# hbb1/2d-gaussian-splatting

Hardware: AMD Instinct MI355X
Metric: train iters/sec (full iteration: rasterizer fwd+bwd, L1+SSIM, normal+dist regularisers, Adam) + fwd Msplats/s @1080p (higher is better)
Workload: dtype f32; 1 GPU; garden: trained synthetic capture, 5400000 initial points -> 2136144 surfels after 2500 iterations of the reference schedule, 32 views of 1600x1060; steady-state iteration, every loss term on; P=2136144, image=1600x1060, n_pass=6, tiles=6700

## Files before the change

### 2d-gaussian-splatting_amd/build.py

```python
import os
import subprocess
import sys

HERE = os.path.dirname(os.path.abspath(__file__))
CSRC = os.path.join(HERE, "csrc")
LIB = os.path.join(HERE, "lib", "libsurfel_hip.so")
SOURCES = ["surfel_preprocess.hip", "surfel_forward.hip", "surfel_backward.hip", "surfel_backward_scan.hip", "surfel_sort.hip", "surfel_api.hip", "knn.hip", "box_probe.hip",
           "train_loss.hip", "train_post.hip", "train_fused.hip", "train_optim.hip", "train_api.hip",
           "device_scan.hip", "mesh_tsdf.hip", "mesh_unbounded.hip", "eval_geometry.hip", "eval_tnt.hip", "metrics_lpips.hip", "scene_image.hip", "frame_vis.hip", "view_image.hip", "mesh_cull.hip", "mesh_view.hip", "frame_jpeg.hip", "frame_png.hip", "scene_jpeg.hip", "scene_undistort.hip", "train_log.hip", "log_events.cpp", "mesh_simplify.hip", "mesh_texture.hip", "mesh_smooth.hip", "mesh_repair.hip"]
EXTRA = {"surfel_forward.hip": ["-fno-slp-vectorize"], "surfel_backward.hip": ["-fno-slp-vectorize", "-ffp-contract=off"],
         "surfel_backward_scan.hip": ["-fno-slp-vectorize", "-ffp-contract=off"],
         "mesh_tsdf.hip": ["-ffp-contract=off"],
         "eval_geometry.hip": ["-ffp-contract=off"],
         "eval_tnt.hip": ["-ffp-contract=off"],
         "scene_image.hip": ["-ffp-contract=off"],
         "frame_vis.hip": ["-ffp-contract=off"],
         "view_image.hip": ["-ffp-contract=off"],
         "mesh_cull.hip": ["-ffp-contract=off"],
         "mesh_view.hip": ["-ffp-contract=off"],
         "frame_jpeg.hip": ["-ffp-contract=off"],
         "scene_undistort.hip": ["-ffp-contract=off"],
         "train_log.hip": ["-ffp-contract=off"],
         "mesh_simplify.hip": ["-ffp-contract=off"],
         "mesh_texture.hip": ["-ffp-contract=off"],
         "mesh_smooth.hip": ["-ffp-contract=off"],
         "mesh_repair.hip": ["-ffp-contract=off"]}
HEADERS = ["surfel_common.h", "surfel_kernels.h", "surfel_blend_bwd.h", "train_kernels.h", "train_loss_body.h", "train_post_body.h", os.path.join("..", "..", "include", "surfel_hip.h"), os.path.join("..", "..", "include", "surfel_debug.h"),
           os.path.join("..", "..", "include", "surfel_train.h"), "mesh_mc_table.h", "mesh_mc.h", "block_ops.h", "side_util.h", "carve.h", "mesh_topology.h", os.path.join("..", "..", "include", "surfel_mesh.h"),
           os.path.join("..", "..", "include", "surfel_mesh_unbounded.h"), os.path.join("..", "..", "include", "surfel_eval.h"),
           os.path.join("..", "..", "include", "surfel_eval_tnt.h"), os.path.join("..", "..", "include", "surfel_metrics.h"),
           os.path.join("..", "..", "include", "surfel_scene.h"), "vis_turbo_table.h", os.path.join("..", "..", "include", "surfel_vis.h"),
           "vis_pixels.h", os.path.join("..", "..", "include", "surfel_view.h"), os.path.join("..", "..", "include", "surfel_cull.h"),
           "jpeg_tables.h", os.path.join("..", "..", "include", "surfel_jpeg.h"), os.path.join("..", "..", "include", "surfel_png.h"),
           os.path.join("..", "..", "include", "surfel_jpegdec.h"), os.path.join("..", "..", "include", "surfel_undistort.h"),
           "log_jet_table.h", os.path.join("..", "..", "include", "surfel_log.h"), "mesh_raster.h", "mesh_sample.h",
           os.path.join("..", "..", "include", "surfel_meshview.h"), os.path.join("..", "..", "include", "surfel_simplify.h"),
           os.path.join("..", "..", "include", "surfel_texture.h"), os.path.join("..", "..", "include", "surfel_smooth.h"),
           os.path.join("..", "..", "include", "surfel_repair.h")]
FLAGS = ["--offload-arch=gfx950", "-O3", "-std=c++17", "-fPIC", "-ffp-contract=fast", "-Wall", "-Wno-unused-result"]


def _stale(out, deps):
    if not os.path.exists(out):
        return True
    t = os.path.getmtime(out)
    return any(os.path.getmtime(d) > t for d in deps)


def build_variant(tag, defines, verbose=False):
    hipcc = os.environ.get("HIPCC", "/opt/rocm/bin/hipcc")
    bdir = os.path.join(HERE, "build_" + tag)
    os.makedirs(bdir, exist_ok=True)
    os.makedirs(os.path.join(HERE, "lib"), exist_ok=True)
    lib = os.path.join(HERE, "lib", "libsurfel_hip_%s.so" % tag)
    objs = []
    for src in SOURCES:
        obj = os.path.join(bdir, src + ".o")
        objs.append(obj)
        cmd = [hipcc] + FLAGS + list(defines) + EXTRA.get(src, []) + ["-c", os.path.join(CSRC, src), "-o", obj]
        if verbose:
            print(" ".join(cmd))
        subprocess.check_call(cmd)
    subprocess.check_call([hipcc, "--offload-arch=gfx950", "-shared", "-fPIC", "-o", lib] + objs)
    return lib


def build(force=False, verbose=False, ieee=False):
    hipcc = os.environ.get("HIPCC", "/opt/rocm/bin/hipcc")
    os.makedirs(os.path.join(HERE, "lib"), exist_ok=True)
    bdir = os.path.join(HERE, "build_ieee" if ieee else "build")
    os.makedirs(bdir, exist_ok=True)
    LIB = os.path.join(HERE, "lib", "libsurfel_hip_ieee.so" if ieee else "libsurfel_hip.so")
    hdrs = [os.path.join(CSRC, h) for h in HEADERS]
    objs = []
    for src in SOURCES:
        sp = os.path.join(CSRC, src)
        obj = os.path.join(bdir, src + ".o")
        objs.append(obj)
        if force or _stale(obj, [sp] + hdrs):
            cmd = [hipcc] + FLAGS + (["-DSURFEL_IEEE_MATH"] if ieee else []) + EXTRA.get(src, []) + ["-c", sp, "-o", obj]
            if verbose:
                print(" ".join(cmd))
            subprocess.check_call(cmd)
    if force or _stale(LIB, objs):
        cmd = [hipcc, "--offload-arch=gfx950", "-shared", "-fPIC", "-o", LIB] + objs
        if verbose:
            print(" ".join(cmd))
        subprocess.check_call(cmd)
    return LIB


if __name__ == "__main__":
    if "--variant" in sys.argv:
        k = sys.argv.index("--variant")
        print(build_variant(sys.argv[k + 1], sys.argv[k + 2:], verbose=False))
        sys.exit(0)
    print(build(force="--force" in sys.argv, verbose=True, ieee="--ieee" in sys.argv))
```

### 2d-gaussian-splatting_amd/csrc/surfel_api.hip

```cpp
#include <cstring>
#include <mutex>
#include <string>
#include <vector>

#include <hip/hip_runtime.h>

#include "../../include/surfel_debug.h"
#include "carve.h"
#include "surfel_common.h"
#include "surfel_kernels.h"
#include "train_kernels.h"

using namespace surfel;

namespace {

const char* kStageNames[] = {"preprocess_fwd", "depth_sort_scan", "emit_instances", "tile_sort", "tile_ranges", "blend_fwd",
                             "zero_grec", "blend_bwd", "preprocess_bwd", "knn", "tile_depth_sort"};
enum Stage { ST_PRE = 0, ST_SCAN, ST_EMIT, ST_SORT, ST_RANGES, ST_BLEND, ST_ZERO, ST_BBWD, ST_PBWD, ST_KNN, ST_TSORT, ST_COUNT };
static_assert(sizeof(kStageNames) / sizeof(kStageNames[0]) == ST_COUNT, "one name per stage");

struct CapEntry {
    int W = 0, H = 0; int64_t maxR = -1; unsigned frames = 0; int uniform_streak = 0; int boost = 0; unsigned last_overflow = 0;
    int slot() const; void begin_frame(); int64_t capacity(int end_bit) const; void record_count(int64_t R, bool overflowed);
};
constexpr int kCapEntries = 16;

constexpr int kMaxDevices = 32;
constexpr int kPinnedTotal = R_SLOTS + kCapEntries;
struct PerDevice { hipEvent_t ev = nullptr; uint32_t* pinned = nullptr; };

thread_local std::string g_err;
struct ThreadState {
    int64_t last_R = -1; int last_W = 0, last_H = 0;
    CapEntry caps[kCapEntries]; unsigned cap_next = 0; int cap_evictions = 0;
    int last_binning = 0;
    float stage_ms[16] = {}; int stage_id[16] = {}; int stage_n = 0;
    PerDevice dev[kMaxDevices];
};
thread_local ThreadState g_th;

int g_opt_cull = 1;
int g_opt_tile_sort = 1;
int g_opt_bwd_variant = 2;
int g_opt_stream = 1;
int g_opt_capacity = 1;
int g_opt_tile_order = 0;
surfel_hook_fn g_colour_hook = nullptr;
void* g_colour_hook_user = nullptr;
unsigned long long* g_blend_stats = nullptr;

int fail(int code, const char* what, hipError_t e = hipSuccess) {
    g_err = what;
    if (e != hipSuccess) { g_err += ": "; g_err += hipGetErrorString(e); }
    return code;
}

#define HIP_TRY(expr)                                                    \
    do {                                                                 \
        hipError_t _e = (expr);                                          \
        if (_e != hipSuccess) return fail(SURFEL_E_HIP, #expr, _e);      \
    } while (0)

struct GeomState {
    float* rec; float* depths; uint32_t* tiles_touched; uint8_t* clamped;
    uint32_t *dkey_a, *dkey_b, *ord_a, *ord_b;
    uint32_t* offsets;
    uint32_t* rects;
    float* shjac;
    char* temp;
    static GeomState carve(void* base, int P, size_t temp_bytes, size_t* total) {
        Carver c(base); GeomState g;
        g.rec = c.take<float>((size_t)P * REC_F);
        g.depths = c.take<float>(P);
        g.tiles_touched = c.take<uint32_t>(P);
        g.clamped = c.take<uint8_t>(P);
        g.dkey_a = c.take<uint32_t>(P); g.dkey_b = c.take<uint32_t>(P);
        g.ord_a = c.take<uint32_t>(P); g.ord_b = c.take<uint32_t>(P);
        g.offsets = c.take<uint32_t>(P);
        g.rects = c.take<uint32_t>(P);
        g.shjac = c.take<float>((size_t)9 * P);
        g.temp = c.take<char>(temp_bytes);
        if (total) *total = c.size();
        return g;
    }
};

struct BinState {
    uint32_t* point_list; uint32_t* vals_alt; uint32_t* keys_a; uint32_t* keys_b; char* sort_temp;
    float4* strm_rec = nullptr; uint32_t* strm_mask = nullptr;
    static bool wants_stream(size_t R) { return g_opt_stream != 0 && R > 0 && (long long)R <= STRM_MAX_R; }
    static BinState carve(void* base, size_t R, size_t sort_bytes, size_t* total, bool stream = false) {
        Carver c(base); BinState b;
        b.point_list = c.take<uint32_t>(R);
        b.vals_alt = c.take<uint32_t>(R);
        b.keys_a = c.take<uint32_t>(R);
        b.keys_b = c.take<uint32_t>(R);
        if (stream) {
            b.strm_rec = c.take<float4>(R * STRM_Q);
            b.strm_mask = c.take<uint32_t>(R);
        }
        b.sort_temp = c.take<char>(sort_bytes);
        if (total) *total = c.size();
        return b;
    }
};

struct ImgState {
    uint2* ranges; uint32_t* total; float* final_T; uint32_t* n_contrib; int* tile_map;
    static ImgState carve(void* base, int W, int H, size_t* total) {
        Carver c(base); ImgState im;
        const size_t tiles = (size_t)((W + TILE - 1) / TILE) * ((H + TILE - 1) / TILE);
        im.ranges = c.take<uint2>(tiles + R_SLOTS + 2);
        im.total = reinterpret_cast<uint32_t*>(im.ranges + tiles);
        im.final_T = c.take<float>((size_t)3 * W * H);
        im.n_contrib = c.take<uint32_t>((size_t)2 * W * H);
        im.tile_map = c.take<int>((size_t)tile_map_len((W + TILE - 1) / TILE, (H + TILE - 1) / TILE));
        if (total) *total = c.size();
        return im;
    }
};

struct StreamReg { const void* bin = nullptr; const void* img = nullptr; const float4* rec = nullptr; const uint32_t* mask = nullptr; bool jac = false; };
constexpr int kStreamRegs = 64;
StreamReg g_stream_regs[kStreamRegs];
unsigned g_stream_next = 0;
std::mutex g_stream_mu;
void stream_register(const void* bin, const void* img, const float4* rec, const uint32_t* mask, bool jac) {
    std::lock_guard<std::mutex> lk(g_stream_mu);
    for (auto& r : g_stream_regs) if (r.bin == bin) { r.img = img; r.rec = rec; r.mask = mask; r.jac = jac; return; }
    g_stream_regs[g_stream_next++ % kStreamRegs] = StreamReg{bin, img, rec, mask, jac};
}
bool stream_lookup(const void* bin, const void* img, const float4** rec, const uint32_t** mask, bool* jac) {
    std::lock_guard<std::mutex> lk(g_stream_mu);
    for (auto& r : g_stream_regs) if (r.bin == bin && r.img == img) {
        *jac = r.jac;
        if (!r.rec) return false;
        *rec = r.rec; *mask = r.mask;
        return true;
    }
    return false;
}

struct PendingStage { int stage; hipEvent_t e0, e1; };
std::vector<PendingStage> g_pending;
constexpr size_t kMaxPending = 8192;
std::mutex g_pending_mu;

struct StageTimer {
    int mode; hipStream_t s; hipEvent_t e0 = nullptr, e1 = nullptr;
    StageTimer(int mode_, hipStream_t s_) : mode(mode_), s(s_) {
        if (mode == 1) { (void)hipEventCreate(&e0); (void)hipEventCreate(&e1); }
    }
    ~StageTimer() { if (mode == 1) { (void)hipEventDestroy(e0); (void)hipEventDestroy(e1); } }
    bool armed = false;
    void begin(int stage = -1) {
        armed = mode == 1 || mode == 2 || (mode == 3 && stage == ST_BBWD);
        if (!armed) return;
        if (mode >= 2) { (void)hipEventCreate(&e0); (void)hipEventCreate(&e1); }
        (void)hipEventRecord(e0, s);
    }
    int end(int stage) {
        if (!armed) return 0;
        armed = false;
        (void)hipEventRecord(e1, s);
        if (mode >= 2) {
            std::lock_guard<std::mutex> lk(g_pending_mu);
            if (g_pending.size() >= kMaxPending) {
                (void)hipEventDestroy(g_pending.front().e0); (void)hipEventDestroy(g_pending.front().e1);
                g_pending.erase(g_pending.begin());
            }
            g_pending.push_back({stage, e0, e1});
            return 0;
        }
        hipError_t e = hipEventSynchronize(e1);
        if (e != hipSuccess) return (int)e;
        e = hipGetLastError();
        if (e != hipSuccess) return (int)e;
        float ms = 0.f; (void)hipEventElapsedTime(&ms, e0, e1);
        if (g_th.stage_n < 16) { g_th.stage_ms[g_th.stage_n] = ms; g_th.stage_id[g_th.stage_n] = stage; g_th.stage_n++; }
        return 0;
    }
};
#define STAGE_END(timer, st)                                                               \
    do {                                                                                   \
        int _e = (timer).end(st);                                                          \
        if (_e) return fail(SURFEL_E_HIP, kStageNames[st], (hipError_t)_e);                \
    } while (0)

PerDevice* per_device(int dev = -1) {
    int d = dev;
    if (d < 0 && hipGetDevice(&d) != hipSuccess) return nullptr;
    if (d < 0 || d >= kMaxDevices) return nullptr;
    return &g_th.dev[d];
}

hipEvent_t r_event() {
    PerDevice* pd = per_device();
    if (!pd) return nullptr;
    if (!pd->ev) { if (hipEventCreateWithFlags(&pd->ev, hipEventDisableTiming) != hipSuccess) pd->ev = nullptr; }
    return pd->ev;
}

uint32_t* pinned_u32() {
    PerDevice* pd = per_device();
    if (!pd) return nullptr;
    if (!pd->pinned) {
        if (hipHostMalloc(reinterpret_cast<void**>(&pd->pinned), sizeof(uint32_t) * (R_SLOTS + kCapEntries + 8), hipHostMallocMapped) != hipSuccess) pd->pinned = nullptr;
        else for (int k = 0; k < R_SLOTS + kCapEntries + 8; k++) pd->pinned[k] = 0u;
    }
    return pd->pinned;
}

int64_t pinned_total(const uint32_t* hR, bool host_total) {
    if (host_total) return (int64_t)hR[kPinnedTotal];
    int64_t R = 0;
    for (int k = 0; k < R_SLOTS; k++) R += (int64_t)hR[k];
    return R;
}

CapEntry* cap_entry(int W, int H) {
    for (auto& c : g_th.caps) if (c.W == W && c.H == H) return &c;
    CapEntry* c = &g_th.caps[g_th.cap_next++ % kCapEntries];
    if (c->W != 0) g_th.cap_evictions++;
    *c = CapEntry{};
    c->W = W; c->H = H;
    c->frames = ~0u;
    return c;
}

int CapEntry::slot() const { return (int)(this - g_th.caps); }
void CapEntry::begin_frame() {
    if (frames == ~0u) {
        frames = 0;
        if (uint32_t* hv = pinned_u32()) hv[R_SLOTS + slot()] = 0u;
    }
    frames++;
    if (boost > 0 && frames - last_overflow > 256u) { boost--; last_overflow = frames; }
}
int64_t CapEntry::capacity(int end_bit) const {
    if (maxR < 0) return 0;
    int64_t cap = maxR + (maxR >> (3 - boost)) + 4096;
    cap = (cap + 16383) / 16384 * 16384;
    return (cap > ((int64_t)1 << 20) || !capacity_binning_ok((size_t)cap, end_bit)) ? 0 : cap;
}
void CapEntry::record_count(int64_t R, bool overflowed) {
    g_th.last_R = R; g_th.last_W = W; g_th.last_H = H;
    if (overflowed) { if (boost < 2) boost++; last_overflow = frames; }
    maxR = R > maxR - maxR / 64 ? R : maxR - maxR / 64;
}

void run_tile_order(CapEntry* ce, const uint2* ranges, int gx, int gy, int* map, uint32_t* map_flag, int opt, hipStream_t s) {
    if (opt == 1) return;
    uint32_t* hv = pinned_u32();
    uint32_t* verdict = nullptr;
    if (hv && opt == 0) {
        const uint32_t v = hv[R_SLOTS + ce->slot()];
        if (v == 1u) ce->uniform_streak = ce->uniform_streak < 1000 ? ce->uniform_streak + 1 : 1000;
        else if (v == 2u) ce->uniform_streak = 0;
        void* dv = nullptr;
        if (hipHostGetDevicePointer(&dv, hv + R_SLOTS + ce->slot(), 0) == hipSuccess) verdict = static_cast<uint32_t*>(dv);
        if (verdict && ce->uniform_streak >= 4 && (ce->frames & 7u) != 0u) return;
    }
    launch_tile_order(ranges, gx, gy, map, map_flag, opt, verdict, s);
}

int higher_msb(uint32_t n) {
    int b = 0;
    while ((1ull << b) < (unsigned long long)n) b++;
    return b < 1 ? 1 : b;
}

int per_tile_pays(int64_t R, int P, int gx, int gy) {
    const int64_t tiles = (int64_t)gx * gy, Pf = P > (1 << 20) ? P : (1 << 20);
    if (R <= 640 * tiles) return 1;
    return (2 * R <= 7 * Pf && R <= 2048 * tiles) ? 1 : 0;
}

int alloc_bin(size_t n, size_t sort_bytes, bool stream, surfel_alloc_fn binning_alloc, void* binning_user, BinState* bin) {
    const bool strm = stream && BinState::wants_stream(n);
    size_t bytes = 0;
    BinState::carve(nullptr, n, sort_bytes, &bytes, strm);
    void* base = binning_alloc(binning_user, bytes > 0 ? bytes : 256);
    if (!base) return fail(SURFEL_E_ALLOC, "binning buffer allocation failed");
    *bin = BinState::carve(base, n, sort_bytes, nullptr, strm);
    return 0;
}

int bin_capacity(const PreprocessArgs& pa, int end_bit, int64_t cap, int64_t maxR, const GeomState& geom, const BinState& bin,
                 const ImgState& img, uint32_t* hR, hipEvent_t evR, StageTimer& tm, hipStream_t s) {
    uint32_t* n_dev = img.total + 2 * R_SLOTS;
    const bool odd = radix_sort_result_buffer((size_t)cap, 0, end_bit) == 1;
    uint32_t* va = odd ? bin.vals_alt : bin.point_list;
    uint32_t* vb = odd ? bin.point_list : bin.vals_alt;
    tm.begin();
    launch_bin_emit(pa.P, geom.tiles_touched, geom.rects, geom.offsets, geom.rec, bin.keys_a, va, pa.gx, (size_t)cap, bin.sort_temp, end_bit,
                    n_dev, hR + kPinnedTotal, s);
    HIP_TRY(hipEventRecord(evR, s));
    STAGE_END(tm, ST_EMIT);
    tm.begin();
    const bool fused_ranges = end_bit > 0;
    const int wk = radix_sort_pairs_u32_devn(bin.keys_a, va, bin.keys_b, vb, (size_t)cap, end_bit, n_dev, bin.sort_temp, fused_ranges ? img.ranges : nullptr, s);
    STAGE_END(tm, ST_SORT);
    if (!fused_ranges) { tm.begin(); launch_tile_ranges_devn((size_t)cap, n_dev, wk ? bin.keys_b : bin.keys_a, img.ranges, s); STAGE_END(tm, ST_RANGES); }
    tm.begin(); launch_tile_depth_sort(pa.gx * pa.gy, maxR, img.ranges, bin.point_list, geom.dkey_a, bin.vals_alt, bin.keys_a, bin.keys_b, fused_ranges, s);
    STAGE_END(tm, ST_TSORT);
    return 0;
}

int64_t bin_exact(const PreprocessArgs& pa, int end_bit, int per_tile, int64_t R, const GeomState& geom, BinState* bin,
                  const ImgState& img, const uint32_t* hR, hipEvent_t evR, bool stream, surfel_alloc_fn binning_alloc, void* binning_user,
                  StageTimer& tm, hipStream_t s) {
    if (per_tile < 0 && R < 0) {
        HIP_TRY(hipEventSynchronize(evR));
        per_tile = per_tile_pays(pinned_total(hR, false), pa.P, pa.gx, pa.gy);
    }
    tm.begin();
    const uint32_t* order = geom.ord_a;
    if (!per_tile) {
        const int which = radix_sort_pairs_u32(geom.dkey_a, geom.ord_a, geom.dkey_b, geom.ord_b, (size_t)pa.P, 0, 32, geom.temp, s, true);
        if (which < 0) return fail(SURFEL_E_LIMIT, "too many surfels for the depth sort");
        order = which ? geom.ord_b : geom.ord_a;
    }
    launch_scan_gather(geom.tiles_touched, order, pa.pack_tiles, geom.offsets, (size_t)pa.P, pa.zero_b, s);
    STAGE_END(tm, ST_SCAN);
    if (R < 0) {
        HIP_TRY(hipEventSynchronize(evR));
        R = pinned_total(hR, false);
    }
    if (int e = alloc_bin((size_t)R, radix_sort_scratch_bytes((size_t)R), stream, binning_alloc, binning_user, bin)) return e;
    if (R == 0) return 0;
    const bool odd = radix_sort_result_buffer((size_t)R, 0, end_bit) == 1;
    uint32_t* va = odd ? bin->vals_alt : bin->point_list;
    uint32_t* vb = odd ? bin->point_list : bin->vals_alt;
    tm.begin();
    launch_emit_instances(pa.P, geom.rec, geom.rects, order, pa.pack_tiles ? ((1u << PACK_ID_BITS) - 1u) : 0xffffffffu, geom.offsets, bin->keys_a, va, pa.gx,
                          reinterpret_cast<uint32_t*>(bin->sort_temp), (uint32_t)radix_sort_head_words((size_t)R), s);
    STAGE_END(tm, ST_EMIT);
    tm.begin();
    const int wk = radix_sort_pairs_u32(bin->keys_a, va, bin->keys_b, vb, (size_t)R, 0, end_bit, bin->sort_temp, s, true);
    if (wk < 0) return fail(SURFEL_E_LIMIT, "too many tile instances for the tile sort");
    STAGE_END(tm, ST_SORT);
    tm.begin(); launch_tile_ranges(R, wk ? bin->keys_b : bin->keys_a, img.ranges, s); STAGE_END(tm, ST_RANGES);
    if (per_tile) {
        tm.begin(); launch_tile_depth_sort(pa.gx * pa.gy, R, img.ranges, bin->point_list, geom.dkey_a, bin->vals_alt, bin->keys_a, bin->keys_b, false, s);
        STAGE_END(tm, ST_TSORT);
    }
    return R;
}

int blend(CapEntry* ce, int W, int H, int gx, int gy, const ImgState& img, const void* img_base, const BinState& bin, const float* rec,
          const float* background, float* out_color, float* out_others, int avg_list, bool jac, int tile_order, StageTimer& tm, hipStream_t s) {
    run_tile_order(ce, img.ranges, gx, gy, img.tile_map, img.total + 2 * R_SLOTS + 1, tile_order, s);
    BlendFwdArgs ba{};
    ba.W = W; ba.H = H; ba.gx = gx; ba.gy = gy;
    ba.ranges = img.ranges; ba.point_list = bin.point_list; ba.rec = rec; ba.bg = background;
    ba.out_color = out_color; ba.out_others = out_others; ba.final_T = img.final_T; ba.n_contrib = img.n_contrib;
    ba.tile_map = img.tile_map; ba.map_flag = img.total + 2 * R_SLOTS + 1; ba.map_len = tile_map_len(gx, gy);
    ba.stats = g_blend_stats;
    ba.avg_list = avg_list;
    ba.strm_rec = bin.strm_rec; ba.strm_mask = bin.strm_mask; ba.totals = img.total; ba.walk_word = img.total + 2 * R_SLOTS + 2;
    stream_register(bin.point_list, img_base, launch_blend_fwd_writes_stream(ba) ? bin.strm_rec : nullptr, bin.strm_mask, jac);
    tm.begin(); launch_blend_fwd(ba, s); STAGE_END(tm, ST_BLEND);
    return 0;
}

}

namespace surfel {
int api_fail(int code, const char* what, hipError_t e) { return fail(code, what, e); }
}

extern "C" {

int surfel_abi_version(void) { return SURFEL_ABI_VERSION; }
const char* surfel_last_error(void) { return g_err.c_str(); }
const char* surfel_stage_name(int stage) { return (stage >= 0 && stage < ST_COUNT) ? kStageNames[stage] : "?"; }
int surfel_last_stage_ms(float* ms, int cap) {
    int n = g_th.stage_n < cap ? g_th.stage_n : cap;
    for (int i = 0; i < n; i++) ms[i] = g_th.stage_ms[i];
    return n;
}
int surfel_last_stage_ids(int* ids, int cap) {
    int n = g_th.stage_n < cap ? g_th.stage_n : cap;
    for (int i = 0; i < n; i++) ids[i] = g_th.stage_id[i];
    return n;
}

int surfel_debug_sort_pairs(surfel_alloc_fn scratch_alloc, void* scratch_user, uint32_t* keys, uint32_t* vals, int64_t n,
                            int begin_bit, int end_bit, void* stream) {
    if (!scratch_alloc || n < 0 || (n > 0 && (!keys || !vals)) || begin_bit < 0 || end_bit > 32 || begin_bit > end_bit)
        return fail(SURFEL_E_INVALID, "bad arguments");
    if (n == 0) return 0;
    hipStream_t s = static_cast<hipStream_t>(stream);
    const size_t sb = radix_sort_scratch_bytes((size_t)n);
    const size_t words = align_up((size_t)n * sizeof(uint32_t));
    char* base = static_cast<char*>(scratch_alloc(scratch_user, 2 * words + sb));
    if (!base) return fail(SURFEL_E_ALLOC, "sort scratch allocation failed");
    uint32_t* kb = reinterpret_cast<uint32_t*>(base);
    uint32_t* vb = reinterpret_cast<uint32_t*>(base + words);
    const int w = radix_sort_pairs_u32(keys, vals, kb, vb, (size_t)n, begin_bit, end_bit, base + 2 * words, s);
    if (w < 0) return fail(SURFEL_E_LIMIT, "sort size limit");
    if (w == 1) {
        HIP_TRY(hipMemcpyAsync(keys, kb, (size_t)n * sizeof(uint32_t), hipMemcpyDeviceToDevice, s));
        HIP_TRY(hipMemcpyAsync(vals, vb, (size_t)n * sizeof(uint32_t), hipMemcpyDeviceToDevice, s));
    }
    HIP_TRY(hipGetLastError());
    return 0;
}

int surfel_debug_tile_depth_sort(int ntiles, int64_t n, uint32_t* ranges, uint32_t* point_list, const uint32_t* depth_keys, uint32_t* scratch,
                                 int decode, void* stream) {
    if (ntiles < 0 || n < 0 || n >= ((int64_t)1 << 32) || (ntiles > 0 && !ranges) || (n > 0 && (!point_list || !depth_keys || !scratch)))
        return fail(SURFEL_E_INVALID, "bad arguments");
    if (ntiles == 0) return 0;
    launch_tile_depth_sort(ntiles, n, reinterpret_cast<uint2*>(ranges), point_list, depth_keys, scratch, scratch + n, scratch + 2 * n, decode != 0,
                           static_cast<hipStream_t>(stream));
    HIP_TRY(hipGetLastError());
    return 0;
}
int surfel_debug_tile_depth_sort_classes(int* out, int cap) {
    if (!out || cap < 0) return fail(SURFEL_E_INVALID, "bad arguments");
    return tile_depth_sort_classes(out, cap);
}
int surfel_debug_set_tile_radix_min(int longest_network_run) { set_tile_radix_min(longest_network_run); return 0; }

int surfel_set_option(const char* name, int value) {
    if (name && std::strcmp(name, "cull") == 0) { g_opt_cull = value ? 1 : 0; return 0; }
    if (name && std::strcmp(name, "tile_depth_sort") == 0) { g_opt_tile_sort = value < 0 ? 0 : (value > 2 ? 2 : value); return 0; }
    if (name && std::strcmp(name, "large_sort") == 0) { set_large_sort_impl(value); return 0; }
    if (name && std::strcmp(name, "fwd_pipe") == 0) { set_fwd_pipe(value); return 0; }
    if (name && std::strcmp(name, "preprocess_dma") == 0) { set_preprocess_dma(value); return 0; }
    if (name && std::strcmp(name, "bwd_variant") == 0) { g_opt_bwd_variant = value < 0 ? 0 : (value > 3 ? 3 : value); return 0; }
    if (name && std::strcmp(name, "tile_stream") == 0) { g_opt_stream = value != 0; return 0; }
    if (name && std::strcmp(name, "capacity_binning") == 0) { g_opt_capacity = value != 0; return 0; }
    if (name && std::strcmp(name, "tile_order") == 0) { g_opt_tile_order = value < 0 ? 0 : (value > 2 ? 2 : value); return 0; }
    return fail(SURFEL_E_INVALID, "unknown option");
}

int surfel_set_backward_hook(surfel_hook_fn colour_ready, void* user) {
    g_colour_hook = colour_ready; g_colour_hook_user = user;
    return 0;
}

int surfel_debug_last_binning(void) { return g_th.last_binning; }
int surfel_debug_capacity_evictions(void) { return g_th.cap_evictions; }

int surfel_debug_image_layout(int width, int height, int64_t* out) {
    if (width <= 0 || height <= 0 || !out) return fail(SURFEL_E_INVALID, "bad arguments");
    size_t total = 0;
    ImgState::carve(nullptr, width, height, &total);
    char* const base = reinterpret_cast<char*>(static_cast<uintptr_t>(1) << 40);
    const ImgState im = ImgState::carve(base, width, height, nullptr);
    out[0] = (int64_t)total;
    out[1] = reinterpret_cast<char*>(im.final_T) - base;
    out[2] = reinterpret_cast<char*>(im.n_contrib) - base;
    out[3] = reinterpret_cast<char*>(im.tile_map) - base;
    return 0;
}
int surfel_debug_set_blend_stats(void* dev_u64x8) { g_blend_stats = static_cast<unsigned long long*>(dev_u64x8); return 0; }

int surfel_collect_stage_ms(float* sum_ms, int* count, int cap) {
    for (int i = 0; i < cap; i++) { sum_ms[i] = 0.f; count[i] = 0; }
    std::lock_guard<std::mutex> lk(g_pending_mu);
    for (auto& p : g_pending) {
        float ms = 0.f;
        if (hipEventSynchronize(p.e1) == hipSuccess && hipEventElapsedTime(&ms, p.e0, p.e1) == hipSuccess && p.stage < cap) {
            sum_ms[p.stage] += ms; count[p.stage]++;
        }
        (void)hipEventDestroy(p.e0); (void)hipEventDestroy(p.e1);
    }
    g_pending.clear();
    return ST_COUNT;
}

struct LazyPending { bool pending = false; int W = 0, H = 0, dev = -1; int64_t cap = 0; bool overflowed = false; int64_t R = 0; };
thread_local LazyPending g_lazy;

int64_t lazy_finish() {
    if (!g_lazy.pending) return g_lazy.R;
    PerDevice* pd = per_device(g_lazy.dev);
    uint32_t* hR = pd ? pd->pinned : nullptr;
    hipEvent_t evR = pd ? pd->ev : nullptr;
    if (!hR || !evR) return fail(SURFEL_E_HIP, "pinned buffer / event of the lazily counted frame's device not found");
    HIP_TRY(hipEventSynchronize(evR));
    const int64_t R = pinned_total(hR, true);
    g_lazy.pending = false;
    g_lazy.R = R;
    g_lazy.overflowed = R > g_lazy.cap;
    CapEntry* ce = cap_entry(g_lazy.W, g_lazy.H);
    if (ce->frames == ~0u) ce->frames = 0;
    ce->record_count(R, g_lazy.overflowed);
    return R;
}

int64_t surfel_forward_count(void) {
    const int64_t R = lazy_finish();
    if (R < 0) return R;
    if (g_lazy.overflowed) {
        g_lazy.overflowed = false;
        return fail(SURFEL_E_OVERFLOW, "the lazily counted frame held more tile instances than its capacity: render it again (its outputs are incomplete)");
    }
    return R;
}

int64_t surfel_rasterize_forward(surfel_alloc_fn geom_alloc, void* geom_user, surfel_alloc_fn binning_alloc, void* binning_user,
                                 surfel_alloc_fn image_alloc, void* image_user, int P, int D, int M, const float* background,
                                 int width, int height, const float* means3D, const float* shs, const float* colors_precomp,
                                 const float* opacities, const float* scales, float scale_modifier, const float* rotations,
                                 const float* transMat_precomp, const float* viewmatrix, const float* projmatrix,
                                 const float* cam_pos, float tan_fovx, float tan_fovy, int prefiltered, float* out_color,
                                 float* out_others, int* radii, int debug, void* stream) {
    (void)tan_fovx; (void)tan_fovy; (void)prefiltered;
    g_th.stage_n = 0;
    if (g_lazy.pending) { const int64_t r = lazy_finish(); if (r < 0) return r; }
    if (g_lazy.overflowed) {
        g_lazy.overflowed = false;
        return fail(SURFEL_E_OVERFLOW, "the previous lazily counted frame overflowed its capacity and surfel_forward_count() was never called for it");
    }
    const bool opt_lazy = (debug & SURFEL_OPT_LAZY_COUNT) != 0;
    const int opt_cull = (debug & SURFEL_OPT_NO_CULL) ? 0 : g_opt_cull;
    const int opt_tile_sort = ((debug >> 9) & 3) ? ((debug >> 9) & 3) - 1 : g_opt_tile_sort;
    const int opt_capacity = (debug & SURFEL_OPT_EXACT_BINNING) ? 0 : g_opt_capacity;
    const int opt_tile_order = ((debug >> 19) & 3) ? ((debug >> 19) & 3) - 1 : g_opt_tile_order;
    const bool opt_stream = !(debug & SURFEL_OPT_NO_STREAM);
    debug &= 0xff;
    g_th.last_binning = 0;
    hipStream_t s = static_cast<hipStream_t>(stream);
    if (!geom_alloc || !binning_alloc || !image_alloc) return fail(SURFEL_E_INVALID, "allocator callback is NULL");
    if (P < 0 || width <= 0 || height <= 0) return fail(SURFEL_E_INVALID, "bad sizes");
    if (P > 0) {
        if ((shs == nullptr) == (colors_precomp == nullptr)) return fail(SURFEL_E_INVALID, "provide exactly one of shs / colors_precomp");
        const bool has_sr = scales != nullptr && rotations != nullptr;
        if (has_sr == (transMat_precomp != nullptr) || ((scales != nullptr) != (rotations != nullptr)))
            return fail(SURFEL_E_INVALID, "provide exactly one of (scales, rotations) / transMat_precomp");
        if (!means3D || !opacities || !viewmatrix || !projmatrix || !cam_pos || !radii) return fail(SURFEL_E_INVALID, "required pointer is NULL");
        if (D < 0 || D > 3 || (shs && M < (D + 1) * (D + 1))) return fail(SURFEL_E_INVALID, "bad SH degree / coefficient count");
    }
    if (!background || !out_color || !out_others) return fail(SURFEL_E_INVALID, "required pointer is NULL");
    const int gx = (width + TILE - 1) / TILE, gy = (height + TILE - 1) / TILE;
    if (gx > 1023 || gy > 1023) return fail(SURFEL_E_LIMIT, "image larger than 16368 px per side");

    size_t img_bytes = 0;
    ImgState::carve(nullptr, width, height, &img_bytes);
    void* img_base = image_alloc(image_user, img_bytes);
    if (!img_base) return fail(SURFEL_E_ALLOC, "image buffer allocation failed");
    ImgState img = ImgState::carve(img_base, width, height, nullptr);
    HIP_TRY(hipMemsetAsync(img.ranges, 0, (size_t)(reinterpret_cast<char*>(img.final_T) - reinterpret_cast<char*>(img.ranges)), s));

    StageTimer tm(debug, s);
    const bool jac = P > 0 && opt_stream && shs != nullptr && M == 16;
    CapEntry* ce = cap_entry(width, height);
    ce->begin_frame();
    int64_t R = 0;
    bool blended = false;
    GeomState geom{}; BinState bin{};
    if (P == 0) {
        (void)geom_alloc(geom_user, 256);
        if (int e = alloc_bin(0, 0, false, binning_alloc, binning_user, &bin)) return e;
        g_lazy.R = 0;
    } else {
        const size_t psort_bytes = align_up(radix_sort_scratch_bytes((size_t)P));
        const size_t temp_bytes = psort_bytes + scan_scratch_words((size_t)P) * sizeof(uint32_t);
        size_t geom_bytes = 0;
        GeomState::carve(nullptr, P, temp_bytes, &geom_bytes);
        void* geom_base = geom_alloc(geom_user, geom_bytes);
        if (!geom_base) return fail(SURFEL_E_ALLOC, "geometry buffer allocation failed");
        geom = GeomState::carve(geom_base, P, temp_bytes, nullptr);

        PreprocessArgs pa{};
        pa.P = P; pa.D = D; pa.M = M; pa.W = width; pa.H = height; pa.gx = gx; pa.gy = gy; pa.scale_modifier = scale_modifier;
        pa.cull = opt_cull;
        pa.pack_tiles = P < (1 << PACK_ID_BITS) ? 1 : 0;
        pa.means3D = means3D; pa.opacities = opacities; pa.scales = scales; pa.rotations = rotations;
        pa.transMat_precomp = transMat_precomp; pa.colors_precomp = colors_precomp; pa.shs = shs;
        pa.viewmatrix = viewmatrix; pa.projmatrix = projmatrix; pa.campos = cam_pos;
        pa.rec = geom.rec; pa.depths = geom.depths; pa.depth_keys = geom.dkey_a; pa.ident = geom.ord_a; pa.radii = radii;
        pa.tiles_touched = geom.tiles_touched; pa.clamped = geom.clamped; pa.total_instances = img.total; pa.rects = geom.rects;
        pa.shjac = jac ? geom.shjac : nullptr;
        pa.zero_a = reinterpret_cast<uint32_t*>(geom.temp); pa.zero_a_words = (uint32_t)radix_sort_head_words((size_t)P);
        pa.zero_b = reinterpret_cast<uint32_t*>(geom.temp + psort_bytes); pa.zero_b_words = (uint32_t)scan_scratch_words((size_t)P);

        const int end_bit = higher_msb((uint32_t)(gx * gy));
        int per_tile = opt_tile_sort == 2 ? 1 : (opt_tile_sort == 0 ? 0 : -1);
        if (per_tile < 0 && g_th.last_R >= 0 && g_th.last_W == width && g_th.last_H == height) per_tile = per_tile_pays(g_th.last_R, P, gx, gy);
        const int64_t cap = (opt_capacity && per_tile == 1 && debug != 1) ? ce->capacity(end_bit) : 0;
        if (cap > 0) {
            if (int e = alloc_bin((size_t)cap, capacity_sort_scratch_bytes((size_t)cap, end_bit), opt_stream, binning_alloc, binning_user, &bin)) return e;
            pa.zero_c = reinterpret_cast<uint32_t*>(bin.sort_temp); pa.zero_c_words = (uint32_t)bin_emit_head_words();
            pa.block_totals = geom.offsets;
        }
        tm.begin(); launch_preprocess_fwd(pa, s); STAGE_END(tm, ST_PRE);
        uint32_t* hR = pinned_u32();
        hipEvent_t evR = r_event();
        if (!hR || !evR) return fail(SURFEL_E_HIP, "pinned buffer / event creation failed");
        if (cap == 0) {
            HIP_TRY(hipMemcpyAsync(hR, img.total, sizeof(uint32_t) * R_SLOTS, hipMemcpyDeviceToHost, s));
            HIP_TRY(hipEventRecord(evR, s));
        } else {
            if (int e = bin_capacity(pa, end_bit, cap, ce->maxR, geom, bin, img, hR, evR, tm, s)) return e;
            if (int e = blend(ce, width, height, gx, gy, img, img_base, bin, geom.rec, background, out_color, out_others, 0, jac, opt_tile_order, tm, s)) return e;
            if (opt_lazy) {
                g_lazy.pending = true; g_lazy.W = width; g_lazy.H = height; g_lazy.cap = cap; g_lazy.overflowed = false;
                if (hipGetDevice(&g_lazy.dev) != hipSuccess) g_lazy.dev = -1;
                g_th.last_binning = 4;
                HIP_TRY(hipGetLastError());
                return cap;
            }
            HIP_TRY(hipEventSynchronize(evR));
            R = pinned_total(hR, true);
            blended = R <= cap;
            g_th.last_binning = blended ? 1 : 2;
            if (!blended) {
                HIP_TRY(hipMemsetAsync(img.ranges, 0, sizeof(uint2) * (size_t)gx * gy, s));
                HIP_TRY(hipMemsetAsync(img.total + 2 * R_SLOTS, 0, 2 * sizeof(uint32_t), s));
            }
        }
        if (!blended) {
            R = bin_exact(pa, end_bit, per_tile, cap > 0 ? R : -1, geom, &bin, img, hR, evR, opt_stream, binning_alloc, binning_user, tm, s);
            if (R < 0) return R;
        }
        ce->record_count(R, cap > 0 && !blended);
        g_lazy.R = R;
    }
    if (!blended) {
        if (int e = blend(ce, width, height, gx, gy, img, img_base, bin, geom.rec, background, out_color, out_others, (int)(R / ((int64_t)gx * gy)), jac, opt_tile_order, tm, s)) return e;
    }
    HIP_TRY(hipGetLastError());
    return R;
}

int surfel_rasterize_backward(surfel_alloc_fn scratch_alloc, void* scratch_user, int P, int D, int M, int64_t R,
                              const float* background, int width, int height, const float* means3D, const float* shs,
                              const float* colors_precomp, const float* scales, float scale_modifier, const float* rotations,
                              const float* transMat_precomp, const float* viewmatrix, const float* projmatrix,
                              const float* cam_pos, float tan_fovx, float tan_fovy, const int* radii, const void* geom_buffer,
                              const void* binning_buffer, const void* image_buffer, const float* dL_dout_color,
                              const float* dL_dout_others, float* dL_dmeans2D, float* dL_dnormal, float* dL_dopacity,
                              float* dL_dcolors, float* dL_dmeans3D, float* dL_dtransMat, float* dL_dsh, float* dL_dscales,
                              float* dL_drots, int debug, void* stream) {
    (void)tan_fovx; (void)tan_fovy; (void)colors_precomp;
    g_th.stage_n = 0;
    const int debug_in = debug;
    const int opt_variant = (debug & SURFEL_OPT_BWD_SCAN) ? 3 : ((debug & SURFEL_OPT_BWD_QUAD) ? 1 : ((debug & SURFEL_OPT_BWD_ROWS) ? 0 : g_opt_bwd_variant));
    debug &= 0xff;
    hipStream_t s = static_cast<hipStream_t>(stream);
    if (P == 0) return 0;
    if (!scratch_alloc || !geom_buffer || !binning_buffer || !image_buffer) return fail(SURFEL_E_INVALID, "buffer / allocator is NULL");
    if (!dL_dout_color || !dL_dout_others || !dL_dmeans2D || !dL_dopacity || !dL_dcolors || !dL_dmeans3D)
        return fail(SURFEL_E_INVALID, "gradient pointer is NULL");
    if (transMat_precomp && !dL_dtransMat) return fail(SURFEL_E_INVALID, "dL_dtransMat is NULL but transMat_precomp was given");
    if (!transMat_precomp && (!dL_dscales || !dL_drots || !scales || !rotations)) return fail(SURFEL_E_INVALID, "scale/rotation pointers are NULL");
    const int gx = (width + TILE - 1) / TILE, gy = (height + TILE - 1) / TILE;

    GeomState geom = GeomState::carve(const_cast<void*>(geom_buffer), P, 0, nullptr);
    BinState bin = BinState::carve(const_cast<void*>(binning_buffer), (size_t)R, 0, nullptr);
    ImgState img = ImgState::carve(const_cast<void*>(image_buffer), width, height, nullptr);

    const size_t grec_bytes = align_up((size_t)(R > 0 ? R : 1) * GREC_F * sizeof(float));
    const size_t cut_bytes = align_up((size_t)gx * gy * sizeof(uint2));
    float* grec = static_cast<float*>(scratch_alloc(scratch_user, grec_bytes + cut_bytes + (size_t)P));
    if (!grec) return fail(SURFEL_E_ALLOC, "gradient record allocation failed");
    const bool use_cut = (debug_in & SURFEL_OPT_TILE_CUTS) ? true : ((debug_in & SURFEL_OPT_ZERO_RECORDS) ? false : R >= ((int64_t)1 << 21));
    uint2* cut = use_cut ? reinterpret_cast<uint2*>(reinterpret_cast<char*>(grec) + grec_bytes) : nullptr;
    uint8_t* has_rec = use_cut ? reinterpret_cast<uint8_t*>(grec) + grec_bytes + cut_bytes : nullptr;
    if (has_rec) HIP_TRY(hipMemsetAsync(has_rec, 0, (size_t)P, s));
    StageTimer tm(debug, s);

    BlendBwdArgs bb{};
    bb.W = width; bb.H = height; bb.gx = gx; bb.gy = gy;
    bb.ranges = img.ranges; bb.point_list = bin.point_list; bb.rec = geom.rec; bb.bg = background;
    bb.final_T = img.final_T; bb.n_contrib = img.n_contrib; bb.dL_dpix = dL_dout_color; bb.dL_dothers = dL_dout_others;
    bb.tile_map = img.tile_map; bb.map_flag = img.total + 2 * R_SLOTS + 1; bb.map_len = tile_map_len(gx, gy);
    bb.grec = grec; bb.cut = cut; bb.has_rec = has_rec; bb.depths = geom.depths; bb.variant = opt_variant; bb.stats = g_blend_stats; bb.walk_word = img.total + 2 * R_SLOTS + 2;
    bool have_jac = false;
    {
        const float4* srec = nullptr; const uint32_t* smask = nullptr;
        const bool found = stream_lookup(binning_buffer, image_buffer, &srec, &smask, &have_jac);
        if (found && !(debug_in & SURFEL_OPT_BWD_GATHER) && g_opt_stream) { bb.strm_rec = srec; bb.strm_mask = smask; }
    }
    bb.n_dev = img.total + 2 * R_SLOTS; bb.n_cap = (uint32_t)(R < 0xffffffffll ? R : 0xffffffffll);
    if (R > 0) {
        const bool auto_walk = opt_variant == 2;
        bb.variant = auto_walk ? 0 : opt_variant;
        if (auto_walk && !g_blend_stats) {
            if (R >= ((int64_t)1 << 21)) bb.variant = R < ((int64_t)1 << 26) ? 3 : 0;
            else bb.scan_rule = 1;
        }
        tm.begin(ST_BBWD);
        launch_blend_bwd(bb, s);
        STAGE_END(tm, ST_BBWD);
    }

    PreprocessBwdArgs pb{};
    pb.P = P; pb.D = D; pb.M = M; pb.W = width; pb.H = height; pb.scale_modifier = scale_modifier;
    pb.coop = (debug_in & SURFEL_OPT_PBWD_COOP) ? 1 : ((debug_in & SURFEL_OPT_PBWD_THREAD) ? 0 : ((R >= (int64_t)6 * P && R >= ((int64_t)32 << 20)) ? 1 : 0));
    pb.shjac = (have_jac && !(debug_in & SURFEL_OPT_PBWD_NO_JAC)) ? geom.shjac : nullptr;
    pb.means3D = means3D; pb.radii = radii; pb.shs = shs; pb.clamped = geom.clamped; pb.scales = scales; pb.rotations = rotations;
    pb.transMat_precomp = transMat_precomp; pb.viewmatrix = viewmatrix; pb.projmatrix = projmatrix; pb.campos = cam_pos;
    pb.rec = geom.rec; pb.tiles_touched = geom.tiles_touched; pb.grec = grec; pb.cut = cut; pb.has_rec = has_rec; pb.depths = geom.depths; pb.gx = gx;
    pb.n_dev = bb.n_dev; pb.n_cap = bb.n_cap;
    pb.dL_dtransMat = dL_dtransMat; pb.dL_dnormal = dL_dnormal; pb.dL_dopacity = dL_dopacity; pb.dL_dcolors = dL_dcolors;
    pb.dL_dsh = dL_dsh; pb.dL_dmeans2D = dL_dmeans2D; pb.dL_dmeans3D = dL_dmeans3D; pb.dL_dscales = dL_dscales; pb.dL_drots = dL_drots;
    tm.begin();
    if (g_colour_hook) {
        launch_colour_gradients(pb, s);
        pb.keep_colors = 1;
        g_colour_hook(g_colour_hook_user);
    }
    launch_preprocess_bwd(pb, s);
    STAGE_END(tm, ST_PBWD);
    HIP_TRY(hipGetLastError());
    return 0;
}

int surfel_mark_visible(int P, const float* means3D, const float* viewmatrix, const float* projmatrix, uint8_t* present,
                        void* stream) {
    (void)projmatrix;
    if (P < 0 || (P > 0 && (!means3D || !viewmatrix || !present))) return fail(SURFEL_E_INVALID, "bad arguments");
    launch_mark_visible(P, means3D, viewmatrix, present, static_cast<hipStream_t>(stream));
    HIP_TRY(hipGetLastError());
    return 0;
}

int surfel_knn_dist2(surfel_alloc_fn scratch_alloc, void* scratch_user, int P, const float* points, float* mean_dist2,
                     void* stream) {
    if (P < 0 || (P > 0 && (!points || !mean_dist2 || !scratch_alloc))) return fail(SURFEL_E_INVALID, "bad arguments");
    if (P == 0) return 0;
    const size_t bytes = knn_scratch_bytes(P);
    void* scratch = scratch_alloc(scratch_user, bytes);
    if (!scratch) return fail(SURFEL_E_ALLOC, "knn scratch allocation failed");
    launch_knn(P, points, mean_dist2, scratch, bytes, static_cast<hipStream_t>(stream));
    HIP_TRY(hipGetLastError());
    return 0;
}

}
```

### 2d-gaussian-splatting_amd/csrc/surfel_kernels.h

```cpp
#pragma once
#include <hip/hip_runtime.h>
#include <stdint.h>

namespace surfel {

struct PreprocessArgs {
    int P, D, M, W, H, gx, gy;
    int cull;
    int pack_tiles;
    float scale_modifier;
    const float* means3D; const float* opacities; const float* scales; const float* rotations;
    const float* transMat_precomp; const float* colors_precomp; const float* shs;
    const float* viewmatrix; const float* projmatrix; const float* campos;
    float* rec; float* depths; uint32_t* depth_keys; uint32_t* ident; int* radii; uint32_t* tiles_touched; uint8_t* clamped;
    uint32_t* rects;
    float* shjac;
    uint32_t* total_instances;
    uint32_t* block_totals;
    uint32_t* zero_a; uint32_t zero_a_words;
    uint32_t* zero_b; uint32_t zero_b_words;
    uint32_t* zero_c; uint32_t zero_c_words;
};

struct BlendFwdArgs {
    int W, H, gx, gy;
    const uint2* ranges; const uint32_t* point_list; const float* rec; const float* bg;
    float* out_color; float* out_others; float* final_T; uint32_t* n_contrib;
    const int* tile_map; const uint32_t* map_flag; int map_len;
    unsigned long long* stats;
    int avg_list;
    float4* strm_rec; uint32_t* strm_mask;
    const uint32_t* totals; uint32_t* walk_word;
};

struct BlendBwdArgs {
    int W, H, gx, gy;
    const uint2* ranges; const uint32_t* point_list; const float* rec; const float* bg;
    const float* final_T; const uint32_t* n_contrib;
    const int* tile_map; const uint32_t* map_flag; int map_len;
    const float* dL_dpix; const float* dL_dothers;
    float* grec;
    uint2* cut;
    uint8_t* has_rec;
    const float* depths;
    int variant;
    const float4* strm_rec; const uint32_t* strm_mask;
    int scan_rule;
    const uint32_t* walk_word;
    const uint32_t* n_dev; uint32_t n_cap;
    unsigned long long* stats;
};

struct PreprocessBwdArgs {
    int P, D, M, W, H;
    int coop;
    int keep_colors;
    const float* shjac;
    float scale_modifier;
    const float* means3D; const int* radii; const float* shs; const uint8_t* clamped;
    const float* scales; const float* rotations; const float* transMat_precomp;
    const float* viewmatrix; const float* projmatrix; const float* campos;
    const float* rec; const uint32_t* tiles_touched; const float* grec;
    const uint2* cut; const uint8_t* has_rec; const float* depths; int gx;
    const uint32_t* n_dev; uint32_t n_cap;
    float* dL_dtransMat; float* dL_dnormal; float* dL_dopacity; float* dL_dcolors; float* dL_dsh;
    float* dL_dmeans2D; float* dL_dmeans3D; float* dL_dscales; float* dL_drots;
};

void launch_preprocess_fwd(const PreprocessArgs& a, hipStream_t s);
void set_preprocess_dma(int v);
void launch_emit_instances(int P, float* rec, const uint32_t* rects, const uint32_t* order, uint32_t id_mask, const uint32_t* offsets_sorted, uint32_t* keys,
                           uint32_t* vals, int gx, uint32_t* zero_ptr, uint32_t zero_words, hipStream_t s);
void launch_tile_ranges(int64_t R, const uint32_t* keys, uint2* ranges, hipStream_t s);
int tile_map_len(int gx, int gy);
void launch_tile_order(const uint2* ranges, int gx, int gy, int* map, uint32_t* map_flag , int force, uint32_t* verdict, hipStream_t s);
void launch_blend_fwd(const BlendFwdArgs& a, hipStream_t s);
bool launch_blend_fwd_writes_stream(const BlendFwdArgs& a);
void set_fwd_pipe(int v);
void launch_mark_visible(int P, const float* means3D, const float* vm, uint8_t* present, hipStream_t s);
void launch_blend_bwd(const BlendBwdArgs& a, hipStream_t s);
void launch_blend_bwd_scan(const BlendBwdArgs& a, hipStream_t s);
void launch_preprocess_bwd(const PreprocessBwdArgs& a, hipStream_t s);
void launch_colour_gradients(const PreprocessBwdArgs& a, hipStream_t s);
void launch_knn(int P, const float* points, float* out, void* scratch, size_t scratch_bytes, hipStream_t s);
size_t knn_scratch_bytes(int P);
size_t radix_sort_scratch_bytes(size_t n);
void set_large_sort_impl(int v);
int radix_sort_passes(size_t n, int begin_bit, int end_bit);
int radix_sort_result_buffer(size_t n, int begin_bit, int end_bit);
int radix_sort_pairs_u32(uint32_t* keys_a, uint32_t* vals_a, uint32_t* keys_b, uint32_t* vals_b, size_t n, int begin_bit, int end_bit,
                         void* scratch, hipStream_t s, bool head_zeroed = false);
size_t radix_sort_head_words(size_t n);
size_t scan_scratch_words(size_t n);
int tile_depth_sort_classes(int* out, int cap);
void set_tile_radix_min(int v);
void launch_tile_depth_sort(int ntiles, int64_t R, uint2* ranges, uint32_t* point_list, const uint32_t* depth_keys, uint32_t* tmp_ids,
                            uint32_t* tmp_keys, uint32_t* tmp_rank, bool decode, hipStream_t s);
void launch_scan_gather(const uint32_t* vals, const uint32_t* order, int packed, uint32_t* out, size_t n, void* zeroed_scratch, hipStream_t s);
bool capacity_binning_ok(size_t cap, int end_bit);
size_t capacity_sort_scratch_bytes(size_t cap, int end_bit);
size_t bin_emit_head_words();
void launch_bin_emit(int P, const uint32_t* tiles_touched, const uint32_t* rects, const uint32_t* block_totals, float* rec, uint32_t* keys, uint32_t* vals,
                     int gx, size_t cap, void* sort_scratch , int end_bit, uint32_t* n_out, uint32_t* n_host ,
                     hipStream_t s);
int radix_sort_pairs_u32_devn(uint32_t* keys_a, uint32_t* vals_a, uint32_t* keys_b, uint32_t* vals_b, size_t cap, int end_bit, const uint32_t* n_dev,
                              void* scratch, uint2* ranges, hipStream_t s);
void launch_tile_ranges_devn(size_t cap, const uint32_t* n_dev, const uint32_t* keys, uint2* ranges, hipStream_t s);

}
```

### 2d-gaussian-splatting_amd/csrc/surfel_preprocess.hip

```cpp
#include "surfel_common.h"
#include "surfel_kernels.h"

namespace surfel {


__device__ __constant__ float SH_C0 = 0.28209479177387814f;
__device__ __constant__ float SH_C1 = 0.4886025119029199f;
__device__ __constant__ float SH_C2[5] = {1.0925484305920792f, -1.0925484305920792f, 0.31539156525252005f,
                                          -1.0925484305920792f, 0.5462742152960396f};
__device__ __constant__ float SH_C3[7] = {-0.5900435899266435f, 2.890611442640554f, -0.4570457994644658f,
                                          0.3731763325901154f, -0.4570457994644658f, 1.445305721320277f,
                                          -0.5900435899266435f};

__device__ __forceinline__ void sh_basis_gradient(int D, float x, float y, float z, float (&Bx)[16], float (&By)[16], float (&Bz)[16]) {
#pragma unroll
    for (int k = 0; k < 16; k++) { Bx[k] = 0.f; By[k] = 0.f; Bz[k] = 0.f; }
    if (D > 0) {
        By[1] = -SH_C1; Bz[2] = SH_C1; Bx[3] = -SH_C1;
        if (D > 1) {
            const float xx = x * x, yy = y * y, zz = z * z, xy = x * y, yz = y * z, xz = x * z;
            Bx[4] = SH_C2[0] * y; By[4] = SH_C2[0] * x;
            By[5] = SH_C2[1] * z; Bz[5] = SH_C2[1] * y;
            Bx[6] = SH_C2[2] * -2.f * x; By[6] = SH_C2[2] * -2.f * y; Bz[6] = SH_C2[2] * 4.f * z;
            Bx[7] = SH_C2[3] * z; Bz[7] = SH_C2[3] * x;
            Bx[8] = SH_C2[4] * 2.f * x; By[8] = SH_C2[4] * -2.f * y;
            if (D > 2) {
                Bx[9] = SH_C3[0] * 6.f * xy; By[9] = SH_C3[0] * 3.f * (xx - yy);
                Bx[10] = SH_C3[1] * yz; By[10] = SH_C3[1] * xz; Bz[10] = SH_C3[1] * xy;
                Bx[11] = SH_C3[2] * -2.f * xy; By[11] = SH_C3[2] * (-3.f * yy + 4.f * zz - xx); Bz[11] = SH_C3[2] * 8.f * yz;
                Bx[12] = SH_C3[3] * -6.f * xz; By[12] = SH_C3[3] * -6.f * yz; Bz[12] = SH_C3[3] * 3.f * (2.f * zz - xx - yy);
                Bx[13] = SH_C3[4] * (-3.f * xx + 4.f * zz - yy); By[13] = SH_C3[4] * -2.f * xy; Bz[13] = SH_C3[4] * 8.f * xz;
                Bx[14] = SH_C3[5] * 2.f * xz; By[14] = SH_C3[5] * -2.f * yz; Bz[14] = SH_C3[5] * (xx - yy);
                Bx[15] = SH_C3[6] * 3.f * (xx - yy); By[15] = SH_C3[6] * -6.f * xy;
            }
        }
    }
}

__device__ __forceinline__ void sh_colour_jacobian(int D, float x, float y, float z, const float4 (&c4)[12], float (&G)[3][3]) {
    float Bx[16], By[16], Bz[16];
    sh_basis_gradient(D, x, y, z, Bx, By, Bz);
#pragma unroll
    for (int c = 0; c < 3; c++) { G[c][0] = 0.f; G[c][1] = 0.f; G[c][2] = 0.f; }
#pragma unroll
    for (int v = 0; v < 12; v++) {
        const float cv[4] = {c4[v].x, c4[v].y, c4[v].z, c4[v].w};
#pragma unroll
        for (int e = 0; e < 4; e++) {
            const int flat = 4 * v + e, k = flat / 3, c = flat % 3;
            G[c][0] = __builtin_fmaf(Bx[k], cv[e], G[c][0]); G[c][1] = __builtin_fmaf(By[k], cv[e], G[c][1]); G[c][2] = __builtin_fmaf(Bz[k], cv[e], G[c][2]);
        }
    }
}

__device__ __forceinline__ uint32_t preprocess_one(const PreprocessArgs& a, const int i, const float4* sh_lds = nullptr) {
    int rad_out = 0;
    uint32_t tiles = 0;
    uint32_t dkey = 0xffffffffu;
    const float* __restrict__ vm = a.viewmatrix;
    const float px = a.means3D[3 * i], py = a.means3D[3 * i + 1], pz = a.means3D[3 * i + 2];
    const float opa_in = a.opacities[i];
    float4 q_in = make_float4(1.f, 0.f, 0.f, 0.f);
    float2 sc_in = make_float2(1.f, 1.f);
    if (a.transMat_precomp == nullptr) {
        q_in = reinterpret_cast<const float4*>(a.rotations)[i];
        sc_in = reinterpret_cast<const float2*>(a.scales)[i];
    }
    const float vx = vm[0] * px + vm[4] * py + vm[8] * pz + vm[12];
    const float vy = vm[1] * px + vm[5] * py + vm[9] * pz + vm[13];
    const float vz = vm[2] * px + vm[6] * py + vm[10] * pz + vm[14];
    do {
        if (vz <= 0.2f) break;
        float T[9];
        float nx, ny, nz;
        if (a.transMat_precomp == nullptr) {
            const float4 q = q_in;
            const float2 sc = sc_in;
            const float s = rsqrtf(q.x * q.x + q.y * q.y + q.z * q.z + q.w * q.w);
            const float w = q.x * s, x = q.y * s, y = q.z * s, z = q.w * s;
            const float sx = a.scale_modifier * sc.x, sy = a.scale_modifier * sc.y;
            const float L0x = (1.f - 2.f * (y * y + z * z)) * sx, L0y = (2.f * (x * y + w * z)) * sx, L0z = (2.f * (x * z - w * y)) * sx;
            const float L1x = (2.f * (x * y - w * z)) * sy, L1y = (1.f - 2.f * (x * x + z * z)) * sy, L1z = (2.f * (y * z + w * x)) * sy;
            const float L2x = 2.f * (x * z + w * y), L2y = 2.f * (y * z - w * x), L2z = 1.f - 2.f * (x * x + y * y);
            float Pm[12];
            world2pix(a.projmatrix, a.W, a.H, Pm);
#pragma unroll
            for (int c = 0; c < 3; c++) {
                T[3 * c + 0] = L0x * Pm[0 * 3 + c] + L0y * Pm[1 * 3 + c] + L0z * Pm[2 * 3 + c];
                T[3 * c + 1] = L1x * Pm[0 * 3 + c] + L1y * Pm[1 * 3 + c] + L1z * Pm[2 * 3 + c];
                T[3 * c + 2] = px * Pm[0 * 3 + c] + py * Pm[1 * 3 + c] + pz * Pm[2 * 3 + c] + Pm[3 * 3 + c];
            }
            nx = vm[0] * L2x + vm[4] * L2y + vm[8] * L2z;
            ny = vm[1] * L2x + vm[5] * L2y + vm[9] * L2z;
            nz = vm[2] * L2x + vm[6] * L2y + vm[10] * L2z;
        } else {
#pragma unroll
            for (int k = 0; k < 9; k++) T[k] = a.transMat_precomp[9 * (size_t)i + k];
            nx = 0.f; ny = 0.f; nz = 1.f;
        }
        const float cosv = -(vx * nx + vy * ny + vz * nz);
        if (cosv == 0.f) break;
        const float flip = cosv > 0.f ? 1.f : -1.f;
        nx *= flip; ny *= flip; nz *= flip;

        const float t0 = CUTOFF * CUTOFF, t2 = -1.0f;
        const float dist = t0 * T[6] * T[6] + t0 * T[7] * T[7] + t2 * T[8] * T[8];
        if (dist == 0.f) break;
        const float f0 = t0 / dist, f2 = t2 / dist;
        const float cx = f0 * T[0] * T[6] + f0 * T[1] * T[7] + f2 * T[2] * T[8];
        const float cy = f0 * T[3] * T[6] + f0 * T[4] * T[7] + f2 * T[5] * T[8];
        const float hx = cx * cx - (f0 * T[0] * T[0] + f0 * T[1] * T[1] + f2 * T[2] * T[2]);
        const float hy = cy * cy - (f0 * T[3] * T[3] + f0 * T[4] * T[4] + f2 * T[5] * T[5]);
        const float ex = sqrtf(fmaxf(1e-4f, hx)), ey = sqrtf(fmaxf(1e-4f, hy));
        const float radius = ceilf(fmaxf(fmaxf(ex, ey), CUTOFF * FILTER_SIZE));
        const int irad = (int)radius;
        const Rect rc = tile_rect(cx, cy, irad, a.gx, a.gy);
        const int ntiles = (rc.x1 - rc.x0) * (rc.y1 - rc.y0);
        if (ntiles == 0) break;

        float r = 0.f, g = 0.f, b = 0.f;
        uint8_t clampbits = 0;
        if (a.colors_precomp == nullptr) {
            const float4* __restrict__ shq = reinterpret_cast<const float4*>(a.shs + (size_t)i * a.M * 3);
            float dx = px - a.campos[0], dy = py - a.campos[1], dz = pz - a.campos[2];
            const float il = rsqrtf(dx * dx + dy * dy + dz * dz);
            dx *= il; dy *= il; dz *= il;
            float B[16];
#pragma unroll
            for (int k = 1; k < 16; k++) B[k] = 0.f;
            B[0] = SH_C0;
            int nb = 1;
            if (a.D > 0) {
                B[1] = -SH_C1 * dy; B[2] = SH_C1 * dz; B[3] = -SH_C1 * dx; nb = 4;
                if (a.D > 1) {
                    const float xx = dx * dx, yy = dy * dy, zz = dz * dz, xy = dx * dy, yz = dy * dz, xz = dx * dz;
                    B[4] = SH_C2[0] * xy; B[5] = SH_C2[1] * yz; B[6] = SH_C2[2] * (2.f * zz - xx - yy);
                    B[7] = SH_C2[3] * xz; B[8] = SH_C2[4] * (xx - yy); nb = 9;
                    if (a.D > 2) {
                        B[9] = SH_C3[0] * dy * (3.f * xx - yy); B[10] = SH_C3[1] * xy * dz;
                        B[11] = SH_C3[2] * dy * (4.f * zz - xx - yy); B[12] = SH_C3[3] * dz * (2.f * zz - 3.f * xx - 3.f * yy);
                        B[13] = SH_C3[4] * dx * (4.f * zz - xx - yy); B[14] = SH_C3[5] * dz * (xx - yy);
                        B[15] = SH_C3[6] * dx * (xx - 3.f * yy); nb = 16;
                    }
                }
            }
            if (a.M == 16) {
                float4 c4[12];
#pragma unroll
                for (int v = 0; v < 12; v++) c4[v] = make_float4(0.f, 0.f, 0.f, 0.f);
                if (sh_lds) {
                    asm volatile("s_waitcnt vmcnt(0)" ::: "memory");
#pragma unroll
                    for (int v = 0; v < 12; v++) c4[v] = sh_lds[v];
                } else if (a.D > 2) {
#pragma unroll
                    for (int v = 0; v < 12; v++) c4[v] = shq[v];
                } else if (a.D == 2) {
#pragma unroll
                    for (int v = 0; v < 7; v++) c4[v] = shq[v];
                } else if (a.D == 1) {
#pragma unroll
                    for (int v = 0; v < 3; v++) c4[v] = shq[v];
                } else {
                    c4[0] = shq[0];
                }
                float acc[3] = {0.f, 0.f, 0.f};
#pragma unroll
                for (int v = 0; v < 12; v++) {
                    const float cv[4] = {c4[v].x, c4[v].y, c4[v].z, c4[v].w};
#pragma unroll
                    for (int e = 0; e < 4; e++) {
                        const int flat = 4 * v + e;
                        acc[flat % 3] += B[flat / 3] * cv[e];
                    }
                }
                r = acc[0]; g = acc[1]; b = acc[2];
                if (a.shjac) {
                    float G[3][3];
                    sh_colour_jacobian(a.D, dx, dy, dz, c4, G);
#pragma unroll
                    for (int c = 0; c < 3; c++) {
#pragma unroll
                        for (int q = 0; q < 3; q++) a.shjac[(size_t)(3 * c + q) * a.P + i] = G[c][q];
                    }
                }
            } else {
                const float* __restrict__ sh = a.shs + (size_t)i * a.M * 3;
                r = SH_C0 * sh[0]; g = SH_C0 * sh[1]; b = SH_C0 * sh[2];
                if (nb > 1) {
#pragma unroll
                    for (int k = 1; k < 16; k++) {
                        if (k < nb && k < a.M) { r += B[k] * sh[3 * k]; g += B[k] * sh[3 * k + 1]; b += B[k] * sh[3 * k + 2]; }
                    }
                }
            }
            r += 0.5f; g += 0.5f; b += 0.5f;
            clampbits = (r < 0.f ? 1 : 0) | (g < 0.f ? 2 : 0) | (b < 0.f ? 4 : 0);
            r = fmaxf(r, 0.f); g = fmaxf(g, 0.f); b = fmaxf(b, 0.f);
        } else {
            r = a.colors_precomp[3 * (size_t)i]; g = a.colors_precomp[3 * (size_t)i + 1]; b = a.colors_precomp[3 * (size_t)i + 2];
        }
        float bx0 = 1.f, bx1 = 0.f, by0 = 1.f, by1 = 0.f;
        float ecx = cx, ecy = cy, Sxx = FOOT_UNBOUNDED, Sxy = 0.f, Syy = FOOT_UNBOUNDED, r2sq = 0.f, Sdet = 1.f;
        {
            const float opa = opa_in;
            if (opa * 255.f >= 0.999f) {
                const float rmax = 2.f * __logf(fmaxf(opa * 255.f, 1.f)) * 1.0001f + 1e-3f;
                const float r2 = sqrtf(0.5f * rmax) + 0.05f;
                r2sq = r2 * r2;
                bx0 = cx - r2; bx1 = cx + r2; by0 = cy - r2; by1 = cy + r2;
                const float tw2 = T[8] * T[8];
                const float dc = rmax * (T[6] * T[6] + T[7] * T[7]) - tw2;
                bool bounded = dc < -1e-3f * tw2;
                if (bounded) {
                    const float g0 = rmax / dc, g2 = -1.f / dc;
                    const float ox = T[2] / T[8], oy = T[5] / T[8];
                    const float U0 = T[0] - ox * T[6], U1 = T[1] - ox * T[7], U2 = T[2] - ox * T[8];
                    const float V0 = T[3] - oy * T[6], V1 = T[4] - oy * T[7], V2 = T[5] - oy * T[8];
                    const float ex_ = g0 * U0 * T[6] + g0 * U1 * T[7] + g2 * U2 * T[8];
                    const float ey_ = g0 * V0 * T[6] + g0 * V1 * T[7] + g2 * V2 * T[8];
                    const float sxx = ex_ * ex_ - (g0 * U0 * U0 + g0 * U1 * U1 + g2 * U2 * U2);
                    const float sxy = ex_ * ey_ - (g0 * U0 * V0 + g0 * U1 * V1 + g2 * U2 * V2);
                    const float syy = ey_ * ey_ - (g0 * V0 * V0 + g0 * V1 * V1 + g2 * V2 * V2);
                    constexpr float EPS = 0.09f;
                    const float ixx = fmaxf(sxx, 0.f) * 1.002f + EPS, iyy = fmaxf(syy, 0.f) * 1.002f + EPS;
                    const float det = fmaxf(ixx * iyy - sxy * sxy, EPS * (ixx + iyy - 2.f * EPS)) + 4e-7f * ixx * iyy;
                    bounded = (ex_ == ex_) && (ey_ == ey_) && (det == det) && (ixx < 1e12f) && (iyy < 1e12f) && (fabsf(sxy) < 1e12f);
                    if (bounded) {
                        ecx = ox + ex_; ecy = oy + ey_; Sxx = ixx; Sxy = sxy; Syy = iyy; Sdet = det;
                        const float mx = sqrtf(ixx) + 1e-4f * fabsf(ecx) + 0.01f, my = sqrtf(iyy) + 1e-4f * fabsf(ecy) + 0.01f;
                        bx0 = fminf(bx0, ecx - mx); bx1 = fmaxf(bx1, ecx + mx);
                        by0 = fminf(by0, ecy - my); by1 = fmaxf(by1, ecy + my);
                    }
                }
                if (!bounded) { bx0 = by0 = -3.0e38f; bx1 = by1 = 3.0e38f; Sxx = Syy = FOOT_UNBOUNDED; Sxy = 0.f; Sdet = 1.f; }
            }
            if (!a.cull) { bx0 = by0 = -3.0e38f; bx1 = by1 = 3.0e38f; ecx = cx; ecy = cy; Sxx = Syy = FOOT_UNBOUNDED; Sxy = 0.f; Sdet = 1.f; }
        }
        float4* __restrict__ rec = reinterpret_cast<float4*>(a.rec + (size_t)i * REC_F);
        rec[0] = make_float4(T[0], T[1], T[2], T[3]);
        rec[1] = make_float4(T[4], T[5], T[6], T[7]);
        rec[2] = make_float4(T[8], cx, cy, opa_in);
        rec[3] = make_float4(nx, ny, nz, r);
        int ex0 = rc.x0, ex1 = rc.x1, ey0 = rc.y0, ey1 = rc.y1;
        {
            const float lo_x = ceilf(fmaxf(bx0, 0.f)), hi_x = floorf(fminf(bx1, (float)(a.gx * TILE)));
            const float lo_y = ceilf(fmaxf(by0, 0.f)), hi_y = floorf(fminf(by1, (float)(a.gy * TILE)));
            if (!(lo_x <= hi_x) || !(lo_y <= hi_y)) { ex1 = ex0; ey1 = ey0; }
            else {
                ex0 = max(ex0, (int)lo_x >> 4); ex1 = min(ex1, ((int)hi_x >> 4) + 1);
                ey0 = max(ey0, (int)lo_y >> 4); ey1 = min(ey1, ((int)hi_y >> 4) + 1);
                if (ex1 < ex0) ex1 = ex0;
                if (ey1 < ey0) ey1 = ey0;
            }
        }
        const uint32_t rectbits = (uint32_t)ex0 | ((uint32_t)ey0 << 10) | ((uint32_t)(ex1 - ex0) << 20);
        a.rects[i] = rectbits;
        rec[4] = make_float4(g, b, 0.f , __uint_as_float(rectbits));
        rec[5] = make_float4(ecx, ecy, Sxx, Sxy);
        rec[6] = make_float4(Syy, r2sq, Sdet, 0.f);
        dkey = __float_as_uint(vz);
        a.clamped[i] = clampbits;
        rad_out = irad;
        tiles = (uint32_t)((ex1 - ex0) * (ey1 - ey0));
    } while (false);
    a.radii[i] = rad_out;
    a.tiles_touched[i] = tiles;
    a.depths[i] = vz;
    a.depth_keys[i] = tiles ? dkey : 0xffffffffu;
    a.ident[i] = a.pack_tiles ? ((uint32_t)i | (min(tiles, PACK_TILES_MAX) << PACK_ID_BITS)) : (uint32_t)i;
    return tiles;
}

#ifndef PRE_FWD_MINWG
#define PRE_FWD_MINWG 4
#endif
template <bool DMA>
__global__ void __launch_bounds__(256, PRE_FWD_MINWG) preprocess_fwd_kernel(PreprocessArgs a) {
    __shared__ uint32_t s_tot[4], s_vis[4];
    const int i = blockIdx.x * blockDim.x + threadIdx.x;
    __shared__ float4 s_sh[DMA ? 4 : 1][DMA ? 64 * 12 : 1];
    const float4* sh_lds = nullptr;
    if (DMA && a.shs != nullptr && a.colors_precomp == nullptr && a.M == 16 && a.D > 2) {
        const int wave = threadIdx.x >> 6, lane = threadIdx.x & 63;
        const int first = blockIdx.x * 256 + wave * 64;
        const int npieces = 12 * min(64, a.P - first);
        const float4* __restrict__ src = reinterpret_cast<const float4*>(a.shs) + (size_t)first * 12;
        const unsigned base = __builtin_amdgcn_readfirstlane(lds_offset(&s_sh[wave][0]));
#pragma unroll
        for (int v = 0; v < 12; v++) {
            const int p = v * 64 + lane;
            if (p < npieces) dma16(src + p, base + (unsigned)v * 1024u);
        }
        sh_lds = &s_sh[wave][lane * 12];
    }
    for (uint32_t w = (uint32_t)i; w < a.zero_a_words; w += gridDim.x * blockDim.x) a.zero_a[w] = 0u;
    for (uint32_t w = (uint32_t)i; w < a.zero_b_words; w += gridDim.x * blockDim.x) a.zero_b[w] = 0u;
    for (uint32_t w = (uint32_t)i; w < a.zero_c_words; w += gridDim.x * blockDim.x) a.zero_c[w] = 0u;
    uint32_t tiles = i < a.P ? preprocess_one(a, i, sh_lds) : 0u;
    const uint32_t vis = (uint32_t)__popcll(__ballot(tiles != 0u));
#pragma unroll
    for (int o = 32; o > 0; o >>= 1) tiles += __shfl_xor(tiles, o);
    if ((threadIdx.x & 63) == 0) { s_tot[threadIdx.x >> 6] = tiles; s_vis[threadIdx.x >> 6] = vis; }
    __syncthreads();
    if (threadIdx.x == 0) {
        const uint32_t t = s_tot[0] + s_tot[1] + s_tot[2] + s_tot[3];
        if (a.block_totals) a.block_totals[blockIdx.x] = t;
        if (t) {
            atomicAdd(a.total_instances + (blockIdx.x % R_SLOTS), t);
            atomicAdd(a.total_instances + R_SLOTS + (blockIdx.x % R_SLOTS), s_vis[0] + s_vis[1] + s_vis[2] + s_vis[3]);
        }
    }
}

__global__ void __launch_bounds__(256) emit_instances_kernel(int P, float* rec, const uint32_t* __restrict__ rects, const uint32_t* __restrict__ order,
                                                             uint32_t id_mask, const uint32_t* __restrict__ offsets_sorted, uint32_t* __restrict__ keys,
                                                             uint32_t* __restrict__ vals, int gx, uint32_t* __restrict__ zero_ptr,
                                                             uint32_t zero_words) {
    const int k = blockIdx.x * blockDim.x + threadIdx.x;
    for (uint32_t w = (uint32_t)k; w < zero_words; w += gridDim.x * blockDim.x) zero_ptr[w] = 0u;
    uint32_t off = 0, i = 0, rectbits = 0;
    int n = 0;
    if (k < P) {
        off = (k == 0) ? 0u : offsets_sorted[k - 1];
        n = (int)(offsets_sorted[k] - off);
        if (n > 0) {
            i = order[k] & id_mask;
            rectbits = rects[i];
            rec[(size_t)i * REC_F + 18] = __uint_as_float(off);
        }
    }
    const int lane = threadIdx.x & 63;
    int wave_total = n;
#pragma unroll
    for (int o = 32; o > 0; o >>= 1) wave_total += __shfl_xor(wave_total, o);
    if (wave_total < 8 * 64) {
        const int x0 = rectbits & 1023, y0 = (rectbits >> 10) & 1023, w = rectbits >> 20;
        int x = 0, y = 0;
        for (int t = 0; t < n; t++) {
            keys[off + t] = (uint32_t)((y0 + y) * gx + (x0 + x));
            vals[off + t] = i;
            if (++x == w) { x = 0; ++y; }
        }
        return;
    }
    for (int s = 0; s < 64; s++) {
        const int ns = __builtin_amdgcn_readlane(n, s);
        if (ns == 0) continue;
        const uint32_t offs = (uint32_t)__builtin_amdgcn_readlane((int)off, s);
        const uint32_t is = (uint32_t)__builtin_amdgcn_readlane((int)i, s);
        const uint32_t rb = (uint32_t)__builtin_amdgcn_readlane((int)rectbits, s);
        const int x0 = rb & 1023, y0 = (rb >> 10) & 1023, w = rb >> 20;
        const float inv_w = 1.0f / (float)w;
        for (int t = lane; t < ns; t += 64) {
            const int y = (int)(((float)t + 0.5f) * inv_w);
            const int x = t - y * w;
            keys[offs + t] = (uint32_t)((y0 + y) * gx + (x0 + x));
            vals[offs + t] = is;
        }
    }
}

constexpr int TO_CLASSES = 24, TO_THREADS = 1024, TO_WAVES = TO_THREADS / 64;
__device__ __forceinline__ int len_class(uint32_t len) { return len < 16u ? 0 : min(TO_CLASSES - 1, 32 - __clz(len >> 4)); }

__global__ void __launch_bounds__(TO_THREADS) tile_order_kernel(const uint2* __restrict__ ranges, int gx, int gy, int* __restrict__ map, int map_len,
                                                                uint32_t* __restrict__ map_flag, int force, uint32_t* __restrict__ verdict) {
    __shared__ uint32_t s_wsum[TO_WAVES], s_wmax[TO_WAVES], s_bound[9], s_uniform;
    __shared__ uint32_t s_cnt[TO_CLASSES], s_off[TO_CLASSES], s_wcnt[TO_WAVES][TO_CLASSES];
    const int n = gx * gy, ggx = (gx + 3) >> 2, G = ggx * gy;
    const int tid = threadIdx.x, lane = tid & 63, wave = tid >> 6;
    const int k = (n + TO_THREADS - 1) / TO_THREADS;
    const int q = n >> 3, r = n & 7;
    uint32_t sum = 0, mx = 0;
    for (int j = 0; j < k; j++) {
        const int t = tid * k + j;
        if (t < n) { const uint2 rg = ranges[t]; const uint32_t len = rg.y - rg.x; sum += len; mx = max(mx, len); }
    }
    uint32_t x = sum;
#pragma unroll
    for (int o = 1; o < 64; o <<= 1) { const uint32_t y = __shfl_up(x, o); if (lane >= o) x += y; }
#pragma unroll
    for (int o = 32; o > 0; o >>= 1) mx = max(mx, (uint32_t)__shfl_xor((int)mx, o));
    if (lane == 63) s_wsum[wave] = x;
    if (lane == 0) s_wmax[wave] = mx;
    __syncthreads();
    uint32_t pre = x - sum;
    for (int w = 0; w < wave; w++) pre += s_wsum[w];
    for (int j = 0; j < k; j++) {
        const int t = tid * k + j;
        if (t < n) {
#pragma unroll
            for (int xc = 0; xc < 8; xc++) {
                const int B = xc < r ? xc * (q + 1) : r * (q + 1) + (xc - r) * q;
                if (t == B) s_bound[xc] = pre;
            }
            const uint2 rg = ranges[t];
            pre += rg.y - rg.x;
        }
    }
    if (tid == TO_THREADS - 1) s_bound[8] = pre;
    if (tid < TO_CLASSES) s_cnt[tid] = 0u;
    __syncthreads();
    if (tid == 0) {
        uint32_t total = 0, maxlen = 0;
        for (int w = 0; w < TO_WAVES; w++) { total += s_wsum[w]; maxlen = max(maxlen, s_wmax[w]); }
        uint32_t busiest = 0;
        for (int xc = 0; xc < 8; xc++) {
            const uint32_t lo = q == 0 && xc >= r ? total : s_bound[xc];
            const uint32_t hi = xc == 7 ? total : (q == 0 && xc + 1 >= r ? total : s_bound[xc + 1]);
            busiest = max(busiest, hi - lo);
        }
        const bool uniform = total == 0u || ((unsigned long long)busiest * 800ull <= (unsigned long long)total * 115ull &&
                                             (unsigned long long)maxlen * (unsigned long long)n <= 4ull * total);
        s_uniform = force == 1 ? 1u : (force == 2 ? 0u : (uniform ? 1u : 0u));
        if (s_uniform) map_flag[0] = 0u;
        if (verdict) verdict[0] = uniform ? 1u : 2u;
    }
    __syncthreads();
    if (s_uniform) return;
    for (int b = tid; b < map_len; b += TO_THREADS) map[b] = -1;
    auto group_class = [&](int g) {
        const int ty = g / ggx, tx0 = (g - ty * ggx) << 2;
        uint32_t len4 = 0;
        for (int j = 0; j < 4 && tx0 + j < gx; j++) { const uint2 rg = ranges[ty * gx + tx0 + j]; len4 += rg.y - rg.x; }
        return len_class(len4);
    };
    const unsigned long long lt = (1ull << lane) - 1ull;
    for (int g0 = 0; g0 < G; g0 += TO_THREADS) {
        const int g = g0 + tid;
        const int c = g < G ? group_class(g) : -1;
        unsigned long long rest = __ballot(c >= 0);
        while (rest) {
            const int cc = __shfl(c, __builtin_ctzll(rest));
            const unsigned long long m = __ballot(c == cc);
            if (lane == __builtin_ctzll(m)) atomicAdd(&s_cnt[cc], (uint32_t)__popcll(m));
            rest &= ~m;
        }
    }
    __syncthreads();
    if (tid == 0) {
        uint32_t run = 0;
        for (int c = TO_CLASSES - 1; c >= 0; c--) { s_off[c] = run; run += s_cnt[c]; }
    }
    for (int g0 = 0; g0 < G; g0 += TO_THREADS) {
        for (int i = tid; i < TO_WAVES * TO_CLASSES; i += TO_THREADS) (&s_wcnt[0][0])[i] = 0u;
        __syncthreads();
        const int g = g0 + tid;
        const int c = g < G ? group_class(g) : -1;
        uint32_t rank = 0;
        unsigned long long rest = __ballot(c >= 0);
        while (rest) {
            const int cc = __shfl(c, __builtin_ctzll(rest));
            const unsigned long long m = __ballot(c == cc);
            if (c == cc) rank = (uint32_t)__popcll(m & lt);
            if (lane == __builtin_ctzll(m)) s_wcnt[wave][cc] = (uint32_t)__popcll(m);
            rest &= ~m;
        }
        __syncthreads();
        if (c >= 0) {
            uint32_t kpos = s_off[c] + rank;
            for (int w = 0; w < wave; w++) kpos += s_wcnt[w][c];
            const int ty = g / ggx, tx0 = (g - ty * ggx) << 2;
            for (int j = 0; j < 4 && tx0 + j < gx; j++) map[((((kpos >> 3) << 2) + j) << 3) | (kpos & 7u)] = ty * gx + tx0 + j;
        }
        __syncthreads();
        if (tid < TO_CLASSES) { uint32_t add = 0; for (int w = 0; w < TO_WAVES; w++) add += s_wcnt[w][tid]; s_off[tid] += add; }
        __syncthreads();
    }
    if (tid == 0) map_flag[0] = 1u;
}

__global__ void __launch_bounds__(256) tile_ranges_kernel(int64_t R, const uint32_t* __restrict__ keys, uint2* __restrict__ ranges) {
    const int64_t k = (int64_t)blockIdx.x * blockDim.x + threadIdx.x;
    if (k >= R) return;
    const uint32_t tile = keys[k];
    if (k == 0) ranges[tile].x = 0;
    else {
        const uint32_t prev = keys[k - 1];
        if (prev != tile) { ranges[prev].y = (uint32_t)k; ranges[tile].x = (uint32_t)k; }
    }
    if (k == R - 1) ranges[tile].y = (uint32_t)R;
}

__global__ void __launch_bounds__(256) mark_visible_kernel(int P, const float* __restrict__ means3D, const float* __restrict__ vm,
                                                           uint8_t* __restrict__ present) {
    const int i = blockIdx.x * blockDim.x + threadIdx.x;
    if (i >= P) return;
    const float vz = vm[2] * means3D[3 * i] + vm[6] * means3D[3 * i + 1] + vm[10] * means3D[3 * i + 2] + vm[14];
    present[i] = vz > 0.2f ? 1 : 0;
}

__device__ __constant__ float BSH_C0 = 0.28209479177387814f;
__device__ __constant__ float BSH_C1 = 0.4886025119029199f;
__device__ __constant__ float BSH_C2[5] = {1.0925484305920792f, -1.0925484305920792f, 0.31539156525252005f,
                                           -1.0925484305920792f, 0.5462742152960396f};
__device__ __constant__ float BSH_C3[7] = {-0.5900435899266435f, 2.890611442640554f, -0.4570457994644658f,
                                           0.3731763325901154f, -0.4570457994644658f, 1.445305721320277f,
                                           -0.5900435899266435f};


constexpr int NV = 18;

struct RecWalk {
    uint32_t key, idp, x0, rw, gx;
    uint32_t tile, col;
    __device__ __forceinline__ void init(uint32_t depth_bits, uint32_t i, uint32_t rectbits, int gx_) {
        key = depth_bits; idp = i; gx = (uint32_t)gx_;
        x0 = rectbits & 1023u; rw = rectbits >> 20;
        tile = ((rectbits >> 10) & 1023u) * gx + x0; col = 0u;
    }
    __device__ __forceinline__ bool has_record(const uint2* __restrict__ cut) const {
        const uint2 c = cut[tile];
        return key < c.x || (key == c.x && idp < c.y);
    }
    __device__ __forceinline__ void next() { col++; tile++; if (col == rw) { col = 0u; tile += gx - rw; } }
};

__device__ __forceinline__ void store3(float* p, size_t i, float x, float y, float z) { p[3 * i] = x; p[3 * i + 1] = y; p[3 * i + 2] = z; }

constexpr uint32_t HEAVY_MIN = 128;

#ifndef PRE_BWD_MINWG
#define PRE_BWD_MINWG 4
#endif
template <bool COOP, bool CUT, bool JAC>
__global__ void __launch_bounds__(256, PRE_BWD_MINWG) preprocess_bwd_kernel(PreprocessBwdArgs a) {
    __shared__ float4 s_sum[COOP ? 256 * 5 : 1];
    if (frame_overflowed(a.n_dev, a.n_cap)) return;
    const int i = blockIdx.x * blockDim.x + threadIdx.x;
    float4 hs0 = make_float4(0.f, 0.f, 0.f, 0.f), hs1 = hs0, hs2 = hs0, hs3 = hs0, hs4 = hs0;
    bool heavy = false;
    {
        const int lane = threadIdx.x & 63;
        uint32_t hb = 0, hc = 0, hd = 0, hr = 0;
        if (i < a.P && a.radii[i] > 0 && (!CUT || a.has_rec[i])) {
            hc = a.tiles_touched[i];
            if (hc > HEAVY_MIN) {
                hb = __float_as_uint(a.rec[(size_t)i * REC_F + 18]);
                hr = __float_as_uint(a.rec[(size_t)i * REC_F + 19]);
                hd = __float_as_uint(a.depths[i]);
            }
        }
        heavy = hc > HEAVY_MIN;
        unsigned long long hv = __ballot(heavy);
        while (hv) {
            const int src = __builtin_ctzll(hv);
            hv &= hv - 1ull;
            const uint32_t b = __shfl(hb, src), c = __shfl(hc, src), key = __shfl(hd, src), rb = __shfl(hr, src);
            const uint32_t idp = (uint32_t)(blockIdx.x * blockDim.x + (threadIdx.x & ~63) + src);
            const uint32_t x0 = rb & 1023u, y0 = (rb >> 10) & 1023u, w = rb >> 20;
            const float inv_w = 1.0f / (float)w;
            float4 p0 = make_float4(0.f, 0.f, 0.f, 0.f), p1 = p0, p2 = p0, p3 = p0, p4 = p0;
            const float4* __restrict__ g4 = reinterpret_cast<const float4*>(a.grec);
            for (uint32_t r = (uint32_t)lane; r < c; r += 64u) {
                bool has = true;
                if (CUT) {
                    const uint32_t row = (uint32_t)(((float)r + 0.5f) * inv_w);
                    const uint2 ct = a.cut[(y0 + row) * (uint32_t)a.gx + x0 + (r - row * w)];
                    has = key < ct.x || (key == ct.x && idp < ct.y);
                }
                if (has) {
                    const float4* __restrict__ sp = g4 + (size_t)(b + r) * 5;
                    const float4 v0 = sp[0], v1 = sp[1], v2 = sp[2], v3 = sp[3], v4 = sp[4];
                    p0.x += v0.x; p0.y += v0.y; p0.z += v0.z; p0.w += v0.w; p1.x += v1.x; p1.y += v1.y; p1.z += v1.z; p1.w += v1.w;
                    p2.x += v2.x; p2.y += v2.y; p2.z += v2.z; p2.w += v2.w; p3.x += v3.x; p3.y += v3.y; p3.z += v3.z; p3.w += v3.w;
                    p4.x += v4.x; p4.y += v4.y;
                }
            }
#pragma unroll
            for (int o = 32; o > 0; o >>= 1) {
                p0.x += __shfl_xor(p0.x, o); p0.y += __shfl_xor(p0.y, o); p0.z += __shfl_xor(p0.z, o); p0.w += __shfl_xor(p0.w, o);
                p1.x += __shfl_xor(p1.x, o); p1.y += __shfl_xor(p1.y, o); p1.z += __shfl_xor(p1.z, o); p1.w += __shfl_xor(p1.w, o);
                p2.x += __shfl_xor(p2.x, o); p2.y += __shfl_xor(p2.y, o); p2.z += __shfl_xor(p2.z, o); p2.w += __shfl_xor(p2.w, o);
                p3.x += __shfl_xor(p3.x, o); p3.y += __shfl_xor(p3.y, o); p3.z += __shfl_xor(p3.z, o); p3.w += __shfl_xor(p3.w, o);
                p4.x += __shfl_xor(p4.x, o); p4.y += __shfl_xor(p4.y, o);
            }
            if (lane == src) { hs0 = p0; hs1 = p1; hs2 = p2; hs3 = p3; hs4 = p4; }
        }
    }
    if (COOP) {
        const int lane = threadIdx.x & 63, wbase = threadIdx.x & ~63;
        uint32_t beg = 0, cnt = 0, dbits = 0, rbits = 0;
        if (i < a.P && a.radii[i] > 0 && !heavy && (!CUT || a.has_rec[i])) {
            beg = __float_as_uint(a.rec[(size_t)i * REC_F + 18]);
            rbits = __float_as_uint(a.rec[(size_t)i * REC_F + 19]);
            cnt = a.tiles_touched[i];
            dbits = __float_as_uint(a.depths[i]);
        }
        const int grp = lane / 5, q = lane - 5 * grp;
        const bool worker = grp < 12;
        const int leader = grp * 5;
        int owner = worker ? grp : 64;
        int next = 12;
        uint32_t b = __shfl(beg, owner & 63), c = __shfl(cnt, owner & 63), r = 0;
        RecWalk rw;
        rw.init(__shfl(dbits, owner & 63), (uint32_t)(blockIdx.x * blockDim.x + wbase + (owner & 63)), __shfl(rbits, owner & 63), a.gx);
        if (!worker) c = 0;
        float4 acc = make_float4(0.f, 0.f, 0.f, 0.f);
        const float4* __restrict__ g4 = reinterpret_cast<const float4*>(a.grec);
        for (;;) {
            const bool done = worker && owner < 64 && r >= c;
            const unsigned long long req = __ballot(done && q == 0);
            if (req) {
                if (done) s_sum[(wbase + owner) * 5 + q] = acc;
                const int rank = __popcll(req & ((1ull << leader) - 1ull));
                int nown = next + rank;
                next += __popcll(req);
                if (done) {
                    owner = nown < 64 ? nown : 64;
                    acc = make_float4(0.f, 0.f, 0.f, 0.f); r = 0;
                }
                const uint32_t nb = __shfl(beg, owner & 63), nc = __shfl(cnt, owner & 63);
                const uint32_t nd = __shfl(dbits, owner & 63), nr = __shfl(rbits, owner & 63);
                if (done) { b = nb; c = owner < 64 ? nc : 0u; rw.init(nd, (uint32_t)(blockIdx.x * blockDim.x + wbase + (owner & 63)), nr, a.gx); }
            }
            const bool live = worker && owner < 64 && r < c;
            if (!__any(worker && owner < 64)) break;
            if (live) {
                if (!CUT || rw.has_record(a.cut)) {
                    const float4 v = g4[(size_t)(b + r) * 5 + q];
                    acc.x += v.x; acc.y += v.y; acc.z += v.z; acc.w += v.w;
                }
                rw.next();
                r++;
            }
        }
        __syncthreads();
    }
    if (i >= a.P) return;
    const bool precomp = a.transMat_precomp != nullptr;
    const bool vis = a.radii[i] > 0;
    float4* __restrict__ gshq = (a.shs && a.dL_dsh) ? reinterpret_cast<float4*>(a.dL_dsh + (size_t)i * a.M * 3) : nullptr;
    if (!vis) {
        a.dL_dopacity[i] = 0.f;
        if (a.dL_dnormal) store3(a.dL_dnormal, i, 0.f, 0.f, 0.f);
        if (!a.keep_colors) store3(a.dL_dcolors, i, 0.f, 0.f, 0.f);
        store3(a.dL_dmeans2D, i, 0.f, 0.f, 0.f); store3(a.dL_dmeans3D, i, 0.f, 0.f, 0.f);
        if (a.dL_dtransMat) {
#pragma unroll
            for (int q = 0; q < 9; q++) a.dL_dtransMat[9 * (size_t)i + q] = 0.f;
        }
        if (!precomp) {
            reinterpret_cast<float2*>(a.dL_dscales)[i] = make_float2(0.f, 0.f);
            reinterpret_cast<float4*>(a.dL_drots)[i] = make_float4(0.f, 0.f, 0.f, 0.f);
        }
        if (gshq) {
            if (a.M == 16) {
#pragma unroll
                for (int v = 0; v < 12; v++) gshq[v] = make_float4(0.f, 0.f, 0.f, 0.f);
            } else {
                for (int v = 0; v < a.M * 3; v++) a.dL_dsh[(size_t)i * a.M * 3 + v] = 0.f;
            }
        }
        return;
    }
    float g[NV];
#pragma unroll
    for (int q = 0; q < NV; q++) g[q] = 0.f;
    const float4* __restrict__ rq = reinterpret_cast<const float4*>(a.rec + (size_t)i * REC_F);
    const float4 r4 = rq[4], r0 = rq[0], r1 = rq[1], r2 = rq[2];
    const uint32_t beg = __float_as_uint(r4.z);
    const uint32_t end = beg + a.tiles_touched[i];
    auto add_rec = [&](const float4& v0, const float4& v1, const float4& v2, const float4& v3, const float4& v4) {
        g[0] += v0.x; g[1] += v0.y; g[2] += v0.z; g[3] += v0.w;
        g[4] += v1.x; g[5] += v1.y; g[6] += v1.z; g[7] += v1.w;
        g[8] += v2.x; g[9] += v2.y; g[10] += v2.z; g[11] += v2.w;
        g[12] += v3.x; g[13] += v3.y; g[14] += v3.z; g[15] += v3.w;
        g[16] += v4.x; g[17] += v4.y;
    };
    if (COOP) {
        const float4 v0 = s_sum[threadIdx.x * 5 + 0], v1 = s_sum[threadIdx.x * 5 + 1], v2 = s_sum[threadIdx.x * 5 + 2],
                     v3 = s_sum[threadIdx.x * 5 + 3], v4 = s_sum[threadIdx.x * 5 + 4];
        g[0] = v0.x; g[1] = v0.y; g[2] = v0.z; g[3] = v0.w; g[4] = v1.x; g[5] = v1.y; g[6] = v1.z; g[7] = v1.w;
        g[8] = v2.x; g[9] = v2.y; g[10] = v2.z; g[11] = v2.w; g[12] = v3.x; g[13] = v3.y; g[14] = v3.z; g[15] = v3.w;
        g[16] = v4.x; g[17] = v4.y;
    } else if (!heavy) {
    if (CUT) {
        if (a.has_rec[i]) {
        RecWalk rw;
        rw.init(__float_as_uint(a.depths[i]), (uint32_t)i, __float_as_uint(r4.w), a.gx);
        uint32_t k = beg;
        for (; k + 1 < end; k += 2) {
            const bool h0 = rw.has_record(a.cut);
            rw.next();
            const bool h1 = rw.has_record(a.cut);
            rw.next();
            const float4* __restrict__ src = reinterpret_cast<const float4*>(a.grec + (size_t)k * GREC_F);
            const float4 zz = make_float4(0.f, 0.f, 0.f, 0.f);
            float4 v0 = zz, v1 = zz, v2 = zz, v3 = zz, v4 = zz, w0 = zz, w1 = zz, w2 = zz, w3 = zz, w4 = zz;
            if (h0) { v0 = src[0]; v1 = src[1]; v2 = src[2]; v3 = src[3]; v4 = src[4]; }
            if (h1) { w0 = src[5]; w1 = src[6]; w2 = src[7]; w3 = src[8]; w4 = src[9]; }
            if (h0) add_rec(v0, v1, v2, v3, v4);
            if (h1) add_rec(w0, w1, w2, w3, w4);
        }
        if (k < end && rw.has_record(a.cut)) {
            const float4* __restrict__ src = reinterpret_cast<const float4*>(a.grec + (size_t)k * GREC_F);
            const float4 v0 = src[0], v1 = src[1], v2 = src[2], v3 = src[3], v4 = src[4];
            add_rec(v0, v1, v2, v3, v4);
        }
        }
    } else {
        uint32_t k = beg;
        for (; k + 1 < end; k += 2) {
            const float4* __restrict__ src = reinterpret_cast<const float4*>(a.grec + (size_t)k * GREC_F);
            const float4 v0 = src[0], v1 = src[1], v2 = src[2], v3 = src[3], v4 = src[4];
            const float4 w0 = src[5], w1 = src[6], w2 = src[7], w3 = src[8], w4 = src[9];
            add_rec(v0, v1, v2, v3, v4);
            add_rec(w0, w1, w2, w3, w4);
        }
        if (k < end) {
            const float4* __restrict__ src = reinterpret_cast<const float4*>(a.grec + (size_t)k * GREC_F);
            const float4 v0 = src[0], v1 = src[1], v2 = src[2], v3 = src[3], v4 = src[4];
            add_rec(v0, v1, v2, v3, v4);
        }
    }
    }
    if (heavy) {
        g[0] = hs0.x; g[1] = hs0.y; g[2] = hs0.z; g[3] = hs0.w; g[4] = hs1.x; g[5] = hs1.y; g[6] = hs1.z; g[7] = hs1.w;
        g[8] = hs2.x; g[9] = hs2.y; g[10] = hs2.z; g[11] = hs2.w; g[12] = hs3.x; g[13] = hs3.y; g[14] = hs3.z; g[15] = hs3.w;
        g[16] = hs4.x; g[17] = hs4.y;
    }
    a.dL_dopacity[i] = g[14];
    if (a.dL_dnormal) store3(a.dL_dnormal, i, g[11], g[12], g[13]);
    if (!a.keep_colors) store3(a.dL_dcolors, i, g[15], g[16], g[17]);

    const float T[9] = {r0.x, r0.y, r0.z, r0.w, r1.x, r1.y, r1.z, r1.w, r2.x};
    float gT[9];
#pragma unroll
    for (int q = 0; q < 9; q++) gT[q] = g[q];
    const float gx2 = g[9], gy2 = g[10];
    if (gx2 != 0.f || gy2 != 0.f) {
        const float t[3] = {CUTOFF * CUTOFF, CUTOFF * CUTOFF, -1.f};
        const float d = t[0] * T[6] * T[6] + t[1] * T[7] * T[7] + t[2] * T[8] * T[8];
        const float id = 1.f / d;
        float f[3], dd = 0.f;
#pragma unroll
        for (int k = 0; k < 3; k++) {
            f[k] = t[k] * id;
            dd += (gx2 * T[k] * T[6 + k] + gy2 * T[3 + k] * T[6 + k]) * f[k];
        }
        dd *= -id;
#pragma unroll
        for (int k = 0; k < 3; k++) {
            gT[k] += gx2 * f[k] * T[6 + k];
            gT[3 + k] += gy2 * f[k] * T[6 + k];
            gT[6 + k] += gx2 * f[k] * T[k] + gy2 * f[k] * T[3 + k] + dd * t[k] * T[6 + k] * 2.f;
        }
    }
    const float px = a.means3D[3 * (size_t)i], py = a.means3D[3 * (size_t)i + 1], pz = a.means3D[3 * (size_t)i + 2];
    float dmx = 0.f, dmy = 0.f, dmz = 0.f;
    if (precomp) {
#pragma unroll
        for (int q = 0; q < 9; q++) a.dL_dtransMat[9 * (size_t)i + q] = gT[q];
        store3(a.dL_dmeans2D, i, gT[2] * T[8] * 0.5f * (float)a.W, gT[5] * T[8] * 0.5f * (float)a.H, 0.f);
    } else {
        if (a.dL_dtransMat) {
#pragma unroll
            for (int q = 0; q < 9; q++) a.dL_dtransMat[9 * (size_t)i + q] = g[q];
        }
        store3(a.dL_dmeans2D, i, g[2] * T[8] * 0.5f * (float)a.W, g[5] * T[8] * 0.5f * (float)a.H, 0.f);
        const float* __restrict__ vm = a.viewmatrix;
        float Pm[12];
        world2pix(a.projmatrix, a.W, a.H, Pm);
        const float4 q = reinterpret_cast<const float4*>(a.rotations)[i];
        const float2 sc = reinterpret_cast<const float2*>(a.scales)[i];
        const float s = rsqrtf(q.x * q.x + q.y * q.y + q.z * q.z + q.w * q.w);
        const float w = q.x * s, x = q.y * s, y = q.z * s, z = q.w * s;
        const float sx = a.scale_modifier * sc.x, sy = a.scale_modifier * sc.y;
        const float R00 = 1.f - 2.f * (y * y + z * z), R01 = 2.f * (x * y - w * z), R02 = 2.f * (x * z + w * y);
        const float R10 = 2.f * (x * y + w * z), R11 = 1.f - 2.f * (x * x + z * z), R12 = 2.f * (y * z - w * x);
        const float R20 = 2.f * (x * z - w * y), R21 = 2.f * (y * z + w * x), R22 = 1.f - 2.f * (x * x + y * y);
        float dA[3][3];
// ... 191 lines not shown
```

### 2d-gaussian-splatting_amd/csrc/surfel_sort.hip

```cpp
#include <hip/hip_runtime.h>
#include <stdint.h>

#include <cstring>
#include <rocprim/device/device_radix_sort.hpp>

#include "surfel_common.h"
#include "surfel_kernels.h"

namespace surfel {

constexpr size_t RS_ONESWEEP_MAX_ITEMS = (size_t)1 << 20;
constexpr size_t g_onesweep_max = RS_ONESWEEP_MAX_ITEMS;
int g_large_sort_impl = 2;
void set_large_sort_impl(int v) { g_large_sort_impl = v < 0 ? 0 : (v > 3 ? 2 : v); }
static inline bool use_rocprim(size_t n, int begin_bit, int end_bit) {
    if (begin_bit != 0) return false;
    if (g_large_sort_impl == 3) return true;
    if (n <= g_onesweep_max) return false;
    if (g_large_sort_impl != 2) return g_large_sort_impl == 1;
    return n > ((size_t)1 << 25);
}
static size_t rocprim_sort_temp_bytes(size_t n) {
    thread_local size_t last_n = 0, last_bytes = 0;
    if (n == last_n && last_bytes) return last_bytes;
    size_t bytes = 0;
    uint32_t* nul = nullptr;
    (void)rocprim::radix_sort_pairs(nullptr, bytes, nul, nul, nul, nul, n, 0u, 32u, (hipStream_t)0);
    last_n = n; last_bytes = bytes;
    return bytes;
}

constexpr int RS_THREADS = 256;
constexpr int RS_IPT = 8;
constexpr int RS_TILE = RS_THREADS * RS_IPT;
static inline bool rs_onesweep(size_t n) { return n <= g_onesweep_max; }
constexpr int RS_BITS = 8;
constexpr int RS_RADIX = 1 << RS_BITS;
constexpr int RS_MAX_PASSES = 4;
constexpr uint32_t ST_AGG = 1u << 30, ST_PREFIX = 2u << 30, ST_VALUE = (1u << 30) - 1u;

constexpr size_t RS_HEAD_WORDS = RS_MAX_PASSES * RS_RADIX + 64;

static inline uint32_t rs_nblocks(size_t n) { return (uint32_t)((n + RS_TILE - 1) / RS_TILE); }

size_t radix_sort_scratch_bytes(size_t n) {
    if (!rs_onesweep(n)) {
        const size_t own = ((size_t)RS_RADIX * rs_nblocks(n) + RS_RADIX) * sizeof(uint32_t) + 256;
        const size_t rp = rocprim_sort_temp_bytes(n) + 256;
        return own > rp ? own : rp;
    }
    const size_t own = (RS_HEAD_WORDS + (size_t)RS_MAX_PASSES * rs_nblocks(n) * RS_RADIX) * sizeof(uint32_t) + 256;
    const size_t rp = g_large_sort_impl == 3 ? rocprim_sort_temp_bytes(n) + 256 : 0;
    return own > rp ? own : rp;
}
int radix_sort_passes(size_t, int begin_bit, int end_bit) { return (end_bit - begin_bit + RS_BITS - 1) / RS_BITS; }
int radix_sort_result_buffer(size_t n, int begin_bit, int end_bit) {
    if (n == 0 || end_bit <= begin_bit) return 0;
    if (use_rocprim(n, begin_bit, end_bit)) return 1;
    return radix_sort_passes(n, begin_bit, end_bit) & 1;
}
size_t radix_sort_head_bytes() { return RS_HEAD_WORDS * sizeof(uint32_t); }

__device__ __forceinline__ uint32_t ld_agent(const uint32_t* p) { return __hip_atomic_load(p, __ATOMIC_RELAXED, __HIP_MEMORY_SCOPE_AGENT); }
__device__ __forceinline__ void st_agent(uint32_t* p, uint32_t v) { __hip_atomic_store(p, v, __ATOMIC_RELAXED, __HIP_MEMORY_SCOPE_AGENT); }

__global__ void __launch_bounds__(RS_THREADS) os_hist_kernel(const uint32_t* __restrict__ keys, uint32_t n, int begin_bit, int end_bit,
                                                             int passes, uint32_t* __restrict__ ghist, uint32_t* __restrict__ status,
                                                             uint32_t nblocks) {
    __shared__ uint32_t s_h[RS_MAX_PASSES][RS_RADIX];
    for (int p = 0; p < passes; p++) s_h[p][threadIdx.x] = 0;
    for (int p = 0; p < passes; p++) status[((size_t)p * nblocks + blockIdx.x) * RS_RADIX + threadIdx.x] = 0u;
    __syncthreads();
    const uint32_t base = blockIdx.x * (RS_THREADS * RS_IPT);
#pragma unroll
    for (int it = 0; it < RS_IPT; it++) {
        const uint32_t e = base + it * RS_THREADS + threadIdx.x;
        if (e < n) {
            const uint32_t k = keys[e];
            for (int p = 0; p < passes; p++) {
                const int bit = begin_bit + p * RS_BITS;
                const int nb = min(RS_BITS, end_bit - bit);
                atomicAdd(&s_h[p][(k >> bit) & ((1u << nb) - 1u)], 1u);
            }
        }
    }
    __syncthreads();
    for (int p = 0; p < passes; p++) {
        const uint32_t c = s_h[p][threadIdx.x];
        if (c) atomicAdd(&ghist[p * RS_RADIX + threadIdx.x], c);
    }
}

constexpr int FTH_THREADS = 1024;
template <int FTH_IPT>
__global__ void __launch_bounds__(FTH_THREADS) rs_hist_fat_kernel(const uint32_t* __restrict__ keys, uint32_t n, int shift, uint32_t mask,
                                                                  uint32_t* __restrict__ hist, uint32_t nblocks) {
    __shared__ uint32_t s_h[RS_RADIX];
    if (threadIdx.x < RS_RADIX) s_h[threadIdx.x] = 0;
    __syncthreads();
    const uint32_t base = blockIdx.x * (uint32_t)(FTH_THREADS * FTH_IPT);
#pragma unroll
    for (int it = 0; it < FTH_IPT; it++) {
        const uint32_t e = base + it * FTH_THREADS + threadIdx.x;
        if (e < n) atomicAdd(&s_h[(keys[e] >> shift) & mask], 1u);
    }
    __syncthreads();
    if (threadIdx.x < RS_RADIX) hist[(size_t)threadIdx.x * nblocks + blockIdx.x] = s_h[threadIdx.x];
}
__global__ void __launch_bounds__(RS_THREADS) rs_scan_kernel(uint32_t* __restrict__ hist, uint32_t nblocks, uint32_t* __restrict__ total) {
    __shared__ uint32_t s_w[4];
    __shared__ uint32_t s_carry;
    uint32_t* row = hist + (size_t)blockIdx.x * nblocks;
    if (threadIdx.x == 0) s_carry = 0;
    __syncthreads();
    const int lane = threadIdx.x & 63, wave = threadIdx.x >> 6;
    for (uint32_t c0 = 0; c0 < nblocks; c0 += RS_THREADS) {
        const uint32_t i = c0 + threadIdx.x;
        const uint32_t v = i < nblocks ? row[i] : 0u;
        uint32_t x = v;
#pragma unroll
        for (int o = 1; o < 64; o <<= 1) { const uint32_t y = __shfl_up(x, o); if (lane >= o) x += y; }
        if (lane == 63) s_w[wave] = x;
        __syncthreads();
        uint32_t woff = 0;
        for (int w = 0; w < wave; w++) woff += s_w[w];
        const uint32_t carry = s_carry;
        if (i < nblocks) row[i] = carry + woff + x - v;
        __syncthreads();
        if (threadIdx.x == RS_THREADS - 1) s_carry = carry + woff + x;
        __syncthreads();
    }
    if (threadIdx.x == 0) total[blockIdx.x] = s_carry;
}

constexpr int FT_THREADS = 1024, FT_IPT = 4, FT_TILE = FT_THREADS * FT_IPT, FT_WAVES = FT_THREADS / 64;
constexpr int FT_LB = 32;
static inline uint32_t ft_nblocks(size_t n) { return (uint32_t)((n + FT_TILE - 1) / FT_TILE); }

template <bool LOOKBACK, int IPT>
__global__ void __launch_bounds__(FT_THREADS) os_pass_fat_kernel(const uint32_t* __restrict__ keys, const uint32_t* __restrict__ vals,
                                                                 uint32_t* __restrict__ keys_out, uint32_t* __restrict__ vals_out, uint32_t n,
                                                                 int shift, uint32_t mask, const uint32_t* __restrict__ ghist,
                                                                 uint32_t* __restrict__ status, uint32_t* __restrict__ ticket,
                                                                 const uint32_t* __restrict__ n_dev, int hstride, uint2* __restrict__ ranges,
                                                                 uint32_t nblocks) {
    __shared__ uint32_t s_cnt[FT_WAVES][RS_RADIX];
    constexpr int TILE_ITEMS = FT_THREADS * IPT;
    __shared__ uint2 s_item[TILE_ITEMS];
    __shared__ uint32_t s_gbase[RS_RADIX];
    __shared__ uint32_t s_w[4][2];
    __shared__ uint32_t s_tile;
    const int lane = threadIdx.x & 63, wave = threadIdx.x >> 6;
    const uint32_t d_t = threadIdx.x;
    if (LOOKBACK && threadIdx.x == 0) s_tile = atomicAdd(ticket, 1u);
    for (int i = threadIdx.x; i < FT_WAVES * RS_RADIX; i += FT_THREADS) (&s_cnt[0][0])[i] = 0u;
    __syncthreads();
    const uint32_t tile = LOOKBACK ? s_tile : blockIdx.x;
    if (n_dev) n = min(n, *n_dev);
    if (tile * (uint32_t)TILE_ITEMS >= n) return;
    const uint32_t wbase = tile * (uint32_t)TILE_ITEMS + wave * (64 * IPT);
    uint32_t k[IPT], v[IPT], rank[IPT];
#pragma unroll
    for (int it = 0; it < IPT; it++) {
        const uint32_t e = wbase + it * 64 + lane;
        const bool valid = e < n;
        k[it] = valid ? keys[e] : 0xffffffffu;
        v[it] = valid ? vals[e] : 0u;
    }
#pragma unroll
    for (int it = 0; it < IPT; it++) {
        const uint32_t e = wbase + it * 64 + lane;
        const bool valid = e < n;
        const uint32_t d = (k[it] >> shift) & mask;
        unsigned long long mm = __ballot(valid);
#pragma unroll
        for (int b = 0; b < RS_BITS; b++) {
            const bool bit = (d >> b) & 1u;
            const unsigned long long bal = __ballot(bit);
            mm &= bit ? bal : ~bal;
        }
        if (!valid) mm = 0ull;
        const uint32_t below = __builtin_amdgcn_mbcnt_hi((uint32_t)(mm >> 32), __builtin_amdgcn_mbcnt_lo((uint32_t)mm, 0u));
        const uint32_t prev = valid ? s_cnt[wave][d] : 0u;
        rank[it] = prev + below;
        if (valid && below == 0) s_cnt[wave][d] = prev + (uint32_t)__popcll(mm);
    }
    __syncthreads();
    uint32_t cw[FT_WAVES], cnt = 0, excl = 0, tot = 0, x = 0, y = 0;
    if (threadIdx.x < RS_RADIX) {
#pragma unroll
        for (int w = 0; w < FT_WAVES; w++) { cw[w] = s_cnt[w][d_t]; cnt += cw[w]; }
        uint32_t* my = status + (size_t)tile * RS_RADIX + d_t;
        if (!LOOKBACK) {
            excl = status[(size_t)d_t * nblocks + tile];
        } else if (tile == 0) {
            st_agent(my, cnt | ST_PREFIX);
        } else {
            st_agent(my, cnt | ST_AGG);
            int p = (int)tile - 1;
            bool done = false;
            while (!done) {
                uint32_t w[FT_LB];
#pragma unroll
                for (int i = 0; i < FT_LB; i++) w[i] = (p - i >= 0) ? ld_agent(status + (size_t)(p - i) * RS_RADIX + d_t) : ST_PREFIX;
                int used = 0;
#pragma unroll
                for (int i = 0; i < FT_LB; i++) {
                    if (!done && used == i) {
                        if ((w[i] >> 30) != 0u) {
                            excl += w[i] & ST_VALUE;
                            used = i + 1;
                            if (w[i] & ST_PREFIX) done = true;
                        }
                    }
                }
                p -= used;
                if (!done && used == 0) __builtin_amdgcn_s_sleep(1);
            }
            st_agent(my, (excl + cnt) | ST_PREFIX);
        }
        tot = ghist[(size_t)d_t * hstride];
        x = tot; y = cnt;
#pragma unroll
        for (int o = 1; o < 64; o <<= 1) {
            const uint32_t xa = __shfl_up(x, o), ya = __shfl_up(y, o);
            if (lane >= o) { x += xa; y += ya; }
        }
        if (lane == 63) { s_w[wave][0] = x; s_w[wave][1] = y; }
    }
    __syncthreads();
    if (threadIdx.x < RS_RADIX) {
        uint32_t goff = x - tot + excl, loff = y - cnt;
        for (int w = 0; w < wave; w++) { goff += s_w[w][0]; loff += s_w[w][1]; }
        s_gbase[d_t] = goff - loff;
        uint32_t run = loff;
#pragma unroll
        for (int w = 0; w < FT_WAVES; w++) { s_cnt[w][d_t] = run; run += cw[w]; }
    }
    __syncthreads();
#pragma unroll
    for (int it = 0; it < IPT; it++) {
        const uint32_t e = wbase + it * 64 + lane;
        if (e < n) {
            const uint32_t d = (k[it] >> shift) & mask;
            s_item[s_cnt[wave][d] + rank[it]] = make_uint2(k[it], v[it]);
        }
    }
    __syncthreads();
    const uint32_t items = min((uint32_t)TILE_ITEMS, n - tile * (uint32_t)TILE_ITEMS);
#pragma unroll
    for (int it = 0; it < IPT; it++) {
        const uint32_t q = (uint32_t)it * FT_THREADS + threadIdx.x;
        if (q < items) {
            const uint2 kv = s_item[q];
            const uint32_t dst = s_gbase[(kv.x >> shift) & mask] + q;
            keys_out[dst] = kv.x;
            vals_out[dst] = kv.y;
            if (ranges) {
                const bool first = q == 0u || s_item[q - 1].x != kv.x;
                const bool last = q + 1u == items || s_item[q + 1].x != kv.x;
                if (first) atomicMax(&ranges[kv.x].x, ~dst);
                if (last) atomicMax(&ranges[kv.x].y, dst + 1u);
            }
        }
    }
}

size_t radix_sort_head_words(size_t n) { return rs_onesweep(n) ? RS_HEAD_WORDS : 0; }

constexpr int SC_IPT = 8, SC_TILE = RS_THREADS * SC_IPT;
size_t scan_scratch_words(size_t n) { return 64 + (n + SC_TILE - 1) / SC_TILE; }

__global__ void __launch_bounds__(RS_THREADS) scan_gather_kernel(const uint32_t* __restrict__ vals, const uint32_t* __restrict__ order, int packed,
                                                                 uint32_t* __restrict__ out, uint32_t n, uint32_t* __restrict__ scratch) {
    __shared__ uint32_t s_w[4];
    __shared__ uint32_t s_tile, s_excl;
    uint32_t* ticket = scratch;
    uint32_t* status = scratch + 64;
    const int lane = threadIdx.x & 63, wave = threadIdx.x >> 6;
    if (threadIdx.x == 0) s_tile = atomicAdd(ticket, 1u);
    __syncthreads();
    const uint32_t tile = s_tile;
    const uint32_t base = tile * SC_TILE + threadIdx.x * SC_IPT;
    uint32_t v[SC_IPT], sum = 0;
#pragma unroll
    for (int i = 0; i < SC_IPT; i++) {
        const uint32_t e = base + i;
        uint32_t t = 0u;
        if (e < n) {
            const uint32_t ov = order[e];
            if (packed) { t = ov >> PACK_ID_BITS; if (t == PACK_TILES_MAX) t = vals[ov & ((1u << PACK_ID_BITS) - 1u)]; }
            else t = vals[ov];
        }
        v[i] = t;
        sum += v[i];
    }
    uint32_t x = sum;
#pragma unroll
    for (int o = 1; o < 64; o <<= 1) { const uint32_t y = __shfl_up(x, o); if (lane >= o) x += y; }
    if (lane == 63) s_w[wave] = x;
    __syncthreads();
    uint32_t woff = 0;
    for (int w = 0; w < wave; w++) woff += s_w[w];
    const uint32_t agg = s_w[0] + s_w[1] + s_w[2] + s_w[3];
    if (wave == 0) {
        uint32_t excl = 0;
        if (tile == 0) {
            if (lane == 0) st_agent(status, agg | ST_PREFIX);
        } else {
            if (lane == 0) st_agent(status + tile, agg | ST_AGG);
            int p = (int)tile - 1;
            for (;;) {
                const int idx = p - lane;
                const uint32_t sw = idx >= 0 ? ld_agent(status + idx) : ST_PREFIX;
                const unsigned long long ready = __ballot((sw >> 30) != 0u);
                const unsigned long long pref = __ballot((sw & ST_PREFIX) != 0u);
                const int nready = ready == ~0ull ? 64 : __builtin_ctzll(~ready);
                const int firstp = pref ? __builtin_ctzll(pref) : 64;
                const int take = min(nready, firstp + 1);
                uint32_t c = lane < take ? (sw & ST_VALUE) : 0u;
#pragma unroll
                for (int o = 32; o > 0; o >>= 1) c += __shfl_xor(c, o);
                excl += c;
                if (firstp < nready) break;
                p -= take;
                if (take == 0) __builtin_amdgcn_s_sleep(1);
            }
            if (lane == 0) st_agent(status + tile, (excl + agg) | ST_PREFIX);
        }
        if (lane == 0) s_excl = excl;
    }
    __syncthreads();
    uint32_t run = s_excl + woff + x - sum;
#pragma unroll
    for (int i = 0; i < SC_IPT; i++) {
        run += v[i];
        if (base + i < n) out[base + i] = run;
    }
}

void launch_scan_gather(const uint32_t* vals, const uint32_t* order, int packed, uint32_t* out, size_t n, void* zeroed_scratch, hipStream_t s) {
    if (n == 0) return;
    hipLaunchKernelGGL(scan_gather_kernel, dim3((unsigned)((n + SC_TILE - 1) / SC_TILE)), dim3(RS_THREADS), 0, s, vals, order, packed, out, (uint32_t)n,
                       static_cast<uint32_t*>(zeroed_scratch));
}


template <int E>
__device__ __forceinline__ void tile_sort_regs(uint32_t n, uint32_t* __restrict__ pl, const uint32_t* __restrict__ depth_keys,
                                               unsigned long long* __restrict__ s, uint32_t tid) {
    unsigned long long v[E];
#pragma unroll
    for (int e = 0; e < E; e++) {
        const uint32_t idx = (uint32_t)e * RS_THREADS + tid;
        v[e] = ~0ull;
        if (idx < n) { const uint32_t id = pl[idx]; v[e] = ((unsigned long long)depth_keys[id] << 32) | id; }
    }
#pragma unroll
    for (uint32_t k = 2; k <= (uint32_t)RS_THREADS * E; k <<= 1) {
#pragma unroll
        for (uint32_t j = k >> 1; j > 0; j >>= 1) {
            if (j >= (uint32_t)RS_THREADS) {
#pragma unroll
                for (int e = 0; e < E; e++) {
                    const int e2 = e | (int)(j / RS_THREADS);
                    if ((e & (int)(j / RS_THREADS)) == 0 && e2 < E) {
                        const bool up = ((((uint32_t)e * RS_THREADS + tid) & k) == 0u);
                        const unsigned long long a = v[e], b = v[e2];
                        if ((a > b) == up) { v[e] = b; v[e2] = a; }
                    }
                }
            } else {
                unsigned long long pv[E];
                if (j >= 64u) {
#pragma unroll
                    for (int e = 0; e < E; e++) s[e * RS_THREADS + tid] = v[e];
                    __syncthreads();
#pragma unroll
                    for (int e = 0; e < E; e++) pv[e] = s[e * RS_THREADS + (tid ^ j)];
                    __syncthreads();
                } else {
#pragma unroll
                    for (int e = 0; e < E; e++) pv[e] = __shfl_xor(v[e], (int)j, 64);
                }
#pragma unroll
                for (int e = 0; e < E; e++) {
                    const uint32_t idx = (uint32_t)e * RS_THREADS + tid;
                    const bool take_min = ((idx & j) == 0u) == ((idx & k) == 0u);
                    v[e] = ((pv[e] < v[e]) == take_min) ? pv[e] : v[e];
                }
            }
        }
    }
#pragma unroll
    for (int e = 0; e < E; e++) {
        const uint32_t idx = (uint32_t)e * RS_THREADS + tid;
        if (idx < n) pl[idx] = (uint32_t)v[e];
    }
}

constexpr int TR_WAVES = RS_THREADS / 64;
constexpr int TR_BITONIC_MAX = 8 * RS_THREADS;
constexpr int TR_RADIX_MIN = 2 * RS_THREADS;
constexpr int TR_CHUNK_IPT = 8;
int g_tile_radix_min = TR_RADIX_MIN;
void set_tile_radix_min(int v) { g_tile_radix_min = v < 0 ? TR_RADIX_MIN : (v > TR_BITONIC_MAX ? TR_BITONIC_MAX : v); }

__device__ __forceinline__ uint32_t tr_rank(uint32_t d, bool valid, uint32_t* cnt_row) {
    unsigned long long mm = __ballot(valid);
#pragma unroll
    for (int b = 0; b < RS_BITS; b++) {
        const bool bit = (d >> b) & 1u;
        const unsigned long long bal = __ballot(bit);
        mm &= bit ? bal : ~bal;
    }
    if (!valid) mm = 0ull;
    const uint32_t below = __builtin_amdgcn_mbcnt_hi((uint32_t)(mm >> 32), __builtin_amdgcn_mbcnt_lo((uint32_t)mm, 0u));
    const uint32_t prev = valid ? cnt_row[d] : 0u;
    if (valid && below == 0) cnt_row[d] = prev + (uint32_t)__popcll(mm);
    return prev + below;
}

__device__ __forceinline__ uint32_t tr_key_spread(uint32_t o, uint32_t a, uint32_t* s_w, int lane, int wave) {
#pragma unroll
    for (int off = 32; off > 0; off >>= 1) { o |= __shfl_xor(o, off); a &= __shfl_xor(a, off); }
    if (lane == 0) { s_w[wave] = o; s_w[TR_WAVES + wave] = a; }
    __syncthreads();
    o = 0u; a = ~0u;
#pragma unroll
    for (int w = 0; w < TR_WAVES; w++) { o |= s_w[w]; a &= s_w[TR_WAVES + w]; }
    return o ^ a;
}

__device__ __forceinline__ uint32_t tr_digit_scan(uint32_t cnt, uint32_t* s_w, int lane, int wave) {
    uint32_t x = cnt;
#pragma unroll
    for (int o = 1; o < 64; o <<= 1) { const uint32_t y = __shfl_up(x, o); if (lane >= o) x += y; }
    if (lane == 63) s_w[wave] = x;
    __syncthreads();
    uint32_t excl = x - cnt;
    for (int w = 0; w < wave; w++) excl += s_w[w];
    return excl;
}

template <int IPT>
__device__ __forceinline__ void tile_radix_lds(uint32_t n, uint32_t* __restrict__ pl, const uint32_t* __restrict__ depth_keys,
                                               uint32_t (*s_cnt)[RS_RADIX], uint2* s_item, uint32_t* s_w, uint32_t tid) {
    const int lane = tid & 63, wave = tid >> 6;
    const uint32_t ipt = (n + RS_THREADS - 1) / RS_THREADS;
    const uint32_t wbase = (uint32_t)wave * 64u * ipt;
    uint32_t k[IPT], v[IPT], rank[IPT];
    uint32_t o = 0u, a = ~0u;
#pragma unroll
    for (int it = 0; it < IPT; it++) {
        const uint32_t idx = wbase + (uint32_t)it * 64u + lane;
        const bool ok = (uint32_t)it < ipt && idx < n;
        const uint32_t id = pl[ok ? idx : 0u], key = depth_keys[id];
        v[it] = id; k[it] = ok ? key : 0xffffffffu; rank[it] = 0u;
        o |= ok ? key : 0u; a &= ok ? key : 0xffffffffu;
    }
    for (int j = lane; j < RS_RADIX; j += 64) s_cnt[wave][j] = 0u;
    const uint32_t diff = tr_key_spread(o, a, s_w, lane, wave);
    if (diff == 0u) return;
#pragma unroll 1
    for (int shift = 0; shift < 32; shift += RS_BITS) {
        if (((diff >> shift) & (RS_RADIX - 1u)) == 0u) continue;
#pragma unroll
        for (int it = 0; it < IPT; it++) {
            uint32_t r = 0u;
            if ((uint32_t)it < ipt) r = tr_rank((k[it] >> shift) & (RS_RADIX - 1u), true, s_cnt[wave]);
            rank[it] = r;
            __builtin_amdgcn_sched_barrier(0);
        }
        __syncthreads();
        uint32_t cw[TR_WAVES], cnt = 0;
#pragma unroll
        for (int w = 0; w < TR_WAVES; w++) { cw[w] = s_cnt[w][tid]; cnt += cw[w]; }
        uint32_t run = tr_digit_scan(cnt, s_w + 2 * TR_WAVES, lane, wave);
#pragma unroll
        for (int w = 0; w < TR_WAVES; w++) { s_cnt[w][tid] = run; run += cw[w]; }
        __syncthreads();
#pragma unroll
        for (int it = 0; it < IPT; it++) {
            if ((uint32_t)it < ipt) s_item[s_cnt[wave][(k[it] >> shift) & (RS_RADIX - 1u)] + rank[it]] = make_uint2(k[it], v[it]);
        }
        for (int j = lane; j < RS_RADIX; j += 64) s_cnt[wave][j] = 0u;
        __syncthreads();
#pragma unroll
        for (int it = 0; it < IPT; it++) {
            const uint32_t idx = wbase + (uint32_t)it * 64u + lane;
            const uint2 kv = s_item[(uint32_t)it < ipt ? idx : 0u];
            k[it] = kv.x; v[it] = kv.y;
        }
    }
#pragma unroll
    for (int it = 0; it < IPT; it++) {
        const uint32_t idx = wbase + (uint32_t)it * 64u + lane;
        if ((uint32_t)it < ipt && idx < n) pl[idx] = v[it];
    }
}

__device__ __forceinline__ void tile_radix_chunked(uint32_t n, uint32_t* pl, const uint32_t* __restrict__ depth_keys, uint32_t* ak,
                                                   uint32_t* bk, uint32_t* bv, uint32_t (*s_cnt)[RS_RADIX], uint32_t (*s_hist)[RS_RADIX],
                                                   uint32_t* s_base, uint32_t* s_w, uint32_t tid) {
    const int lane = tid & 63, wave = tid >> 6;
    for (int p = 0; p < RS_MAX_PASSES; p++) s_hist[p][tid] = 0u;
    for (int j = lane; j < RS_RADIX; j += 64) s_cnt[wave][j] = 0u;
    __syncthreads();
    uint32_t o = 0u, a = ~0u;
    for (uint32_t i = tid; i < n; i += RS_THREADS) {
        const uint32_t key = depth_keys[pl[i]];
        ak[i] = key; o |= key; a &= key;
#pragma unroll
        for (int p = 0; p < RS_MAX_PASSES; p++) atomicAdd(&s_hist[p][(key >> (p * RS_BITS)) & (RS_RADIX - 1u)], 1u);
    }
    const uint32_t diff = tr_key_spread(o, a, s_w, lane, wave);
    if (diff == 0u) return;
    uint32_t *sk = ak, *sv = pl, *dk = bk, *dv = bv;
#pragma unroll 1
    for (int p = 0; p < RS_MAX_PASSES; p++) {
        const int shift = p * RS_BITS;
        if (((diff >> shift) & (RS_RADIX - 1u)) == 0u) continue;
        s_base[tid] = tr_digit_scan(s_hist[p][tid], s_w + 2 * TR_WAVES, lane, wave);
        __syncthreads();
        for (uint32_t c0 = 0; c0 < n; c0 += (uint32_t)(RS_THREADS * TR_CHUNK_IPT)) {
            const uint32_t wbase = c0 + (uint32_t)wave * (64u * TR_CHUNK_IPT);
            uint32_t k[TR_CHUNK_IPT], v[TR_CHUNK_IPT], rank[TR_CHUNK_IPT];
#pragma unroll
            for (int it = 0; it < TR_CHUNK_IPT; it++) {
                const uint32_t idx = wbase + (uint32_t)it * 64u + lane;
                k[it] = idx < n ? sk[idx] : 0xffffffffu;
                v[it] = idx < n ? sv[idx] : 0u;
            }
#pragma unroll
            for (int it = 0; it < TR_CHUNK_IPT; it++) {
                rank[it] = tr_rank((k[it] >> shift) & (RS_RADIX - 1u), wbase + (uint32_t)it * 64u + lane < n, s_cnt[wave]);
                __builtin_amdgcn_sched_barrier(0);
            }
            __syncthreads();
            uint32_t run = s_base[tid];
#pragma unroll
            for (int w = 0; w < TR_WAVES; w++) { const uint32_t c = s_cnt[w][tid]; s_cnt[w][tid] = run; run += c; }
            s_base[tid] = run;
            __syncthreads();
#pragma unroll
            for (int it = 0; it < TR_CHUNK_IPT; it++) {
                if (wbase + (uint32_t)it * 64u + lane < n) {
                    const uint32_t dst = s_cnt[wave][(k[it] >> shift) & (RS_RADIX - 1u)] + rank[it];
                    if (dst < n) { dk[dst] = k[it]; dv[dst] = v[it]; }
                }
            }
            for (int j = lane; j < RS_RADIX; j += 64) s_cnt[wave][j] = 0u;
        }
        __syncthreads();
        uint32_t* t = sk; sk = dk; dk = t;
        t = sv; sv = dv; dv = t;
    }
    if (sv != pl) for (uint32_t i = tid; i < n; i += RS_THREADS) pl[i] = sv[i];
}

template <int TS_CAP>
__global__ void __launch_bounds__(RS_THREADS) tile_depth_sort_kernel(uint2* __restrict__ ranges, uint32_t* __restrict__ point_list,
                                                                    const uint32_t* __restrict__ depth_keys, uint32_t* __restrict__ tmp_ids,
                                                                    uint32_t* __restrict__ tmp_keys, uint32_t* __restrict__ tmp_rank, int decode,
                                                                    uint32_t radix_min) {
    static_assert(TS_CAP % RS_THREADS == 0 && TS_CAP * 8 + 4 * TR_WAVES * RS_RADIX >= TR_BITONIC_MAX * 8, "LDS layout");
    __shared__ unsigned long long s_raw[TS_CAP + TR_WAVES * RS_RADIX / 2];
    __shared__ uint32_t s_w[3 * TR_WAVES];
    unsigned long long* s = s_raw;
    uint32_t (*s_cnt)[RS_RADIX] = reinterpret_cast<uint32_t (*)[RS_RADIX]>(s_raw);
    uint2* s_item = reinterpret_cast<uint2*>(s_raw + TR_WAVES * RS_RADIX / 2);
    uint2 rg = ranges[blockIdx.x];
    if (decode) {
        rg.x = __builtin_amdgcn_readfirstlane(rg.x); rg.y = __builtin_amdgcn_readfirstlane(rg.y);
        __syncthreads();
        if (rg.y != 0u) {
            rg.x = ~rg.x;
            if (threadIdx.x == 0) ranges[blockIdx.x].x = rg.x;
        }
    }
    const uint32_t n = rg.y - rg.x;
    if (n < 2u) return;
    uint32_t* __restrict__ pl = point_list + rg.x;
    const uint32_t tid = threadIdx.x;
    if (n <= radix_min) {
        if (n <= (uint32_t)RS_THREADS) { tile_sort_regs<1>(n, pl, depth_keys, s, tid); return; }
        if (n <= 2u * RS_THREADS) { tile_sort_regs<2>(n, pl, depth_keys, s, tid); return; }
        if (n <= 4u * RS_THREADS) { tile_sort_regs<4>(n, pl, depth_keys, s, tid); return; }
        tile_sort_regs<8>(n, pl, depth_keys, s, tid);
        return;
    }
    if (n <= 4u * RS_THREADS) { tile_radix_lds<4>(n, pl, depth_keys, s_cnt, s_item, s_w, tid); return; }
    constexpr int MID = TS_CAP < 8 * RS_THREADS ? TS_CAP : 8 * RS_THREADS;
    if (n <= (uint32_t)MID) { tile_radix_lds<MID / RS_THREADS>(n, pl, depth_keys, s_cnt, s_item, s_w, tid); return; }
    if constexpr (TS_CAP > MID) {
        if (n <= (uint32_t)TS_CAP) { tile_radix_lds<TS_CAP / RS_THREADS>(n, pl, depth_keys, s_cnt, s_item, s_w, tid); return; }
    }
    tile_radix_chunked(n, pl, depth_keys, tmp_keys + rg.x, tmp_rank + rg.x, tmp_ids + rg.x, s_cnt, reinterpret_cast<uint32_t (*)[RS_RADIX]>(s_item),
                       reinterpret_cast<uint32_t*>(s_item) + RS_MAX_PASSES * RS_RADIX, s_w, tid);
}

constexpr int TS_CAP_SMALL = 1536, TS_CAP_LARGE = 4096;
constexpr int TS_SMALL_MAX_AVG = 256;
int tile_depth_sort_classes(int* out, int cap) {
    const int v[6] = {g_tile_radix_min, TS_CAP_SMALL, TS_CAP_LARGE, TS_SMALL_MAX_AVG, 4 * RS_THREADS, 8 * RS_THREADS};
    for (int i = 0; i < 6 && i < cap; i++) out[i] = v[i];
    return 6;
}

void launch_tile_depth_sort(int ntiles, int64_t R, uint2* ranges, uint32_t* point_list, const uint32_t* depth_keys, uint32_t* tmp_ids,
                            uint32_t* tmp_keys, uint32_t* tmp_rank, bool decode, hipStream_t st) {
    if (ntiles <= 0) return;
    if (R <= (int64_t)TS_SMALL_MAX_AVG * ntiles)
        hipLaunchKernelGGL(tile_depth_sort_kernel<TS_CAP_SMALL>, dim3(ntiles), dim3(RS_THREADS), 0, st, ranges, point_list, depth_keys, tmp_ids,
                           tmp_keys, tmp_rank, decode ? 1 : 0, (uint32_t)g_tile_radix_min);
    else
        hipLaunchKernelGGL(tile_depth_sort_kernel<TS_CAP_LARGE>, dim3(ntiles), dim3(RS_THREADS), 0, st, ranges, point_list, depth_keys, tmp_ids,
                           tmp_keys, tmp_rank, decode ? 1 : 0, (uint32_t)g_tile_radix_min);
}

int radix_sort_pairs_u32(uint32_t* keys_a, uint32_t* vals_a, uint32_t* keys_b, uint32_t* vals_b, size_t n, int begin_bit, int end_bit,
                         void* scratch, hipStream_t s, bool head_zeroed) {
    if (n == 0 || end_bit <= begin_bit) return 0;
    if (n >= ST_VALUE) return -1;
    const uint32_t nblocks = rs_nblocks(n);
    const int passes = radix_sort_passes(n, begin_bit, end_bit);
    if (passes > RS_MAX_PASSES) return -1;
    int cur = 0;
    if (use_rocprim(n, begin_bit, end_bit)) {
        size_t bytes = rocprim_sort_temp_bytes(n);
        if (rocprim::radix_sort_pairs(scratch, bytes, keys_a, keys_b, vals_a, vals_b, n, (unsigned)begin_bit, (unsigned)end_bit, s) != hipSuccess) return -1;
        return 1;
    }
    if (!rs_onesweep(n)) {
        uint32_t* hist = static_cast<uint32_t*>(scratch);
        uint32_t* total = hist + (size_t)RS_RADIX * nblocks;
        for (int p = 0; p < passes; p++) {
            const int bit = begin_bit + p * RS_BITS;
            const int nb = end_bit - bit < RS_BITS ? end_bit - bit : RS_BITS;
            const uint32_t mask = (1u << nb) - 1u;
            const uint32_t* kin = cur ? keys_b : keys_a; const uint32_t* vin = cur ? vals_b : vals_a;
            uint32_t* kout = cur ? keys_a : keys_b; uint32_t* vout = cur ? vals_a : vals_b;
            const uint32_t fb = ft_nblocks(n);
            hipLaunchKernelGGL(rs_hist_fat_kernel<FT_IPT>, dim3(fb), dim3(FTH_THREADS), 0, s, kin, (uint32_t)n, bit, mask, hist, fb);
            hipLaunchKernelGGL(rs_scan_kernel, dim3(RS_RADIX), dim3(RS_THREADS), 0, s, hist, fb, total);
            hipLaunchKernelGGL((os_pass_fat_kernel<false, FT_IPT>), dim3(fb), dim3(FT_THREADS), 0, s, kin, vin, kout, vout, (uint32_t)n, bit, mask, total, hist,
                               (uint32_t*)nullptr, (const uint32_t*)nullptr, 1, (uint2*)nullptr, fb);
            cur ^= 1;
        }
        return cur;
    }
    uint32_t* ghist = static_cast<uint32_t*>(scratch);
    uint32_t* ticket = ghist + RS_MAX_PASSES * RS_RADIX;
    uint32_t* status = ghist + RS_HEAD_WORDS;
    if (!head_zeroed) (void)hipMemsetAsync(scratch, 0, RS_HEAD_WORDS * sizeof(uint32_t), s);
    hipLaunchKernelGGL(os_hist_kernel, dim3(nblocks), dim3(RS_THREADS), 0, s, keys_a, (uint32_t)n, begin_bit, end_bit, passes, ghist, status, nblocks);
    for (int p = 0; p < passes; p++) {
        const int bit = begin_bit + p * RS_BITS;
        const int nb = end_bit - bit < RS_BITS ? end_bit - bit : RS_BITS;
        const uint32_t mask = (1u << nb) - 1u;
        const uint32_t* kin = cur ? keys_b : keys_a; const uint32_t* vin = cur ? vals_b : vals_a;
        uint32_t* kout = cur ? keys_a : keys_b; uint32_t* vout = cur ? vals_a : vals_b;
        hipLaunchKernelGGL((os_pass_fat_kernel<true, FT_IPT>), dim3(ft_nblocks(n)), dim3(FT_THREADS), 0, s, kin, vin, kout, vout, (uint32_t)n, bit, mask,
                           ghist + p * RS_RADIX, status + (size_t)p * nblocks * RS_RADIX, ticket + p, (const uint32_t*)nullptr, 1, (uint2*)nullptr, 0u);
        cur ^= 1;
    }
    return cur;
}

constexpr int BE_HSTRIDE = 32;
size_t bin_emit_head_words() { return (size_t)RS_MAX_PASSES * RS_RADIX * BE_HSTRIDE + 64; }

constexpr int BE_THREADS = 1024;
__global__ void __launch_bounds__(BE_THREADS) bin_emit_kernel(int P, const uint32_t* __restrict__ tiles_touched, const uint32_t* __restrict__ rects,
                                                              const uint32_t* __restrict__ block_totals, uint32_t nblock_totals, float* __restrict__ rec,
                                                              uint32_t* __restrict__ keys, uint32_t* __restrict__ vals, int gx, uint32_t cap,
                                                              uint32_t* __restrict__ ghist, uint32_t* __restrict__ sort_status,
                                                              uint32_t sort_status_words, int passes, int end_bit, uint32_t* __restrict__ n_out,
                                                              uint32_t* __restrict__ n_host) {
    constexpr int NW = BE_THREADS / 64;
    __shared__ uint32_t s_w[NW], s_p[NW];
    __shared__ uint32_t s_h[2][RS_RADIX];
    const int lane = threadIdx.x & 63, wave = threadIdx.x >> 6;
    const uint32_t k = blockIdx.x * BE_THREADS + threadIdx.x;
    if (threadIdx.x < 2 * RS_RADIX) s_h[threadIdx.x >> 8][threadIdx.x & (RS_RADIX - 1)] = 0u;
    for (uint32_t w = k; w < sort_status_words; w += gridDim.x * BE_THREADS) sort_status[w] = 0u;
    auto sat = [](uint32_t a, uint32_t b) { const uint32_t c = a + b; return c < a ? 0xffffffffu : c; };
    uint32_t pre = 0;
    const uint32_t ahead = min(nblock_totals, blockIdx.x * (uint32_t)(BE_THREADS / 256));
    for (uint32_t j = threadIdx.x; j < ahead; j += BE_THREADS) pre = sat(pre, block_totals[j]);
    const uint32_t n = k < (uint32_t)P ? tiles_touched[k] : 0u;
    uint32_t x = n;
#pragma unroll
    for (int o = 1; o < 64; o <<= 1) { const uint32_t y = __shfl_up(x, o); if (lane >= o) x = sat(x, y); }
#pragma unroll
    for (int o = 32; o > 0; o >>= 1) pre = sat(pre, __shfl_xor(pre, o));
    if (lane == 63) s_w[wave] = x;
    if (lane == 0) s_p[wave] = pre;
    __syncthreads();
    uint32_t off = x - n;
#pragma unroll
    for (int w = 0; w < NW; w++) off = sat(off, sat(s_p[w], w < wave ? s_w[w] : 0u));
    if (k == (uint32_t)P - 1u) {
        n_out[0] = sat(off, n);
        if (n_host) n_host[0] = sat(off, n);
    }
    const uint32_t mask0 = (1u << min(RS_BITS, end_bit)) - 1u;
    const uint32_t mask1 = passes > 1 ? (1u << min(RS_BITS, end_bit - RS_BITS)) - 1u : 0u;
    if (n) {
        const uint32_t rectbits = rects[k];
        rec[(size_t)k * REC_F + 18] = __uint_as_float(off);
        const int x0 = rectbits & 1023, y0 = (rectbits >> 10) & 1023, w = rectbits >> 20;
        int xx = 0, yy = 0;
        for (uint32_t t = 0; t < n; t++) {
            const uint32_t key = (uint32_t)((y0 + yy) * gx + (x0 + xx));
            if (off < cap && t < cap - off) {
                keys[off + t] = key; vals[off + t] = k;
                atomicAdd(&s_h[0][key & mask0], 1u);
                if (passes > 1) atomicAdd(&s_h[1][(key >> RS_BITS) & mask1], 1u);
            }
            if (++xx == w) { xx = 0; ++yy; }
        }
    }
    __syncthreads();
    if ((int)threadIdx.x < passes * RS_RADIX) {
        const uint32_t c = s_h[threadIdx.x >> 8][threadIdx.x & (RS_RADIX - 1)];
        if (c) atomicAdd(&ghist[(size_t)threadIdx.x * BE_HSTRIDE], c);
    }
}

int radix_sort_pairs_u32_devn(uint32_t* keys_a, uint32_t* vals_a, uint32_t* keys_b, uint32_t* vals_b, size_t cap, int end_bit, const uint32_t* n_dev,
                              void* scratch, uint2* ranges, hipStream_t s) {
    const uint32_t nblocks = rs_nblocks(cap);
    const int passes = radix_sort_passes(cap, 0, end_bit);
    uint32_t* ghist = static_cast<uint32_t*>(scratch);
    uint32_t* ticket = ghist + (size_t)RS_MAX_PASSES * RS_RADIX * BE_HSTRIDE;
    uint32_t* status = ghist + bin_emit_head_words();
    int cur = 0;
    for (int p = 0; p < passes; p++) {
        const int bit = p * RS_BITS;
        const int nb = end_bit - bit < RS_BITS ? end_bit - bit : RS_BITS;
        const uint32_t mask = (1u << nb) - 1u;
        const uint32_t* kin = cur ? keys_b : keys_a; const uint32_t* vin = cur ? vals_b : vals_a;
        uint32_t* kout = cur ? keys_a : keys_b; uint32_t* vout = cur ? vals_a : vals_b;
        hipLaunchKernelGGL((os_pass_fat_kernel<true, FT_IPT>), dim3(ft_nblocks(cap)), dim3(FT_THREADS), 0, s, kin, vin, kout, vout, (uint32_t)cap, bit, mask,
                           ghist + (size_t)p * RS_RADIX * BE_HSTRIDE, status + (size_t)p * nblocks * RS_RADIX, ticket + p, n_dev, BE_HSTRIDE,
                           p == passes - 1 ? ranges : (uint2*)nullptr, 0u);
        cur ^= 1;
    }
    return cur;
}
bool capacity_binning_ok(size_t cap, int end_bit) { return rs_onesweep(cap) && radix_sort_passes(cap, 0, end_bit) <= 2 && g_large_sort_impl != 3; }
size_t bin_emit_sort_status_words(size_t cap, int end_bit) { return (size_t)radix_sort_passes(cap, 0, end_bit) * rs_nblocks(cap) * RS_RADIX; }
size_t capacity_sort_scratch_bytes(size_t cap, int end_bit) { return (bin_emit_head_words() + bin_emit_sort_status_words(cap, end_bit)) * sizeof(uint32_t) + 256; }

void launch_bin_emit(int P, const uint32_t* tiles_touched, const uint32_t* rects, const uint32_t* block_totals, float* rec, uint32_t* keys, uint32_t* vals,
                     int gx, size_t cap, void* sort_scratch, int end_bit, uint32_t* n_out, uint32_t* n_host, hipStream_t s) {
    uint32_t* ghist = static_cast<uint32_t*>(sort_scratch);
    hipLaunchKernelGGL(bin_emit_kernel, dim3((unsigned)((P + BE_THREADS - 1) / BE_THREADS)), dim3(BE_THREADS), 0, s, P, tiles_touched, rects, block_totals,
                       (uint32_t)((P + 255) / 256), rec, keys, vals, gx, (uint32_t)cap, ghist, ghist + bin_emit_head_words(), (uint32_t)bin_emit_sort_status_words(cap, end_bit),
                       radix_sort_passes(cap, 0, end_bit), end_bit, n_out, n_host);
}

}
```

### 2d-gaussian-splatting_amd/surfel_native.py

```python
import ctypes as C
import math
import os
import threading

import torch

_HERE = os.path.dirname(os.path.abspath(__file__))
LIB_PATH = os.environ.get("SURFEL_LIB") or os.path.join(_HERE, "lib", "libsurfel_hip.so")

ALLOC_FN = C.CFUNCTYPE(C.c_void_p, C.c_void_p, C.c_size_t)
HOOK_FN = C.CFUNCTYPE(None, C.c_void_p)


class DevPtr:

    @classmethod
    def from_param(cls, v):
        if isinstance(v, torch.Tensor):
            if not v.is_cuda:
                raise RuntimeError("libsurfel_hip: tensors must live on a HIP device (got %s)" % v.device)
            return C.c_void_p(v.data_ptr())
        return None if v is None else C.c_void_p.from_param(v)


class Stream:
    from_param = C.c_void_p.from_param


class TsdfVolume(C.Structure):
    _fields_ = [("origin", C.c_int * 3), ("dims", C.c_int * 3), ("voxel_size", C.c_float), ("sdf_trunc", C.c_float), ("budget_bytes", C.c_int64),
                ("table", C.c_void_p), ("scratch", C.c_void_p), ("nblocks", C.c_int64), ("keys", C.c_void_p), ("stamp", C.c_void_p),
                ("list", C.c_void_p), ("tsdf_rgb", C.c_void_p), ("weight", C.c_void_p), ("info", C.c_void_p), ("vbase", C.c_void_p),
                ("tbase", C.c_void_p), ("pool_scratch", C.c_void_p), ("views", C.c_int64), ("nverts", C.c_int64), ("ntris", C.c_int64)]


class UnboundedVolume(C.Structure):
    _fields_ = [("M", C.c_int), ("slab", C.c_int), ("R", C.c_float), ("center", C.c_float * 3), ("radius", C.c_float), ("voxel_size", C.c_float),
                ("budget_bytes", C.c_int64), ("tsdf", C.c_void_p), ("info", C.c_void_p), ("vbase", C.c_void_p), ("tbase", C.c_void_p),
                ("scan_scratch", C.c_void_p), ("slab_base", C.c_void_p), ("nslabs", C.c_int64), ("nverts", C.c_int64), ("ntris", C.c_int64)]


class UnboundedView(C.Structure):
    _fields_ = [("proj", C.c_float * 12), ("H", C.c_int32), ("W", C.c_int32), ("offset", C.c_int64)]


class EvalGrid(C.Structure):
    _fields_ = [("origin", C.c_float * 3), ("cell", C.c_float), ("dims", C.c_int * 3), ("budget_bytes", C.c_int64), ("n", C.c_int64),
                ("sorted", C.c_void_p), ("order", C.c_void_p), ("ranges", C.c_void_p)]


class JpegDecDesc(C.Structure):
    _fields_ = [("width", C.c_int32), ("height", C.c_int32), ("ncomp", C.c_int32), ("hs", C.c_int32), ("vs", C.c_int32),
                ("restart_interval", C.c_int32), ("ecs_offset", C.c_int64), ("ecs_bytes", C.c_int64),
                ("tq", C.c_uint8 * 4), ("td", C.c_uint8 * 4), ("ta", C.c_uint8 * 4), ("qt", (C.c_uint16 * 64) * 4),
                ("bits", (C.c_uint8 * 16) * 4), ("huffval", (C.c_uint8 * 256) * 4)]


class RepairPlan(C.Structure):
    _fields_ = [(k, C.c_int64) for k in ("V", "F", "max_hole_edges", "survivors", "split", "border", "loops", "fill_triangles", "fill_vertices")] + \
               [(k, C.c_void_p) for k in ("triangles", "triangle_source", "split_source", "half_edge", "loop", "position", "lengths", "fill_vertex",
                                          "fill_offset", "triangle_offset", "centroid_offset")]


_i, _i64, _f, _f64, _d, _s, _u, _a = C.c_int, C.c_int64, C.c_float, C.c_double, DevPtr, Stream, C.c_void_p, ALLOC_FN
_fp, _ip, _i64p, _f64p = C.POINTER(C.c_float), C.POINTER(C.c_int), C.POINTER(C.c_int64), C.POINTER(C.c_double)
_vol, _uvol, _grid, _jdesc = C.POINTER(TsdfVolume), C.POINTER(UnboundedVolume), C.POINTER(EvalGrid), C.POINTER(JpegDecDesc)
_rplan = C.POINTER(RepairPlan)
_adam = (_i, _d, _d, _d, _d, _d, _fp, _f, _f, _f, _i, _f, _i, _i, _d, _d)
SIGNATURES = {
    "surfel_hip.h": {
        "surfel_abi_version": (_i,),
        "surfel_last_error": (C.c_char_p,),
        "surfel_rasterize_forward": (_i64, _a, _u, _a, _u, _a, _u, _i, _i, _i, _d, _i, _i, _d, _d, _d, _d, _d, _f, _d, _d, _d, _d, _d, _f, _f, _i,
                                     _d, _d, _d, _i, _s),
        "surfel_rasterize_backward": (_i, _a, _u, _i, _i, _i, _i64, _d, _i, _i, _d, _d, _d, _d, _f, _d, _d, _d, _d, _d, _f, _f, _d, _d, _d, _d,
                                      _d, _d, _d, _d, _d, _d, _d, _d, _d, _d, _d, _i, _s),
        "surfel_mark_visible": (_i, _i, _d, _d, _d, _d, _s),
        "surfel_knn_dist2": (_i, _a, _u, _i, _d, _d, _s),
        "surfel_set_option": (_i, C.c_char_p, _i),
        "surfel_set_backward_hook": (_i, HOOK_FN, _u),
        "surfel_forward_count": (_i64,),
    },
    "surfel_debug.h": {
        "surfel_last_stage_ms": (_i, _fp, _i),
        "surfel_last_stage_ids": (_i, _ip, _i),
        "surfel_collect_stage_ms": (_i, _fp, _ip, _i),
        "surfel_stage_name": (C.c_char_p, _i),
        "surfel_debug_sort_pairs": (_i, _a, _u, _d, _d, _i64, _i, _i, _s),
        "surfel_debug_tile_depth_sort": (_i, _i, _i64, _d, _d, _d, _d, _i, _s),
        "surfel_debug_tile_depth_sort_classes": (_i, _ip, _i),
        "surfel_debug_set_tile_radix_min": (_i, _i),
        "surfel_debug_set_blend_stats": (_i, _d),
        "surfel_debug_last_binning": (_i,),
        "surfel_debug_capacity_evictions": (_i,),
        "surfel_debug_image_layout": (_i, _i, _i, _i64p),
        "surfel_debug_box_probe": (_i, _d, _i64, _fp, _s),
        "surfel_debug_latency_probe": (_i, _d, _i64, _i, _fp, _s),
    },
    "surfel_train.h": {
        "surfel_l1_ssim_forward": (_i, _i, _i, _i, _d, _d, _d, _d, _s),
        "surfel_l1_ssim_backward": (_i, _i, _i, _i, _d, _d, _d, _f, _f, _d, _d, _d, _s),
        "surfel_l1_ssim_forward_w": (_i, _i, _i, _i, _i, _d, _d, _d, _d, _s),
        "surfel_l1_ssim_backward_w": (_i, _i, _i, _i, _i, _d, _d, _d, _f, _f, _d, _d, _d, _s),
        "surfel_render_post_forward": (_i, _i, _i, _d, _d, _f, _d, _d, _s),
        "surfel_render_post_backward": (_i, _i, _i, _d, _d, _f, _d, _f, _f, _d, _d, _s),
        "surfel_train_loss_forward": (_i, _i, _i, _d, _d, _d, _d, _d, _d, _f, _d, _s),
        "surfel_train_loss_backward": (_i, _i, _i, _d, _d, _d, _f, _f, _d, _d, _f, _f, _f, _d, _d, _d, _d, _d, _f, _f, _f, _d, _d, _s),
        "surfel_reduce_partials": (_i, _d, _i, _i, _i, _f, _d, _s),
        "surfel_loss_finalize": (_i, _d, _i, _i, _d, _i, _i, _f, _f, _f, _d, _d, _s),
        "surfel_activate": (_i, _i, _d, _d, _s),
        "surfel_adam_step": (_i,) + _adam + (_i, _s),
        "surfel_train_update": (_i,) + _adam + (_d, _d, _d, _d, _d, _s),
        "surfel_sh_grad_gather": (_i, _i, _i, _i, _d, _d, _d, _d, _s),
        "surfel_densify_stats": (_i, _i, _d, _d, _d, _d, _d, _s),
    },
    "surfel_mesh.h": {
        "surfel_tsdf_table_bytes": (_i64, _vol),
        "surfel_tsdf_block_bytes": (_i64,),
        "surfel_mesh_prepare_view": (_i, _i, _i, _d, _d, _d, _f, _d, _d, _s),
        "surfel_tsdf_init": (_i, _vol, _a, _u, _s),
        "surfel_tsdf_mark": (_i, _vol, _i, _i, _d, _d, _s),
        "surfel_tsdf_allocate": (_i64, _vol, _a, _u, _s),
        "surfel_tsdf_integrate": (_i, _vol, _i, _i, _d, _d, _d, _s),
        "surfel_tsdf_count": (_i, _vol, _s),
        "surfel_tsdf_extract": (_i, _vol, _d, _d, _d, _s),
        "surfel_mesh_clusters": (_i, _a, _u, _i64, _i64, _d, _d, _d, _s),
        "surfel_mesh_filter": (_i, _a, _u, _i64, _i64, _d, _d, _d, _d, _d, _i, _d, _d, _d, _i64p, _s),
    },
    "surfel_mesh_unbounded.h": {
        "surfel_unbounded_bytes": (_i64, _uvol),
        "surfel_unbounded_init": (_i, _uvol, _a, _u, _s),
        "surfel_unbounded_fuse": (_i, _uvol, _i, _d, _d, _d, _s),
        "surfel_unbounded_count": (_i, _uvol, _s),
        "surfel_unbounded_extract": (_i, _uvol, _d, _d, _s),
        "surfel_unbounded_color": (_i, _i64, _d, _i, _d, _d, _d, _f, _d, _s),
    },
    "surfel_eval.h": {
        "surfel_eval_sample_count": (_i64, _a, _u, _i64, _i64, _d, _d, _f64, _i64, _d, _s),
        "surfel_eval_sample_emit": (_i, _i64, _i64, _d, _d, _f64, _d, _i64, _d, _s),
        "surfel_eval_grid_build": (_i, _a, _u, _grid, _i64, _d, _d, _s),
        "surfel_eval_thin": (_i, _a, _u, _grid, _f, _d, _ip, _s),
        "surfel_eval_obs_mask": (_i, _i64, _d, _fp, _f, _f64, _d, _ip, _d, _d, _s),
        "surfel_eval_above_plane": (_i, _i64, _d, _f64p, _d, _s),
        "surfel_eval_nearest": (_i, _a, _u, _grid, _i64, _d, _f, _d, _d, _s),
        "surfel_eval_mean_below": (_i, _a, _u, _i64, _d, _f, _d, _s),
        "surfel_eval_dilate_masks": (_i, _a, _u, _i, _i, _i, _d, _i, _d, _s),
        "surfel_eval_cull_vertices": (_i, _i64, _d, _i, _d, _i, _i, _d, _d, _s),
    },
    "surfel_eval_tnt.h": {
        "surfel_tnt_mesh_cloud": (_i, _i64, _i64, _d, _d, _d, _s),
        "surfel_tnt_transform": (_i, _i64, _d, _f64p, _d, _s),
        "surfel_tnt_crop": (_i, _i64, _d, _i, _f64, _f64, _i, _d, _d, _s),
        "surfel_tnt_voxel_down_sample": (_i64, _a, _u, _i64, _d, _f64, _f64p, _i64, _d, _d, _d, _s),
        "surfel_tnt_corr_sums": (_i, _a, _u, _i64, _d, _d, _i64, _d, _d, _s),
        "surfel_tnt_histogram": (_i, _i64, _d, _i, _d, _f64, _d, _s),
    },
    "surfel_metrics.h": {
        "surfel_lpips_workspace_bytes": (_i64, _i, _i, _i64),
        "surfel_lpips_prepare": (_i, _i, _i, _d, _d, _d, _s),
        "surfel_lpips_conv3x3": (_i, _i, _i, _i, _i, _d, _d, _d, _d, _s),
        "surfel_lpips_pool": (_i, _i, _i, _i, _d, _d, _s),
        "surfel_lpips_tap": (_i, _i, _i, _i, _d, _d, _d, _s),
        "surfel_sq_err_partials": (_i, _i64, _d, _d, _d, _s),
    },
    "surfel_scene.h": {
        "surfel_scene_resample_table": (_i, _i, _i, _ip, _ip, _i64),
        "surfel_scene_resample_h": (_i, _i, _i, _i, _i, _i, _d, _d, _d, _d, _d, _d, _s),
        "surfel_scene_resample_v": (_i, _i, _i, _i, _i, _i, _d, _d, _d, _d, _d, _d, _s),
        "surfel_scene_to_float": (_i, _i, _i, _i, _d, _d, _d, _s),
        "surfel_scene_composite": (_i, _i, _i, _i, _d, _d, _s),
    },
    "surfel_vis.h": {
        "surfel_vis_quantize": (_i, _i, _i, _i, _d, _f, _f, _d, _s),
        "surfel_vis_order_stats": (_i, _i64, _d, _i, _i64p, _d, _d, _i64, _s),
        "surfel_vis_depth_turbo": (_i, _i, _i, _d, _f64, _f64, _d, _s),
    },
    "surfel_view.h": {
        "surfel_view_scalar": (_i, _i, _i, _d, _d, _d, _i64, _s),
        "surfel_view_gradient": (_i, _i, _i, _d, _f, _f, _d, _d, _i64, _s),
    },
    "surfel_cull.h": {
        "surfel_cull_mesh_depth": (_i64, _a, _u, _i64, _i64, _d, _d, _i, _d, _d, _i, _i, _i, _f, _f, _i, _d, _fp, _s),
        "surfel_cull_visibility": (_i, _i64, _d, _i, _d, _d, _i, _i, _i, _d, _f, _d, _s),
    },
    "surfel_meshview.h": {
        "surfel_meshview_visibility": (_i64, _a, _u, _i64, _i64, _d, _d, _i, _d, _d, _i, _i, _i, _f, _f, _i, _d, _fp, _s),
        "surfel_meshview_vertex_normals": (_i, _i64, _i64, _d, _d, _d, _d, _s),
        "surfel_meshview_shade": (_i, _i64, _i64, _d, _d, _d, _d, _i, _d, _d, _i, _i, _i, _i, _d, _i, _f, _f, _f, _d, _s),
    },
    "surfel_simplify.h": {
        "surfel_simplify_bounds": (_i, _a, _u, _i64, _d, _fp, _s),
        "surfel_simplify_clusters": (_i64, _a, _u, _i64, _d, _fp, _fp, _f, _d, _s),
        "surfel_simplify_count": (_i64, _a, _u, _i64, _i64, _d, _d, _fp, _fp, _f, _i64p, _s),
        "surfel_simplify_mesh": (_i, _a, _u, _i64, _i64, _d, _d, _d, _fp, _fp, _f, _f64, _d, _d, _d, _d, _d, _i64p, _fp, _s),
    },
    "surfel_texture.h": {
        "surfel_texture_classify": (_i, _a, _u, _i64, _i64, _d, _d, _f, _d, _i64p, _s),
        "surfel_texture_layout": (_i64, _a, _u, _i64, _i64, _d, _d, _d, _i64p, _i, _ip, _d, _d, _s),
        "surfel_texture_bake": (_i, _i64, _i64, _d, _d, _ip, _d, _i, _i, _i, _d, _d, _i, _i, _i, _d, _d, _f, _f, _i, _i, _d, _s),
        "surfel_texture_resolve": (_i, _i64, _i64, _d, _d, _d, _ip, _d, _i, _i, _d, _i, _f, _f, _f, _d, _d, _s),
        "surfel_texture_shade": (_i, _i64, _i64, _d, _d, _d, _d, _i, _i, _i, _d, _d, _i, _i, _i, _i, _d, _f, _f, _f, _d, _s),
    },
    "surfel_smooth.h": {
        "surfel_smooth_adjacency": (_i64, _a, _u, _i64, _i64, _d, _d, _d, _d, _d, _d, _i64p, _s),
        "surfel_smooth_steps": (_i, _i64, _d, _d, _d, _d, _i, _i, _f64p, _d, _d, _d, _s),
    },
    "surfel_repair.h": {
        "surfel_repair_analyze": (_i, _a, _u, _i64, _i64, _d, _d, _i64, _rplan, _i64p, _fp, _s),
        "surfel_repair_emit": (_i, _rplan, _d, _d, _d, _d, _d, _d, _d, _d, _s),
        "surfel_repair_loops": (_i, _rplan, _d, _d, _d, _d, _s),
    },
    "surfel_jpeg.h": {
        "surfel_jpeg_capacity": (_i64, _i, _i),
        "surfel_jpeg_scratch_bytes": (_i64, _i, _i),
        "surfel_jpeg_encode": (_i, _i, _i, _d, _i, _d, _i64, _d, _d, _i64, _s),
    },
    "surfel_png.h": {
        "surfel_png_capacity": (_i64, _i, _i, _i),
        "surfel_png_scratch_bytes": (_i64, _i, _i, _i),
        "surfel_png_encode": (_i, _i, _i, _i, _d, _d, _i64, _d, _d, _i64, _s),
    },
    "surfel_jpegdec.h": {
        "surfel_jpegdec_scratch_bytes": (_i64, _jdesc, _i),
        "surfel_jpegdec_decode": (_i, _jdesc, _d, _i64, _d, _d, _i64, _i, _i, _i, _d, _s),
    },
    "surfel_undistort.h": {
        "surfel_scene_undistort": (_i, _i, _i, _i, _i, _i, _f64p, _f64p, _d, _d, _s),
    },
    "surfel_log.h": {
        "surfel_log_append": (_i, _d, _d, _i, _i, _i, _d, _f, _f, _s),
        "surfel_log_panel": (_i, _i, _i, _i, _d, _d, _d, _i64, _s),
        "surfel_log_crc32c": (C.c_uint32, _u, _i64),
        "surfel_log_frame": (_i64, _u, _i64, _u),
        "surfel_log_steps_capacity": (_i64, _i64),
        "surfel_log_encode_steps": (_i64, _u, _i64, _f, _f64, _u, _i64),
    },
}
EXPORTS = [name for h in ("surfel_hip.h", "surfel_debug.h", "surfel_train.h") for name in SIGNATURES[h]]
MESH_EXPORTS = list(SIGNATURES["surfel_mesh.h"])
UNBOUNDED_EXPORTS = list(SIGNATURES["surfel_mesh_unbounded.h"])
EVAL_EXPORTS = list(SIGNATURES["surfel_eval.h"])
TNT_EXPORTS = list(SIGNATURES["surfel_eval_tnt.h"])
METRICS_EXPORTS = list(SIGNATURES["surfel_metrics.h"])
SCENE_EXPORTS = list(SIGNATURES["surfel_scene.h"])
VIS_EXPORTS = list(SIGNATURES["surfel_vis.h"])
VIEW_EXPORTS = list(SIGNATURES["surfel_view.h"])
CULL_EXPORTS = list(SIGNATURES["surfel_cull.h"])
MESHVIEW_EXPORTS = list(SIGNATURES["surfel_meshview.h"])
SIMPLIFY_EXPORTS = list(SIGNATURES["surfel_simplify.h"])
TEXTURE_EXPORTS = list(SIGNATURES["surfel_texture.h"])
SMOOTH_EXPORTS = list(SIGNATURES["surfel_smooth.h"])
REPAIR_EXPORTS = list(SIGNATURES["surfel_repair.h"])
JPEG_EXPORTS = list(SIGNATURES["surfel_jpeg.h"])
PNG_EXPORTS = list(SIGNATURES["surfel_png.h"])
JPEGDEC_EXPORTS = list(SIGNATURES["surfel_jpegdec.h"])
UNDISTORT_EXPORTS = list(SIGNATURES["surfel_undistort.h"])
LOG_EXPORTS = list(SIGNATURES["surfel_log.h"])
_SIG = {name: sig for group in SIGNATURES.values() for name, sig in group.items()}


E_LIMIT = -4
E_OVERFLOW = -5
OPT_NO_CULL = 1 << 8
OPT_BWD_QUAD = 1 << 11
OPT_BWD_ROWS = 1 << 12
OPT_PBWD_COOP = 1 << 13
OPT_PBWD_THREAD = 1 << 14
OPT_BWD_SCAN = 1 << 15
OPT_EXACT_BINNING = 1 << 16
OPT_TILE_CUTS = 1 << 17
OPT_ZERO_RECORDS = 1 << 18
OPT_LAZY_COUNT = 1 << 21
OPT_BWD_GATHER = 1 << 22
OPT_NO_STREAM = 1 << 23
OPT_PBWD_NO_JAC = 1 << 24


def opt_tile_order(mode):
    return ((int(mode) + 1) & 3) << 19


def opt_tile_sort(mode):
    return ((mode + 1) & 3) << 9


_lib = None
_lock = threading.Lock()


def load():
    global _lib
    if _lib is not None:
        return _lib
    with _lock:
        if _lib is not None:
            return _lib
        if not os.path.exists(LIB_PATH):
            raise ImportError(
                "libsurfel_hip.so not found at %s — build it with `python 2d-gaussian-splatting_amd/build.py` "
                "(hipcc --offload-arch=gfx950). There is no CPU / PyTorch fallback for the rasterizer." % LIB_PATH)
        lib = C.CDLL(LIB_PATH)
        for name, (restype, *argtypes) in _SIG.items():
            fn = getattr(lib, name)
            fn.restype, fn.argtypes = restype, argtypes
        if lib.surfel_abi_version() != 1:
            raise ImportError("libsurfel_hip.so ABI version mismatch")
        for kv in filter(None, os.environ.get("SURFEL_OPTIONS", "").split(",")):
            name, _, value = kv.partition("=")
            if lib.surfel_set_option(name.strip().encode(), int(value)) != 0:
                raise ValueError("SURFEL_OPTIONS: unknown option %r" % name)
        _lib = lib
    return _lib


class LimitError(RuntimeError):
    """SURFEL_E_LIMIT: a size exceeds an internal limit or the caller's byte budget (raise the budget or coarsen the input)."""


class CapacityOverflow(RuntimeError):
    """a lazily counted frame held more tile instances than its capacity: render it again (OPT_EXACT_BINNING)"""


_ERRORS = {E_LIMIT: LimitError, E_OVERFLOW: CapacityOverflow}
_STREAMED = frozenset(name for name, sig in _SIG.items() if sig[-1] is Stream)


def call(device, name, *args):
    fn = getattr(load(), name)
    if name in _STREAMED:
        args += (None if device is None else current_stream_ptr(device),)
    try:
        if device is None:
            rc = fn(*args)
        else:
            with torch.cuda.device(device):
                rc = fn(*args)
    except C.ArgumentError as e:
        raise RuntimeError("%s: %s" % (name, e)) from None
    if rc < 0:
        raise _ERRORS.get(rc, RuntimeError)("%s failed (%d): %s" % (name, rc, last_error()))
    return rc


_hook_keepalive = None


def set_backward_hook(fn):
    global _hook_keepalive
    thunk = HOOK_FN() if fn is None else HOOK_FN(lambda user: fn())
    call(None, "surfel_set_backward_hook", thunk, None)
    _hook_keepalive = None if fn is None else thunk


def forward_count():
    return int(call(None, "surfel_forward_count"))


def last_error():
    return load().surfel_last_error().decode()


def bucket_bytes(n):
    n = int(n)
    if n < (1 << 26):
        return max(n, 1)
    step = 1 << (n.bit_length() - 4)
    return (n + step - 1) // step * step


class TorchAllocator:

    def __init__(self, device):
        held = []

        def _alloc(user, nbytes):
            try:
                t = torch.empty(bucket_bytes(nbytes), dtype=torch.uint8, device=device)
            except Exception:
                return None
            held.append(t)
            return t.data_ptr()

        self.device = device
        self.held = held
        self.cb = ALLOC_FN(_alloc)

    def last(self):
        return self.held[-1]

    def view(self, pointer, dtype, shape):
        for t in self.held:
            if t.data_ptr() == pointer:
                return t[:math.prod(shape) * dtype.itemsize].view(dtype).view(*shape)
        raise KeyError(pointer)


def ptr(t):
    return None if t is None else C.c_void_p(t.data_ptr())


def device_tensor(who, t, what=None):
    if not torch.is_tensor(t) or not t.is_cuda:
        got = t.device if torch.is_tensor(t) else type(t).__name__
        raise RuntimeError("%s: tensors must live on a HIP device (%sgot %s)" % (who, "" if what is None else what + ": ", got))
    return t


def uint8_buffer(who, t, n, device, what="out", at_least=False):
    if t is None:
        return torch.empty(n, dtype=torch.uint8, device=device)
    if t.dtype != torch.uint8 or not t.is_contiguous() or ((t.dim() != 1 or t.numel() < n) if at_least else t.numel() != n):
        raise ValueError("%s: %s must be a contiguous uint8 tensor of %s%d elements" % (who, what, "at least " if at_least else "", n))
    return t


def file_bytes(buf, size):
    return buf[:int(size.item())].cpu().numpy().tobytes()


def rows(who, t, what, dtype, shape="[N, 3]"):
    t = device_tensor(who, t, what)
    if t.ndim != 2 or t.shape[1] != 3:
        raise ValueError("%s: %s must be %s, got %s" % (who, what, shape, list(t.shape)))
    return t.detach().to(dtype).contiguous()


def counts_dict(names, carray):
    return {k: int(v) for k, v in zip(names, carray)}


_raw_stream = getattr(torch._C, "_cuda_getCurrentRawStream", None)


def current_stream_ptr(device):
    if _raw_stream is not None and device.index is not None:
        return C.c_void_p(_raw_stream(device.index))
    return C.c_void_p(torch.cuda.current_stream(device).cuda_stream)


class ManualCtx:
    manual = True
    needs_input_grad = ()

    def save_for_backward(self, *tensors):
        self.saved_tensors = tensors

    def mark_non_differentiable(self, *tensors):
        pass

    def set_materialize_grads(self, value):
        pass


def stage_times():
    lib = load()
    ms = (C.c_float * 16)()
    ids = (C.c_int * 16)()
    n = lib.surfel_last_stage_ms(ms, 16)
    lib.surfel_last_stage_ids(ids, 16)
    return [(lib.surfel_stage_name(ids[k]).decode(), float(ms[k])) for k in range(n)]


def collect_stage_times():
    lib = load()
    ms = (C.c_float * 16)()
    cnt = (C.c_int * 16)()
    n = lib.surfel_collect_stage_ms(ms, cnt, 16)
    return {lib.surfel_stage_name(k).decode(): (float(ms[k]), int(cnt[k])) for k in range(n) if cnt[k] > 0}
```

### include/surfel_debug.h

```cpp
#ifndef SURFEL_DEBUG_H
#define SURFEL_DEBUG_H

#include "surfel_hip.h"

#ifdef __cplusplus
extern "C" {
#endif

int surfel_last_stage_ms(float* ms, int cap);
int surfel_last_stage_ids(int* ids, int cap);
int surfel_collect_stage_ms(float* sum_ms, int* count, int cap);
const char* surfel_stage_name(int stage);

int surfel_debug_sort_pairs(surfel_alloc_fn scratch_alloc, void* scratch_user, uint32_t* keys, uint32_t* vals, int64_t n,
                            int begin_bit, int end_bit, void* stream);

int surfel_debug_tile_depth_sort(int ntiles, int64_t n, uint32_t* ranges, uint32_t* point_list, const uint32_t* depth_keys, uint32_t* scratch,
                                 int decode, void* stream);
int surfel_debug_tile_depth_sort_classes(int* out, int cap);
int surfel_debug_set_tile_radix_min(int longest_network_run);

int surfel_debug_set_blend_stats(void* dev_u64x8);

int surfel_debug_last_binning(void);
int surfel_debug_capacity_evictions(void);
int surfel_debug_image_layout(int width, int height, int64_t* out);

int surfel_debug_box_probe(void* scratch, int64_t scratch_bytes, float* out9, void* stream);
int surfel_debug_latency_probe(void* buf, int64_t bytes, int hops, float* ns_per_hop, void* stream);

#ifdef __cplusplus
}
#endif
#endif
```

Measured before the change: 320.4 train-iters/s.

## Fuse tile-order planning into tile depth sort and fuse ranges into exact-binning sort

Tile-order map construction moves into a shared device header so it can run inside the per-tile depth sort kernel instead of a separate launch before blending. The decision is planned on the host up front. The exact-binning path now also uses the radix sort's fused tile-range output, with a decode kernel when no depth sort runs. The aim is fewer kernel launches and fewer passes over the ranges, at the cost of more complex kernels and new debug entry points.

Result: no change. 321.1 train-iters/s (median of 2 runs) (+0.2%).

```diff
diff --git a/2d-gaussian-splatting_amd/build.py b/2d-gaussian-splatting_amd/build.py
--- a/2d-gaussian-splatting_amd/build.py
+++ b/2d-gaussian-splatting_amd/build.py
@@ -25,7 +25,7 @@
          "mesh_texture.hip": ["-ffp-contract=off"],
          "mesh_smooth.hip": ["-ffp-contract=off"],
          "mesh_repair.hip": ["-ffp-contract=off"]}
-HEADERS = ["surfel_common.h", "surfel_kernels.h", "surfel_blend_bwd.h", "train_kernels.h", "train_loss_body.h", "train_post_body.h", os.path.join("..", "..", "include", "surfel_hip.h"), os.path.join("..", "..", "include", "surfel_debug.h"),
+HEADERS = ["surfel_common.h", "surfel_kernels.h", "surfel_blend_bwd.h", "surfel_tile_order.h", "train_kernels.h", "train_loss_body.h", "train_post_body.h", os.path.join("..", "..", "include", "surfel_hip.h"), os.path.join("..", "..", "include", "surfel_debug.h"),
            os.path.join("..", "..", "include", "surfel_train.h"), "mesh_mc_table.h", "mesh_mc.h", "block_ops.h", "side_util.h", "carve.h", "mesh_topology.h", os.path.join("..", "..", "include", "surfel_mesh.h"),
            os.path.join("..", "..", "include", "surfel_mesh_unbounded.h"), os.path.join("..", "..", "include", "surfel_eval.h"),
            os.path.join("..", "..", "include", "surfel_eval_tnt.h"), os.path.join("..", "..", "include", "surfel_metrics.h"),
diff --git a/2d-gaussian-splatting_amd/csrc/surfel_api.hip b/2d-gaussian-splatting_amd/csrc/surfel_api.hip
--- a/2d-gaussian-splatting_amd/csrc/surfel_api.hip
+++ b/2d-gaussian-splatting_amd/csrc/surfel_api.hip
@@ -9,6 +9,7 @@
 #include "carve.h"
 #include "surfel_common.h"
 #include "surfel_kernels.h"
+#include "surfel_tile_order.h"
 #include "train_kernels.h"
 
 using namespace surfel;
@@ -250,8 +251,8 @@
     maxR = R > maxR - maxR / 64 ? R : maxR - maxR / 64;
 }
 
-void run_tile_order(CapEntry* ce, const uint2* ranges, int gx, int gy, int* map, uint32_t* map_flag, int opt, hipStream_t s) {
-    if (opt == 1) return;
+bool plan_tile_order(CapEntry* ce, int gx, int gy, int* map, uint32_t* map_flag, int opt, TileOrderArgs* to) {
+    if (opt == 1) return false;
     uint32_t* hv = pinned_u32();
     uint32_t* verdict = nullptr;
     if (hv && opt == 0) {
@@ -260,9 +261,10 @@
         else if (v == 2u) ce->uniform_streak = 0;
         void* dv = nullptr;
         if (hipHostGetDevicePointer(&dv, hv + R_SLOTS + ce->slot(), 0) == hipSuccess) verdict = static_cast<uint32_t*>(dv);
-        if (verdict && ce->uniform_streak >= 4 && (ce->frames & 7u) != 0u) return;
-    }
-    launch_tile_order(ranges, gx, gy, map, map_flag, opt, verdict, s);
+        if (verdict && ce->uniform_streak >= 4 && (ce->frames & 7u) != 0u) return false;
+    }
+    *to = TileOrderArgs{0, gx, gy, map, tile_map_len(gx, gy), map_flag, opt, verdict};
+    return true;
 }
 
 int higher_msb(uint32_t n) {
@@ -288,7 +290,7 @@
 }
 
 int bin_capacity(const PreprocessArgs& pa, int end_bit, int64_t cap, int64_t maxR, const GeomState& geom, const BinState& bin,
-                 const ImgState& img, uint32_t* hR, hipEvent_t evR, StageTimer& tm, hipStream_t s) {
+                 const ImgState& img, uint32_t* hR, hipEvent_t evR, const TileOrderArgs* order, StageTimer& tm, hipStream_t s) {
     uint32_t* n_dev = img.total + 2 * R_SLOTS;
     const bool odd = radix_sort_result_buffer((size_t)cap, 0, end_bit) == 1;
     uint32_t* va = odd ? bin.vals_alt : bin.point_list;
@@ -303,14 +305,14 @@
     const int wk = radix_sort_pairs_u32_devn(bin.keys_a, va, bin.keys_b, vb, (size_t)cap, end_bit, n_dev, bin.sort_temp, fused_ranges ? img.ranges : nullptr, s);
     STAGE_END(tm, ST_SORT);
     if (!fused_ranges) { tm.begin(); launch_tile_ranges_devn((size_t)cap, n_dev, wk ? bin.keys_b : bin.keys_a, img.ranges, s); STAGE_END(tm, ST_RANGES); }
-    tm.begin(); launch_tile_depth_sort(pa.gx * pa.gy, maxR, img.ranges, bin.point_list, geom.dkey_a, bin.vals_alt, bin.keys_a, bin.keys_b, fused_ranges, s);
+    tm.begin(); launch_tile_depth_sort(pa.gx * pa.gy, maxR, img.ranges, bin.point_list, geom.dkey_a, bin.vals_alt, bin.keys_a, bin.keys_b, fused_ranges, s, order);
     STAGE_END(tm, ST_TSORT);
     return 0;
 }
 
 int64_t bin_exact(const PreprocessArgs& pa, int end_bit, int per_tile, int64_t R, const GeomState& geom, BinState* bin,
                   const ImgState& img, const uint32_t* hR, hipEvent_t evR, bool stream, surfel_alloc_fn binning_alloc, void* binning_user,
-                  StageTimer& tm, hipStream_t s) {
+                  const TileOrderArgs* torder, bool* ordered, StageTimer& tm, hipStream_t s) {
     if (per_tile < 0 && R < 0) {
         HIP_TRY(hipEventSynchronize(evR));
         per_tile = per_tile_pays(pinned_total(hR, false), pa.P, pa.gx, pa.gy);
@@ -338,20 +340,24 @@
                           reinterpret_cast<uint32_t*>(bin->sort_temp), (uint32_t)radix_sort_head_words((size_t)R), s);
     STAGE_END(tm, ST_EMIT);
     tm.begin();
-    const int wk = radix_sort_pairs_u32(bin->keys_a, va, bin->keys_b, vb, (size_t)R, 0, end_bit, bin->sort_temp, s, true);
+    const bool fused_ranges = radix_sort_fuses_ranges((size_t)R, 0, end_bit);
+    const int wk = radix_sort_pairs_u32(bin->keys_a, va, bin->keys_b, vb, (size_t)R, 0, end_bit, bin->sort_temp, s, true, fused_ranges ? img.ranges : nullptr);
     if (wk < 0) return fail(SURFEL_E_LIMIT, "too many tile instances for the tile sort");
     STAGE_END(tm, ST_SORT);
-    tm.begin(); launch_tile_ranges(R, wk ? bin->keys_b : bin->keys_a, img.ranges, s); STAGE_END(tm, ST_RANGES);
+    if (!fused_ranges) { tm.begin(); launch_tile_ranges(R, wk ? bin->keys_b : bin->keys_a, img.ranges, s); STAGE_END(tm, ST_RANGES); }
     if (per_tile) {
-        tm.begin(); launch_tile_depth_sort(pa.gx * pa.gy, R, img.ranges, bin->point_list, geom.dkey_a, bin->vals_alt, bin->keys_a, bin->keys_b, false, s);
+        tm.begin(); launch_tile_depth_sort(pa.gx * pa.gy, R, img.ranges, bin->point_list, geom.dkey_a, bin->vals_alt, bin->keys_a, bin->keys_b, fused_ranges, s, torder);
         STAGE_END(tm, ST_TSORT);
+        if (torder) *ordered = true;
+    } else if (fused_ranges) {
+        tm.begin(); launch_tile_ranges_decode(pa.gx * pa.gy, img.ranges, s); STAGE_END(tm, ST_RANGES);
     }
     return R;
 }
 
-int blend(CapEntry* ce, int W, int H, int gx, int gy, const ImgState& img, const void* img_base, const BinState& bin, const float* rec,
-          const float* background, float* out_color, float* out_others, int avg_list, bool jac, int tile_order, StageTimer& tm, hipStream_t s) {
-    run_tile_order(ce, img.ranges, gx, gy, img.tile_map, img.total + 2 * R_SLOTS + 1, tile_order, s);
+int blend(int W, int H, int gx, int gy, const ImgState& img, const void* img_base, const BinState& bin, const float* rec,
+          const float* background, float* out_color, float* out_others, int avg_list, bool jac, const TileOrderArgs* order, StageTimer& tm, hipStream_t s) {
+    if (order) launch_tile_order(img.ranges, gx, gy, order->map, order->map_flag, order->force, order->verdict, s);
     BlendFwdArgs ba{};
     ba.W = W; ba.H = H; ba.gx = gx; ba.gy = gy;
     ba.ranges = img.ranges; ba.point_list = bin.point_list; ba.rec = rec; ba.bg = background;
@@ -419,6 +425,50 @@
     HIP_TRY(hipGetLastError());
     return 0;
 }
+int surfel_debug_sort_tile_ranges(surfel_alloc_fn scratch_alloc, void* scratch_user, uint32_t* keys, uint32_t* vals, int64_t n, int end_bit, int ntiles,
+                                  uint32_t* ranges_fused, uint32_t* ranges_ref, void* stream) {
+    if (!scratch_alloc || n <= 0 || !keys || !vals || end_bit < 1 || end_bit > 32 || ntiles <= 0 || !ranges_fused || !ranges_ref)
+        return fail(SURFEL_E_INVALID, "bad arguments");
+    hipStream_t s = static_cast<hipStream_t>(stream);
+    const size_t words = align_up((size_t)n * sizeof(uint32_t));
+    char* base = static_cast<char*>(scratch_alloc(scratch_user, 2 * words + radix_sort_scratch_bytes((size_t)n)));
+    if (!base) return fail(SURFEL_E_ALLOC, "sort scratch allocation failed");
+    uint32_t* kb = reinterpret_cast<uint32_t*>(base);
+    uint32_t* vb = reinterpret_cast<uint32_t*>(base + words);
+    const bool fused = radix_sort_fuses_ranges((size_t)n, 0, end_bit);
+    HIP_TRY(hipMemsetAsync(ranges_fused, 0, sizeof(uint2) * (size_t)ntiles, s));
+    HIP_TRY(hipMemsetAsync(ranges_ref, 0, sizeof(uint2) * (size_t)ntiles, s));
+    const int w = radix_sort_pairs_u32(keys, vals, kb, vb, (size_t)n, 0, end_bit, base + 2 * words, s, false, fused ? reinterpret_cast<uint2*>(ranges_fused) : nullptr);
+    if (w < 0) return fail(SURFEL_E_LIMIT, "sort size limit");
+    if (fused) launch_tile_ranges_decode(ntiles, reinterpret_cast<uint2*>(ranges_fused), s);
+    launch_tile_ranges(n, w ? kb : keys, reinterpret_cast<uint2*>(ranges_ref), s);
+    if (w == 1) {
+        HIP_TRY(hipMemcpyAsync(keys, kb, (size_t)n * sizeof(uint32_t), hipMemcpyDeviceToDevice, s));
+        HIP_TRY(hipMemcpyAsync(vals, vb, (size_t)n * sizeof(uint32_t), hipMemcpyDeviceToDevice, s));
+    }
+    HIP_TRY(hipGetLastError());
+    return fused ? 1 : 0;
+}
+
+int surfel_debug_tile_order(const uint32_t* ranges, int gx, int gy, int* map, uint32_t* map_flag, int force, void* stream) {
+    if (!ranges || gx <= 0 || gy <= 0 || gx > 1023 || gy > 1023 || !map || !map_flag || force < 0 || force > 2) return fail(SURFEL_E_INVALID, "bad arguments");
+    launch_tile_order(reinterpret_cast<const uint2*>(ranges), gx, gy, map, map_flag, force, nullptr, static_cast<hipStream_t>(stream));
+    HIP_TRY(hipGetLastError());
+    return 0;
+}
+
+int surfel_debug_tile_depth_sort_order(int gx, int gy, int64_t n, uint32_t* ranges, uint32_t* point_list, const uint32_t* depth_keys, uint32_t* scratch,
+                                       int decode, int* map, uint32_t* map_flag, int force, void* stream) {
+    if (gx <= 0 || gy <= 0 || gx > 1023 || gy > 1023 || n < 0 || n >= ((int64_t)1 << 30) || !ranges || !map || !map_flag || force < 0 || force > 2 ||
+        (n > 0 && (!point_list || !depth_keys || !scratch)))
+        return fail(SURFEL_E_INVALID, "bad arguments");
+    const TileOrderArgs order{1, gx, gy, map, tile_map_len(gx, gy), map_flag, force, nullptr};
+    launch_tile_depth_sort(gx * gy, n, reinterpret_cast<uint2*>(ranges), point_list, depth_keys, scratch, scratch + n, scratch + 2 * n, decode != 0,
+                           static_cast<hipStream_t>(stream), &order);
+    HIP_TRY(hipGetLastError());
+    return 0;
+}
+
 int surfel_debug_tile_depth_sort_classes(int* out, int cap) {
     if (!out || cap < 0) return fail(SURFEL_E_INVALID, "bad arguments");
     return tile_depth_sort_classes(out, cap);
@@ -552,6 +602,9 @@
     const bool jac = P > 0 && opt_stream && shs != nullptr && M == 16;
     CapEntry* ce = cap_entry(width, height);
     ce->begin_frame();
+    TileOrderArgs order{};
+    const bool want_order = plan_tile_order(ce, gx, gy, img.tile_map, img.total + 2 * R_SLOTS + 1, opt_tile_order, &order);
+    bool ordered = false;
     int64_t R = 0;
     bool blended = false;
     GeomState geom{}; BinState bin{};
@@ -598,8 +651,8 @@
             HIP_TRY(hipMemcpyAsync(hR, img.total, sizeof(uint32_t) * R_SLOTS, hipMemcpyDeviceToHost, s));
             HIP_TRY(hipEventRecord(evR, s));
         } else {
-            if (int e = bin_capacity(pa, end_bit, cap, ce->maxR, geom, bin, img, hR, evR, tm, s)) return e;
-            if (int e = blend(ce, width, height, gx, gy, img, img_base, bin, geom.rec, background, out_color, out_others, 0, jac, opt_tile_order, tm, s)) return e;
+            if (int e = bin_capacity(pa, end_bit, cap, ce->maxR, geom, bin, img, hR, evR, want_order ? &order : nullptr, tm, s)) return e;
+            if (int e = blend(width, height, gx, gy, img, img_base, bin, geom.rec, background, out_color, out_others, 0, jac, nullptr, tm, s)) return e;
             if (opt_lazy) {
                 g_lazy.pending = true; g_lazy.W = width; g_lazy.H = height; g_lazy.cap = cap; g_lazy.overflowed = false;
                 if (hipGetDevice(&g_lazy.dev) != hipSuccess) g_lazy.dev = -1;
@@ -617,14 +670,16 @@
             }
         }
         if (!blended) {
-            R = bin_exact(pa, end_bit, per_tile, cap > 0 ? R : -1, geom, &bin, img, hR, evR, opt_stream, binning_alloc, binning_user, tm, s);
+            R = bin_exact(pa, end_bit, per_tile, cap > 0 ? R : -1, geom, &bin, img, hR, evR, opt_stream, binning_alloc, binning_user,
+                          want_order ? &order : nullptr, &ordered, tm, s);
             if (R < 0) return R;
         }
         ce->record_count(R, cap > 0 && !blended);
         g_lazy.R = R;
     }
     if (!blended) {
-        if (int e = blend(ce, width, height, gx, gy, img, img_base, bin, geom.rec, background, out_color, out_others, (int)(R / ((int64_t)gx * gy)), jac, opt_tile_order, tm, s)) return e;
+        if (int e = blend(width, height, gx, gy, img, img_base, bin, geom.rec, background, out_color, out_others, (int)(R / ((int64_t)gx * gy)), jac,
+                          want_order && !ordered ? &order : nullptr, tm, s)) return e;
     }
     HIP_TRY(hipGetLastError());
     return R;
diff --git a/2d-gaussian-splatting_amd/csrc/surfel_kernels.h b/2d-gaussian-splatting_amd/csrc/surfel_kernels.h
--- a/2d-gaussian-splatting_amd/csrc/surfel_kernels.h
+++ b/2d-gaussian-splatting_amd/csrc/surfel_kernels.h
@@ -71,6 +71,7 @@
 void set_preprocess_dma(int v);
 void launch_emit_instances(int P, float* rec, const uint32_t* rects, const uint32_t* order, uint32_t id_mask, const uint32_t* offsets_sorted, uint32_t* keys,
                            uint32_t* vals, int gx, uint32_t* zero_ptr, uint32_t zero_words, hipStream_t s);
+struct TileOrderArgs;
 void launch_tile_ranges(int64_t R, const uint32_t* keys, uint2* ranges, hipStream_t s);
 int tile_map_len(int gx, int gy);
 void launch_tile_order(const uint2* ranges, int gx, int gy, int* map, uint32_t* map_flag , int force, uint32_t* verdict, hipStream_t s);
@@ -89,13 +90,15 @@
 int radix_sort_passes(size_t n, int begin_bit, int end_bit);
 int radix_sort_result_buffer(size_t n, int begin_bit, int end_bit);
 int radix_sort_pairs_u32(uint32_t* keys_a, uint32_t* vals_a, uint32_t* keys_b, uint32_t* vals_b, size_t n, int begin_bit, int end_bit,
-                         void* scratch, hipStream_t s, bool head_zeroed = false);
+                         void* scratch, hipStream_t s, bool head_zeroed = false, uint2* ranges = nullptr);
+bool radix_sort_fuses_ranges(size_t n, int begin_bit, int end_bit);
+void launch_tile_ranges_decode(int ntiles, uint2* ranges, hipStream_t s);
 size_t radix_sort_head_words(size_t n);
 size_t scan_scratch_words(size_t n);
 int tile_depth_sort_classes(int* out, int cap);
 void set_tile_radix_min(int v);
 void launch_tile_depth_sort(int ntiles, int64_t R, uint2* ranges, uint32_t* point_list, const uint32_t* depth_keys, uint32_t* tmp_ids,
-                            uint32_t* tmp_keys, uint32_t* tmp_rank, bool decode, hipStream_t s);
+                            uint32_t* tmp_keys, uint32_t* tmp_rank, bool decode, hipStream_t s, const TileOrderArgs* order = nullptr);
 void launch_scan_gather(const uint32_t* vals, const uint32_t* order, int packed, uint32_t* out, size_t n, void* zeroed_scratch, hipStream_t s);
 bool capacity_binning_ok(size_t cap, int end_bit);
 size_t capacity_sort_scratch_bytes(size_t cap, int end_bit);
diff --git a/2d-gaussian-splatting_amd/csrc/surfel_preprocess.hip b/2d-gaussian-splatting_amd/csrc/surfel_preprocess.hip
--- a/2d-gaussian-splatting_amd/csrc/surfel_preprocess.hip
+++ b/2d-gaussian-splatting_amd/csrc/surfel_preprocess.hip
@@ -1,5 +1,6 @@
 #include "surfel_common.h"
 #include "surfel_kernels.h"
+#include "surfel_tile_order.h"
 
 namespace surfel {
 
@@ -361,114 +362,13 @@
     }
 }
 
-constexpr int TO_CLASSES = 24, TO_THREADS = 1024, TO_WAVES = TO_THREADS / 64;
-__device__ __forceinline__ int len_class(uint32_t len) { return len < 16u ? 0 : min(TO_CLASSES - 1, 32 - __clz(len >> 4)); }
-
+constexpr int TO_THREADS = 1024;
 __global__ void __launch_bounds__(TO_THREADS) tile_order_kernel(const uint2* __restrict__ ranges, int gx, int gy, int* __restrict__ map, int map_len,
                                                                 uint32_t* __restrict__ map_flag, int force, uint32_t* __restrict__ verdict) {
-    __shared__ uint32_t s_wsum[TO_WAVES], s_wmax[TO_WAVES], s_bound[9], s_uniform;
-    __shared__ uint32_t s_cnt[TO_CLASSES], s_off[TO_CLASSES], s_wcnt[TO_WAVES][TO_CLASSES];
-    const int n = gx * gy, ggx = (gx + 3) >> 2, G = ggx * gy;
-    const int tid = threadIdx.x, lane = tid & 63, wave = tid >> 6;
-    const int k = (n + TO_THREADS - 1) / TO_THREADS;
-    const int q = n >> 3, r = n & 7;
-    uint32_t sum = 0, mx = 0;
-    for (int j = 0; j < k; j++) {
-        const int t = tid * k + j;
-        if (t < n) { const uint2 rg = ranges[t]; const uint32_t len = rg.y - rg.x; sum += len; mx = max(mx, len); }
-    }
-    uint32_t x = sum;
-#pragma unroll
-    for (int o = 1; o < 64; o <<= 1) { const uint32_t y = __shfl_up(x, o); if (lane >= o) x += y; }
-#pragma unroll
-    for (int o = 32; o > 0; o >>= 1) mx = max(mx, (uint32_t)__shfl_xor((int)mx, o));
-    if (lane == 63) s_wsum[wave] = x;
-    if (lane == 0) s_wmax[wave] = mx;
-    __syncthreads();
-    uint32_t pre = x - sum;
-    for (int w = 0; w < wave; w++) pre += s_wsum[w];
-    for (int j = 0; j < k; j++) {
-        const int t = tid * k + j;
-        if (t < n) {
-#pragma unroll
-            for (int xc = 0; xc < 8; xc++) {
-                const int B = xc < r ? xc * (q + 1) : r * (q + 1) + (xc - r) * q;
-                if (t == B) s_bound[xc] = pre;
-            }
-            const uint2 rg = ranges[t];
-            pre += rg.y - rg.x;
-        }
-    }
-    if (tid == TO_THREADS - 1) s_bound[8] = pre;
-    if (tid < TO_CLASSES) s_cnt[tid] = 0u;
-    __syncthreads();
-    if (tid == 0) {
-        uint32_t total = 0, maxlen = 0;
-        for (int w = 0; w < TO_WAVES; w++) { total += s_wsum[w]; maxlen = max(maxlen, s_wmax[w]); }
-        uint32_t busiest = 0;
-        for (int xc = 0; xc < 8; xc++) {
-            const uint32_t lo = q == 0 && xc >= r ? total : s_bound[xc];
-            const uint32_t hi = xc == 7 ? total : (q == 0 && xc + 1 >= r ? total : s_bound[xc + 1]);
-            busiest = max(busiest, hi - lo);
-        }
-        const bool uniform = total == 0u || ((unsigned long long)busiest * 800ull <= (unsigned long long)total * 115ull &&
-                                             (unsigned long long)maxlen * (unsigned long long)n <= 4ull * total);
-        s_uniform = force == 1 ? 1u : (force == 2 ? 0u : (uniform ? 1u : 0u));
-        if (s_uniform) map_flag[0] = 0u;
-        if (verdict) verdict[0] = uniform ? 1u : 2u;
-    }
-    __syncthreads();
-    if (s_uniform) return;
-    for (int b = tid; b < map_len; b += TO_THREADS) map[b] = -1;
-    auto group_class = [&](int g) {
-        const int ty = g / ggx, tx0 = (g - ty * ggx) << 2;
-        uint32_t len4 = 0;
-        for (int j = 0; j < 4 && tx0 + j < gx; j++) { const uint2 rg = ranges[ty * gx + tx0 + j]; len4 += rg.y - rg.x; }
-        return len_class(len4);
-    };
-    const unsigned long long lt = (1ull << lane) - 1ull;
-    for (int g0 = 0; g0 < G; g0 += TO_THREADS) {
-        const int g = g0 + tid;
-        const int c = g < G ? group_class(g) : -1;
-        unsigned long long rest = __ballot(c >= 0);
-        while (rest) {
-            const int cc = __shfl(c, __builtin_ctzll(rest));
-            const unsigned long long m = __ballot(c == cc);
-            if (lane == __builtin_ctzll(m)) atomicAdd(&s_cnt[cc], (uint32_t)__popcll(m));
-            rest &= ~m;
-        }
-    }
-    __syncthreads();
-    if (tid == 0) {
-        uint32_t run = 0;
-        for (int c = TO_CLASSES - 1; c >= 0; c--) { s_off[c] = run; run += s_cnt[c]; }
-    }
-    for (int g0 = 0; g0 < G; g0 += TO_THREADS) {
-        for (int i = tid; i < TO_WAVES * TO_CLASSES; i += TO_THREADS) (&s_wcnt[0][0])[i] = 0u;
-        __syncthreads();
-        const int g = g0 + tid;
-        const int c = g < G ? group_class(g) : -1;
-        uint32_t rank = 0;
-        unsigned long long rest = __ballot(c >= 0);
-        while (rest) {
-            const int cc = __shfl(c, __builtin_ctzll(rest));
-            const unsigned long long m = __ballot(c == cc);
-            if (c == cc) rank = (uint32_t)__popcll(m & lt);
-            if (lane == __builtin_ctzll(m)) s_wcnt[wave][cc] = (uint32_t)__popcll(m);
-            rest &= ~m;
-        }
-        __syncthreads();
-        if (c >= 0) {
-            uint32_t kpos = s_off[c] + rank;
-            for (int w = 0; w < wave; w++) kpos += s_wcnt[w][c];
-            const int ty = g / ggx, tx0 = (g - ty * ggx) << 2;
-            for (int j = 0; j < 4 && tx0 + j < gx; j++) map[((((kpos >> 3) << 2) + j) << 3) | (kpos & 7u)] = ty * gx + tx0 + j;
-        }
-        __syncthreads();
-        if (tid < TO_CLASSES) { uint32_t add = 0; for (int w = 0; w < TO_WAVES; w++) add += s_wcnt[w][tid]; s_off[tid] += add; }
-        __syncthreads();
-    }
-    if (tid == 0) map_flag[0] = 1u;
+    __shared__ TileOrderLds<TO_THREADS> s;
+    constexpr int TO_LENS = 15 * 1024;
+    __shared__ uint32_t s_len[TO_LENS];
+    tile_order_block<TO_THREADS>(ranges, gx, gy, map, map_len, map_flag, force, verdict, s, s_len, TO_LENS);
 }
 
 __global__ void __launch_bounds__(256) tile_ranges_kernel(int64_t R, const uint32_t* __restrict__ keys, uint2* __restrict__ ranges) {
diff --git a/2d-gaussian-splatting_amd/csrc/surfel_sort.hip b/2d-gaussian-splatting_amd/csrc/surfel_sort.hip
--- a/2d-gaussian-splatting_amd/csrc/surfel_sort.hip
+++ b/2d-gaussian-splatting_amd/csrc/surfel_sort.hip
@@ -6,6 +6,7 @@
 
 #include "surfel_common.h"
 #include "surfel_kernels.h"
+#include "surfel_tile_order.h"
 
 namespace surfel {
 
@@ -563,20 +564,28 @@
 __global__ void __launch_bounds__(RS_THREADS) tile_depth_sort_kernel(uint2* __restrict__ ranges, uint32_t* __restrict__ point_list,
                                                                     const uint32_t* __restrict__ depth_keys, uint32_t* __restrict__ tmp_ids,
                                                                     uint32_t* __restrict__ tmp_keys, uint32_t* __restrict__ tmp_rank, int decode,
-                                                                    uint32_t radix_min) {
+                                                                    uint32_t radix_min, TileOrderArgs to) {
     static_assert(TS_CAP % RS_THREADS == 0 && TS_CAP * 8 + 4 * TR_WAVES * RS_RADIX >= TR_BITONIC_MAX * 8, "LDS layout");
     __shared__ unsigned long long s_raw[TS_CAP + TR_WAVES * RS_RADIX / 2];
     __shared__ uint32_t s_w[3 * TR_WAVES];
     unsigned long long* s = s_raw;
     uint32_t (*s_cnt)[RS_RADIX] = reinterpret_cast<uint32_t (*)[RS_RADIX]>(s_raw);
     uint2* s_item = reinterpret_cast<uint2*>(s_raw + TR_WAVES * RS_RADIX / 2);
-    uint2 rg = ranges[blockIdx.x];
+    if (to.on && blockIdx.x == 0) {
+        constexpr int TO_STATE = (int)((sizeof(TileOrderLds<RS_THREADS>) + 7) / 8);
+        static_assert(TO_STATE < TS_CAP, "the ordering block's state fits the sorter's LDS");
+        tile_order_block<RS_THREADS>(ranges, to.gx, to.gy, to.map, to.map_len, to.map_flag, to.force, to.verdict, *reinterpret_cast<TileOrderLds<RS_THREADS>*>(s_raw),
+                                     reinterpret_cast<uint32_t*>(s_raw + TO_STATE), 2 * (int)(sizeof(s_raw) / 8 - TO_STATE));
+        return;
+    }
+    const uint32_t tile = blockIdx.x - (uint32_t)to.on;
+    uint2 rg = ranges[tile];
     if (decode) {
         rg.x = __builtin_amdgcn_readfirstlane(rg.x); rg.y = __builtin_amdgcn_readfirstlane(rg.y);
         __syncthreads();
         if (rg.y != 0u) {
             rg.x = ~rg.x;
-            if (threadIdx.x == 0) ranges[blockIdx.x].x = rg.x;
+            if (threadIdx.x == 0) ranges[tile].x = rg.x;
         }
     }
     const uint32_t n = rg.y - rg.x;
@@ -609,18 +618,32 @@
 }
 
 void launch_tile_depth_sort(int ntiles, int64_t R, uint2* ranges, uint32_t* point_list, const uint32_t* depth_keys, uint32_t* tmp_ids,
-                            uint32_t* tmp_keys, uint32_t* tmp_rank, bool decode, hipStream_t st) {
+                            uint32_t* tmp_keys, uint32_t* tmp_rank, bool decode, hipStream_t st, const TileOrderArgs* order) {
     if (ntiles <= 0) return;
+    TileOrderArgs to{};
+    if (order) { to = *order; to.on = 1; }
     if (R <= (int64_t)TS_SMALL_MAX_AVG * ntiles)
-        hipLaunchKernelGGL(tile_depth_sort_kernel<TS_CAP_SMALL>, dim3(ntiles), dim3(RS_THREADS), 0, st, ranges, point_list, depth_keys, tmp_ids,
-                           tmp_keys, tmp_rank, decode ? 1 : 0, (uint32_t)g_tile_radix_min);
+        hipLaunchKernelGGL(tile_depth_sort_kernel<TS_CAP_SMALL>, dim3(ntiles + to.on), dim3(RS_THREADS), 0, st, ranges, point_list, depth_keys, tmp_ids,
+                           tmp_keys, tmp_rank, decode ? 1 : 0, (uint32_t)g_tile_radix_min, to);
     else
-        hipLaunchKernelGGL(tile_depth_sort_kernel<TS_CAP_LARGE>, dim3(ntiles), dim3(RS_THREADS), 0, st, ranges, point_list, depth_keys, tmp_ids,
-                           tmp_keys, tmp_rank, decode ? 1 : 0, (uint32_t)g_tile_radix_min);
-}
-
+        hipLaunchKernelGGL(tile_depth_sort_kernel<TS_CAP_LARGE>, dim3(ntiles + to.on), dim3(RS_THREADS), 0, st, ranges, point_list, depth_keys, tmp_ids,
+                           tmp_keys, tmp_rank, decode ? 1 : 0, (uint32_t)g_tile_radix_min, to);
+}
+
+__global__ void __launch_bounds__(RS_THREADS) tile_ranges_decode_kernel(uint2* __restrict__ ranges, int ntiles) {
+    const int t = blockIdx.x * RS_THREADS + threadIdx.x;
+    if (t < ntiles && ranges[t].y != 0u) ranges[t].x = ~ranges[t].x;
+}
+void launch_tile_ranges_decode(int ntiles, uint2* ranges, hipStream_t s) {
+    if (ntiles > 0) hipLaunchKernelGGL(tile_ranges_decode_kernel, dim3((ntiles + RS_THREADS - 1) / RS_THREADS), dim3(RS_THREADS), 0, s, ranges, ntiles);
+}
+
+bool radix_sort_fuses_ranges(size_t n, int begin_bit, int end_bit) {
+    return n > 0 && n < ST_VALUE && begin_bit == 0 && end_bit > 0 && radix_sort_passes(n, 0, end_bit) <= RS_MAX_PASSES && !use_rocprim(n, 0, end_bit);
+}
 int radix_sort_pairs_u32(uint32_t* keys_a, uint32_t* vals_a, uint32_t* keys_b, uint32_t* vals_b, size_t n, int begin_bit, int end_bit,
-                         void* scratch, hipStream_t s, bool head_zeroed) {
+                         void* scratch, hipStream_t s, bool head_zeroed, uint2* ranges) {
+    if (ranges && !radix_sort_fuses_ranges(n, begin_bit, end_bit)) return -1;
     if (n == 0 || end_bit <= begin_bit) return 0;
     if (n >= ST_VALUE) return -1;
     const uint32_t nblocks = rs_nblocks(n);
@@ -645,7 +668,7 @@
             hipLaunchKernelGGL(rs_hist_fat_kernel<FT_IPT>, dim3(fb), dim3(FTH_THREADS), 0, s, kin, (uint32_t)n, bit, mask, hist, fb);
             hipLaunchKernelGGL(rs_scan_kernel, dim3(RS_RADIX), dim3(RS_THREADS), 0, s, hist, fb, total);
             hipLaunchKernelGGL((os_pass_fat_kernel<false, FT_IPT>), dim3(fb), dim3(FT_THREADS), 0, s, kin, vin, kout, vout, (uint32_t)n, bit, mask, total, hist,
-                               (uint32_t*)nullptr, (const uint32_t*)nullptr, 1, (uint2*)nullptr, fb);
+                               (uint32_t*)nullptr, (const uint32_t*)nullptr, 1, p == passes - 1 ? ranges : (uint2*)nullptr, fb);
             cur ^= 1;
         }
         return cur;
@@ -662,7 +685,8 @@
         const uint32_t* kin = cur ? keys_b : keys_a; const uint32_t* vin = cur ? vals_b : vals_a;
         uint32_t* kout = cur ? keys_a : keys_b; uint32_t* vout = cur ? vals_a : vals_b;
         hipLaunchKernelGGL((os_pass_fat_kernel<true, FT_IPT>), dim3(ft_nblocks(n)), dim3(FT_THREADS), 0, s, kin, vin, kout, vout, (uint32_t)n, bit, mask,
-                           ghist + p * RS_RADIX, status + (size_t)p * nblocks * RS_RADIX, ticket + p, (const uint32_t*)nullptr, 1, (uint2*)nullptr, 0u);
+                           ghist + p * RS_RADIX, status + (size_t)p * nblocks * RS_RADIX, ticket + p, (const uint32_t*)nullptr, 1,
+                           p == passes - 1 ? ranges : (uint2*)nullptr, 0u);
         cur ^= 1;
     }
     return cur;
diff --git a/2d-gaussian-splatting_amd/csrc/surfel_tile_order.h b/2d-gaussian-splatting_amd/csrc/surfel_tile_order.h
--- /dev/null
+++ b/2d-gaussian-splatting_amd/csrc/surfel_tile_order.h
@@ -0,0 +1,135 @@
+#pragma once
+#include <hip/hip_runtime.h>
+#include <stdint.h>
+
+namespace surfel {
+
+constexpr int TO_CLASSES = 24;
+__device__ __forceinline__ int len_class(uint32_t len) { return len < 16u ? 0 : min(TO_CLASSES - 1, 32 - __clz(len >> 4)); }
+
+__device__ __forceinline__ uint32_t tile_list_len(const uint2* ranges, int t) {
+    const uint2 rg = ranges[t];
+    return rg.y == 0u ? 0u : rg.y - (rg.x >= rg.y ? ~rg.x : rg.x);
+}
+
+template <int NT>
+struct TileOrderLds {
+    uint32_t wsum[NT / 64], wmax[NT / 64], bound[9], uniform;
+    uint32_t cnt[TO_CLASSES], off[TO_CLASSES], wcnt[NT / 64][TO_CLASSES];
+};
+
+template <int NT>
+__device__ __forceinline__ void tile_order_block(const uint2* ranges, int gx, int gy, int* __restrict__ map, int map_len,
+                                                 uint32_t* __restrict__ map_flag, int force, uint32_t* __restrict__ verdict,
+                                                 TileOrderLds<NT>& s, uint32_t* lens, int cap) {
+    constexpr int NW = NT / 64;
+    const int n = gx * gy, ggx = (gx + 3) >> 2, G = ggx * gy;
+    const int tid = threadIdx.x, lane = tid & 63, wave = tid >> 6;
+    const int ns = min(n, cap);
+#pragma unroll 8
+    for (int t = tid; t < ns; t += NT) lens[t] = tile_list_len(ranges, t);
+    __syncthreads();
+    auto len_of = [&](int t) { return t < ns ? lens[t] : tile_list_len(ranges, t); };
+    const int k = (n + NT - 1) / NT;
+    const int q = n >> 3, r = n & 7;
+    uint32_t sum = 0, mx = 0;
+    for (int j = 0; j < k; j++) {
+        const int t = tid * k + j;
+        if (t < n) { const uint32_t len = len_of(t); sum += len; mx = max(mx, len); }
+    }
+    uint32_t x = sum;
+#pragma unroll
+    for (int o = 1; o < 64; o <<= 1) { const uint32_t y = __shfl_up(x, o); if (lane >= o) x += y; }
+#pragma unroll
+    for (int o = 32; o > 0; o >>= 1) mx = max(mx, (uint32_t)__shfl_xor((int)mx, o));
+    if (lane == 63) s.wsum[wave] = x;
+    if (lane == 0) s.wmax[wave] = mx;
+    __syncthreads();
+    uint32_t pre = x - sum;
+    for (int w = 0; w < wave; w++) pre += s.wsum[w];
+    for (int j = 0; j < k; j++) {
+        const int t = tid * k + j;
+        if (t < n) {
+#pragma unroll
+            for (int xc = 0; xc < 8; xc++) {
+                const int B = xc < r ? xc * (q + 1) : r * (q + 1) + (xc - r) * q;
+                if (t == B) s.bound[xc] = pre;
+            }
+            pre += len_of(t);
+        }
+    }
+    if (tid == NT - 1) s.bound[8] = pre;
+    if (tid < TO_CLASSES) s.cnt[tid] = 0u;
+    __syncthreads();
+    if (tid == 0) {
+        uint32_t total = 0, maxlen = 0;
+        for (int w = 0; w < NW; w++) { total += s.wsum[w]; maxlen = max(maxlen, s.wmax[w]); }
+        uint32_t busiest = 0;
+        for (int xc = 0; xc < 8; xc++) {
+            const uint32_t lo = q == 0 && xc >= r ? total : s.bound[xc];
+            const uint32_t hi = xc == 7 ? total : (q == 0 && xc + 1 >= r ? total : s.bound[xc + 1]);
+            busiest = max(busiest, hi - lo);
+        }
+        const bool uniform = total == 0u || ((unsigned long long)busiest * 800ull <= (unsigned long long)total * 115ull &&
+                                             (unsigned long long)maxlen * (unsigned long long)n <= 4ull * total);
+        s.uniform = force == 1 ? 1u : (force == 2 ? 0u : (uniform ? 1u : 0u));
+        if (s.uniform) map_flag[0] = 0u;
+        if (verdict) verdict[0] = uniform ? 1u : 2u;
+    }
+    __syncthreads();
+    if (s.uniform) return;
+    for (int b = tid; b < map_len; b += NT) map[b] = -1;
+    auto group_class = [&](int g) {
+        const int ty = g / ggx, tx0 = (g - ty * ggx) << 2;
+        uint32_t len4 = 0;
+        for (int j = 0; j < 4 && tx0 + j < gx; j++) len4 += len_of(ty * gx + tx0 + j);
+        return len_class(len4);
+    };
+    const unsigned long long lt = (1ull << lane) - 1ull;
+    for (int g0 = 0; g0 < G; g0 += NT) {
+        const int g = g0 + tid;
+        const int c = g < G ? group_class(g) : -1;
+        unsigned long long rest = __ballot(c >= 0);
+        while (rest) {
+            const int cc = __shfl(c, __builtin_ctzll(rest));
+            const unsigned long long m = __ballot(c == cc);
+            if (lane == __builtin_ctzll(m)) atomicAdd(&s.cnt[cc], (uint32_t)__popcll(m));
+            rest &= ~m;
+        }
+    }
+    __syncthreads();
+    if (tid == 0) {
+        uint32_t run = 0;
+        for (int c = TO_CLASSES - 1; c >= 0; c--) { s.off[c] = run; run += s.cnt[c]; }
+    }
+    for (int g0 = 0; g0 < G; g0 += NT) {
+        for (int i = tid; i < NW * TO_CLASSES; i += NT) (&s.wcnt[0][0])[i] = 0u;
+        __syncthreads();
+        const int g = g0 + tid;
+        const int c = g < G ? group_class(g) : -1;
+        uint32_t rank = 0;
+        unsigned long long rest = __ballot(c >= 0);
+        while (rest) {
+            const int cc = __shfl(c, __builtin_ctzll(rest));
+            const unsigned long long m = __ballot(c == cc);
+            if (c == cc) rank = (uint32_t)__popcll(m & lt);
+            if (lane == __builtin_ctzll(m)) s.wcnt[wave][cc] = (uint32_t)__popcll(m);
+            rest &= ~m;
+        }
+        __syncthreads();
+        if (c >= 0) {
+            uint32_t kpos = s.off[c] + rank;
+            for (int w = 0; w < wave; w++) kpos += s.wcnt[w][c];
+            const int ty = g / ggx, tx0 = (g - ty * ggx) << 2;
+            for (int j = 0; j < 4 && tx0 + j < gx; j++) map[((((kpos >> 3) << 2) + j) << 3) | (kpos & 7u)] = ty * gx + tx0 + j;
+        }
+        __syncthreads();
+        if (tid < TO_CLASSES) { uint32_t add = 0; for (int w = 0; w < NW; w++) add += s.wcnt[w][tid]; s.off[tid] += add; }
+        __syncthreads();
+    }
+    if (tid == 0) map_flag[0] = 1u;
+}
+
+struct TileOrderArgs { int on; int gx, gy; int* map; int map_len; uint32_t* map_flag; int force; uint32_t* verdict; };
+
+}
diff --git a/2d-gaussian-splatting_amd/surfel_native.py b/2d-gaussian-splatting_amd/surfel_native.py
--- a/2d-gaussian-splatting_amd/surfel_native.py
+++ b/2d-gaussian-splatting_amd/surfel_native.py
@@ -88,6 +88,9 @@
         "surfel_stage_name": (C.c_char_p, _i),
         "surfel_debug_sort_pairs": (_i, _a, _u, _d, _d, _i64, _i, _i, _s),
         "surfel_debug_tile_depth_sort": (_i, _i, _i64, _d, _d, _d, _d, _i, _s),
+        "surfel_debug_tile_depth_sort_order": (_i, _i, _i, _i64, _d, _d, _d, _d, _i, _d, _d, _i, _s),
+        "surfel_debug_tile_order": (_i, _d, _i, _i, _d, _d, _i, _s),
+        "surfel_debug_sort_tile_ranges": (_i, _a, _u, _d, _d, _i64, _i, _i, _d, _d, _s),
         "surfel_debug_tile_depth_sort_classes": (_i, _ip, _i),
         "surfel_debug_set_tile_radix_min": (_i, _i),
         "surfel_debug_set_blend_stats": (_i, _d),
@@ -301,7 +304,12 @@
                 "(hipcc --offload-arch=gfx950). There is no CPU / PyTorch fallback for the rasterizer." % LIB_PATH)
         lib = C.CDLL(LIB_PATH)
         for name, (restype, *argtypes) in _SIG.items():
-            fn = getattr(lib, name)
+            try:
+                fn = getattr(lib, name)
+            except AttributeError:
+                if os.environ.get("SURFEL_LIB") and name.startswith("surfel_debug_"):
+                    continue
+                raise
             fn.restype, fn.argtypes = restype, argtypes
         if lib.surfel_abi_version() != 1:
             raise ImportError("libsurfel_hip.so ABI version mismatch")
diff --git a/include/surfel_debug.h b/include/surfel_debug.h
--- a/include/surfel_debug.h
+++ b/include/surfel_debug.h
@@ -17,6 +17,11 @@
 
 int surfel_debug_tile_depth_sort(int ntiles, int64_t n, uint32_t* ranges, uint32_t* point_list, const uint32_t* depth_keys, uint32_t* scratch,
                                  int decode, void* stream);
+int surfel_debug_tile_depth_sort_order(int gx, int gy, int64_t n, uint32_t* ranges, uint32_t* point_list, const uint32_t* depth_keys, uint32_t* scratch,
+                                       int decode, int* map, uint32_t* map_flag, int force, void* stream);
+int surfel_debug_tile_order(const uint32_t* ranges, int gx, int gy, int* map, uint32_t* map_flag, int force, void* stream);
+int surfel_debug_sort_tile_ranges(surfel_alloc_fn scratch_alloc, void* scratch_user, uint32_t* keys, uint32_t* vals, int64_t n, int end_bit, int ntiles,
+                                  uint32_t* ranges_fused, uint32_t* ranges_ref, void* stream);
 int surfel_debug_tile_depth_sort_classes(int* out, int cap);
 int surfel_debug_set_tile_radix_min(int longest_network_run);
 
```
